# ThomasZiegler/RS-aware-differential-SfM

Hardware: AMD Instinct MI355X
Metric: Mpixels/sec RS depth+pose solve, 1280x720 pair (higher is better)
Workload: dtype f64

## Files before the change

### rs-aware-differential-sfm_amd/csrc/frame_host.hip

```cpp
#include <stdlib.h>
#include <string.h>

#include <atomic>

#include <algorithm>
#include <new>

#include "rsdsfm_internal.hpp"
#include "sequence_host.hpp"

namespace rsdsfm {

static std::atomic<int> g_frames_in_flight[64];
int frames_in_flight(const Ctx* c) { return g_frames_in_flight[c->device & 63].load(std::memory_order_relaxed); }

int alpha_ones_launch(Ctx* c, double* d_alpha, int64_t n);
int flatten_device(Ctx* c, const double* d_img, int32_t rows, int32_t cols, int32_t col0, double fx, double fy, double cx, double cy, double gamma,
                   double thr, double* d_q, double* d_u, double* d_alpha, double* d_alpha_k, int64_t* n_out);

struct FrameRun {
    rsdsfm_frame_job job;
    rsdsfm_frame_params prm;
    size_t N = 0;
    int64_t n = 0;
    double *d_q = nullptr, *d_u = nullptr, *d_a = nullptr, *d_ak = nullptr, *d_in_a = nullptr, *d_in_ak = nullptr, *d_inl = nullptr, *d_inl_ref = nullptr;
    int64_t* d_idx = nullptr;
    uint8_t* d_mask = nullptr;
    int32_t* d_ys = nullptr;
    double *d_zpartials = nullptr, *d_zheader = nullptr;
    char* d_refine_ws = nullptr;
    rsdsfm_ransac_out ro;
    RansacRun ransac;
    RefineRun refine;
    Minimal9Direct direct;
    DenseFlatten dense;
    bool refinement_enqueued = false, ahead = false, side_flatten = false, dense_in_launch = false, open = false;
    bool counted = false;
    int rc_begin = RSDSFM_OK;
    int64_t m_known = -1;
    RefineTail tail;
    FinishClaim claim;
    RansacSpecTail spec_tail;
    std::function<int()> join;
};

namespace {

inline double* header_host(Ctx* c) { return reinterpret_cast<double*>(static_cast<char*>(c->h_pinned) + c->pinned_bytes - 64); }
inline RefineState* state_host(Ctx* c) { return reinterpret_cast<RefineState*>(static_cast<char*>(c->h_pinned) + c->pinned_bytes - kPinnedTail); }
inline int64_t* count_host(Ctx* c) { return reinterpret_cast<int64_t*>(static_cast<char*>(c->h_pinned) + c->pinned_bytes - kPinnedTail / 2); }
static_assert(sizeof(RefineState) + sizeof(int) <= kPinnedTail / 2, "reserved tail: state read-back | point count ... depth-map header");

struct StreamSwap {
    Ctx* c;
    hipStream_t main;
    StreamSwap(Ctx* ctx, hipStream_t other) : c(ctx), main(ctx->stream) { c->stream = other; }
    ~StreamSwap() { c->stream = main; }
};

int ensure_side_stream(Ctx* c) {
    if (c->aux_stream) return RSDSFM_OK;
    RSDSFM_HIP_CHECK(c, hipStreamCreateWithFlags(&c->aux_stream, hipStreamNonBlocking));
    RSDSFM_HIP_CHECK(c, hipEventCreateWithFlags(&c->ev_fork, hipEventDisableTiming));
    RSDSFM_HIP_CHECK(c, hipEventCreateWithFlags(&c->ev_join, hipEventDisableTiming));
    return RSDSFM_OK;
}

static void frame_uncount(const Ctx* c, FrameRun* F) {
    if (F && F->counted) {
        F->counted = false;
        g_frames_in_flight[c->device & 63].fetch_sub(1, std::memory_order_relaxed);
    }
}
struct FrameInFlightEnd {
    const Ctx* c;
    FrameRun* F;
    ~FrameInFlightEnd() { frame_uncount(c, F); }
};

int frame_begin(Ctx* c, FrameRun* F) {
    const rsdsfm_frame_job& J = F->job;
    const rsdsfm_frame_params* prm = &F->prm;
    frame_uncount(c, F);
    F->open = false;
    F->rc_begin = RSDSFM_OK;
    if (J.rows <= 0 || J.cols <= 0 || !J.d_flow_img || !J.d_depth_map_colmajor) return fail(c, RSDSFM_ERR_INVALID, "bad arguments");
    if (prm->flow_index_mode != RSDSFM_FLOW_COMPAT_RANK && prm->flow_index_mode != RSDSFM_FLOW_GATHERED) return fail(c, RSDSFM_ERR_INVALID, "unknown flow_index_mode");
    if (prm->struct_bytes != 0 && prm->struct_bytes != (int32_t)sizeof(rsdsfm_frame_params))
        return fail(c, RSDSFM_ERR_INVALID, "rsdsfm_frame_params: struct_bytes is neither 0 nor sizeof(rsdsfm_frame_params) -- caller built against another header (use rsdsfm_frame_params_init)");
    const int32_t rows = J.rows, cols = J.cols;
    const double fx = J.fx, fy = J.fy, cx = J.cx, cy = J.cy, gamma = J.gamma;
    const size_t N = (size_t)rows * (size_t)cols;
    F->N = N;
    const size_t ncells = (size_t)flatten_cells(rows, cols);
    const size_t need = 2 * Arena::need(16 * N) + 4 * Arena::need(8 * N) + 2 * Arena::need(24 * N) + Arena::need(8 * N) + Arena::need(N) +
                        Arena::need(4 * N) + Arena::need(8 * 1024) + Arena::need(64) + Arena::need(refine_workspace_bytes(c, (int64_t)N, true)) +
                        2 * Arena::need(sizeof(int64_t) * (ncells + 2048)) + Arena::need(64) + 4096;
    if (need > c->frame_bytes) {
        RSDSFM_HIP_CHECK(c, hipStreamSynchronize(c->stream));
        if (c->d_frame) RSDSFM_HIP_CHECK(c, hipFree(c->d_frame));
        c->d_frame = nullptr;
        c->frame_bytes = 0;
        RSDSFM_HIP_CHECK(c, hipMalloc(&c->d_frame, need));
        c->frame_bytes = need;
    }
    Arena fa(c->d_frame);
    F->d_q = fa.take<double>(2 * N);
    F->d_u = fa.take<double>(2 * N);
    F->d_a = fa.take<double>(N);
    F->d_ak = fa.take<double>(N);
    F->d_in_a = fa.take<double>(N);
    F->d_in_ak = fa.take<double>(N);
    F->d_inl = fa.take<double>(3 * N);
    F->d_inl_ref = fa.take<double>(3 * N);
    F->d_idx = fa.take<int64_t>(N);
    F->d_mask = fa.take<uint8_t>(N);
    F->d_ys = fa.take<int32_t>(N);
    F->d_zpartials = fa.take<double>(1024);
    F->d_zheader = fa.take<double>(8);
    F->d_refine_ws = fa.take<char>(refine_workspace_bytes(c, (int64_t)N, true));
    int64_t* d_flat_counts = fa.take<int64_t>(ncells);
    int64_t* d_flat_offsets = fa.take<int64_t>(ncells + 2048);

    int rc = ensure_pinned(c, ransac_pinned_bytes(prm->ransac_trials));
    if (rc != RSDSFM_OK) return rc;
    int64_t n = (int64_t)N;
    F->side_flatten = false;
    if (c->frame_dense_hint) {
        *count_host(c) = -1;
        int side = prm->ransac_trials > 0 ? c->frame_side_flatten : 0;
        if (side == 3 && prm->ransac_trials > c->num_cus * 2) side = 0;
        F->dense_in_launch = false;
        if (side) {
            F->side_flatten = true;
            F->direct = Minimal9Direct();
            F->direct.img = J.d_flow_img, F->direct.rows = rows, F->direct.cols = cols, F->direct.alpha_ones = prm->use_global_shutter_mode ? 1 : 0;
            F->direct.fx = fx, F->direct.fy = fy, F->direct.cx = cx, F->direct.cy = cy, F->direct.gamma = gamma;
        }
        if (side == 3) {
            if (!c->d_flat_counters) {
                RSDSFM_HIP_CHECK(c, hipMalloc(reinterpret_cast<void**>(&c->d_flat_counters), 2 * sizeof(unsigned long long)));
                RSDSFM_HIP_CHECK(c, hipMemsetAsync(c->d_flat_counters, 0, 2 * sizeof(unsigned long long), c->stream));
            }
            F->dense = DenseFlatten();
            F->dense.thr = prm->flow_threshold;
            F->dense.d_q = F->d_q, F->dense.d_u = F->d_u, F->dense.d_alpha = F->d_a, F->dense.d_alpha_k = F->d_ak;
            F->dense.d_counters = c->d_flat_counters;
            F->dense.total_out = count_host(c);
            F->dense_in_launch = true;
        } else if (side == 2) {
            F->join = [c, F, d_flat_counts, d_flat_offsets]() -> int {
                const rsdsfm_frame_job& J2 = F->job;
                int rc2 = flatten_launch(c, J2.d_flow_img, J2.rows, J2.cols, 0, J2.fx, J2.fy, J2.cx, J2.cy, J2.gamma, F->prm.flow_threshold, F->d_q, F->d_u, F->d_a,
                                         F->d_ak, d_flat_counts, d_flat_offsets, count_host(c), nullptr);
                if (rc2 == RSDSFM_OK && F->prm.use_global_shutter_mode) rc2 = alpha_ones_launch(c, F->d_a, (int64_t)F->N);
                return rc2;
            };
        } else if (side == 1) {
            rc = ensure_side_stream(c);
            if (rc != RSDSFM_OK) return rc;
            RSDSFM_HIP_CHECK(c, hipEventRecord(c->ev_fork, c->stream));
            RSDSFM_HIP_CHECK(c, hipStreamWaitEvent(c->aux_stream, c->ev_fork, 0));
            {
                StreamSwap on_side(c, c->aux_stream);
                rc = flatten_launch(c, J.d_flow_img, rows, cols, 0, fx, fy, cx, cy, gamma, prm->flow_threshold, F->d_q, F->d_u, F->d_a, F->d_ak,
                                    d_flat_counts, d_flat_offsets, count_host(c), nullptr);
                if (rc == RSDSFM_OK && prm->use_global_shutter_mode) rc = alpha_ones_launch(c, F->d_a, n);
            }
            if (rc != RSDSFM_OK) return rc;
            RSDSFM_HIP_CHECK(c, hipEventRecord(c->ev_join, c->aux_stream));
            F->join = [c]() -> int {
                RSDSFM_HIP_CHECK(c, hipStreamWaitEvent(c->stream, c->ev_join, 0));
                return RSDSFM_OK;
            };
        } else {
            rc = flatten_enqueue(c, J.d_flow_img, rows, cols, fx, fy, cx, cy, gamma, prm->flow_threshold, F->d_q, F->d_u, F->d_a, F->d_ak, count_host(c));
            if (rc != RSDSFM_OK) return rc;
        }
    } else {
        rc = flatten_device(c, J.d_flow_img, rows, cols, 0, fx, fy, cx, cy, gamma, prm->flow_threshold, F->d_q, F->d_u, F->d_a, F->d_ak, &n);
        if (rc != RSDSFM_OK) return rc;
        *count_host(c) = n;
    }
    if (prm->use_global_shutter_mode && !F->side_flatten) {
        rc = alpha_ones_launch(c, F->d_a, n);
        if (rc != RSDSFM_OK) return rc;
    }
    F->n = n;
    memset(&F->ro, 0, sizeof(F->ro));
    F->ro.inlier_idx = F->d_idx;
    F->ro.inliers = F->d_inl;
    F->ro.alpha = F->d_in_a;
    F->ro.alpha_k = F->d_in_ak;
    F->ro.mask = F->d_mask;
    F->m_known = -1;
    F->tail = [c, F](const RefineBuffers& B) -> int {
        const rsdsfm_frame_job& J2 = F->job;
        const RefineState* st = B.state;
        const int64_t m_arg = F->m_known >= 0 ? F->m_known : F->n;
        const int64_t* m_dev = F->m_known >= 0 ? nullptr : &st->m;
        PoseTableOut pt;
        if (J2.d_R_rows9_or_null && J2.d_t_rows3_or_null)
            pt.R = J2.d_R_rows9_or_null, pt.t = J2.d_t_rows3_or_null, pt.rows = J2.rows, pt.gamma = J2.gamma, pt.wk_dev = st->p + 3;
        if (B.claim.on)
            return depth_map_decided_launch(c, F->d_inl_ref, m_arg, F->d_zpartials, refine_finish_grid(c, B), B, J2.d_depth_map_colmajor, F->d_zheader,
                                            header_host(c), st->p, m_dev, &pt);
        return depth_map_slab_launch(c, F->d_inl_ref, m_arg, F->d_zpartials, refine_finish_grid(c, B), m_arg, nullptr, J2.fx, J2.fy, J2.cx, J2.cy, J2.rows,
                                     0, J2.cols, J2.d_depth_map_colmajor, nullptr, F->d_ys, F->d_zheader, header_host(c), st->p, m_dev, &pt);
    };
    F->claim = FinishClaim();
    if (c->frame_tail == 0) {
        F->claim.on = true;
        F->claim.fx = J.fx, F->claim.fy = J.fy, F->claim.cx = J.cx, F->claim.cy = J.cy;
        F->claim.rows = rows, F->claim.cols = cols;
        F->claim.ys = F->d_ys;
    }
    F->spec_tail = [c, F](const RansacBest* d_best) -> int {
        return refine_begin(c, F->d_u, F->n, F->n, F->d_inl, F->d_in_a, F->d_in_ak, F->d_idx, nullptr, nullptr, 0.0, F->prm.use_acceleration_mode,
                            F->prm.flow_index_mode, F->d_inl_ref, &F->tail, d_best, F->d_refine_ws, &F->refine, state_host(c), F->d_zpartials, false,
                            &F->claim);
    };
    F->refinement_enqueued = false;
    F->ahead = prm->use_refinement && c->ransac_spec_miss < 2;
    F->open = true;
    g_frames_in_flight[c->device & 63].fetch_add(1, std::memory_order_relaxed);
    F->counted = true;
    F->rc_begin = ransac_begin(c, F->d_q, F->d_u, F->d_a, F->d_ak, n, prm->use_acceleration_mode, prm->ransac_trials, prm->ransac_tol, nullptr, J.seed,
                               prm->depth_mode, prm->k_sign_mode, &F->ro, prm->use_refinement ? &F->spec_tail : nullptr, &F->refinement_enqueued, &F->ransac,
                               F->side_flatten ? &F->direct : nullptr, F->side_flatten && !F->dense_in_launch ? &F->join : nullptr,
                               F->dense_in_launch ? &F->dense : nullptr, F->ahead, true,
                               F->claim.on && prm->use_refinement ? refine_flag_words(F->d_refine_ws) : nullptr);
    return RSDSFM_OK;
}

int frame_finish(Ctx* c, FrameRun* F, rsdsfm_frame_result* res) {
    if (!F->open) return fail(c, RSDSFM_ERR_INVALID, "no frame solve in flight");
    F->open = false;
    FrameInFlightEnd in_flight_end_{c, F};
    const rsdsfm_frame_job& J = F->job;
    const rsdsfm_frame_params* prm = &F->prm;
    memset(res, 0, sizeof(*res));
    int rc = F->rc_begin;
    if (rc == RSDSFM_OK) rc = ransac_finish(c, &F->ransac);
    if (rc != RSDSFM_OK) RSDSFM_HIP_CHECK(c, hipStreamSynchronize(c->stream));
    if (F->side_flatten && c->aux_stream) RSDSFM_HIP_CHECK(c, hipStreamSynchronize(c->aux_stream));
    int64_t n = F->n;
    if (*count_host(c) < 0) {
        c->frame_dense_hint = 1;
        return rc != RSDSFM_OK ? rc : fail(c, RSDSFM_ERR_NUMERIC, "frame solve: the point count did not arrive");
    }
    bool counted = true;
    if (*count_host(c) != n) {
        if (F->dense_in_launch) {
            int64_t n_real = 0;
            rc = flatten_device(c, J.d_flow_img, J.rows, J.cols, 0, J.fx, J.fy, J.cx, J.cy, J.gamma, prm->flow_threshold, F->d_q, F->d_u, F->d_a, F->d_ak, &n_real);
            if (rc == RSDSFM_OK && prm->use_global_shutter_mode) rc = alpha_ones_launch(c, F->d_a, n_real);
            if (rc != RSDSFM_OK) return rc;
            *count_host(c) = n_real;
        }
        n = *count_host(c);
        F->n = n;
        F->refinement_enqueued = false;
        counted = false;
        rc = ransac_begin(c, F->d_q, F->d_u, F->d_a, F->d_ak, n, prm->use_acceleration_mode, prm->ransac_trials, prm->ransac_tol, nullptr, J.seed,
                          prm->depth_mode, prm->k_sign_mode, &F->ro, prm->use_refinement ? &F->spec_tail : nullptr, &F->refinement_enqueued, &F->ransac, nullptr, nullptr,
                          nullptr, F->ahead, true,
                               F->claim.on && prm->use_refinement ? refine_flag_words(F->d_refine_ws) : nullptr);
        if (rc == RSDSFM_OK) rc = ransac_finish(c, &F->ransac);
        counted = rc == RSDSFM_OK;
    }
    c->frame_dense_hint = n == (int64_t)F->N ? 1 : 0;
    if (rc != RSDSFM_OK) return rc;
    if (counted) ransac_commit_hints(c, F->ransac);
    const rsdsfm_ransac_out& ro = F->ro;
    res->n_points = n;
    res->num_inliers = ro.num_inliers;
    res->best_trial = ro.best_trial;
    memcpy(res->ransac_w, ro.w, sizeof(ro.w));
    memcpy(res->ransac_v, ro.v, sizeof(ro.v));
    res->ransac_k = ro.k;
    double v[3], w[3], k = ro.k;
    for (int i = 0; i < 3; ++i) v[i] = ro.v[i], w[i] = ro.w[i];
    double* d_final = F->d_inl;
    int flipped = 0;
    F->m_known = ro.num_inliers;
    if (prm->use_refinement) {
        bool exact = false;
        if (F->refinement_enqueued) {
            rc = refine_poll(c, &F->refine, v, w, &k, &res->refine_summary);
            exact = rc == kRcRefineRestartExact;
        }
        if (!F->refinement_enqueued || exact)
            rc = refine_device(c, F->d_u, n, ro.num_inliers, F->d_inl, F->d_in_a, F->d_in_ak, F->d_idx, v, w, k, prm->use_acceleration_mode,
                               prm->flow_index_mode, F->d_inl_ref, v, w, &k, &res->refine_summary, &F->tail, F->d_zpartials, exact, &F->claim);
        if (rc != RSDSFM_OK) return rc;
        d_final = F->d_inl_ref;
        const double* h_header = header_host(c);
        flipped = h_header[0] != 0.0;
        v[0] = h_header[1], v[1] = h_header[2], v[2] = h_header[3];
    } else {
        rc = depth_map_device(c, d_final, ro.num_inliers, v, J.fx, J.fy, J.cx, J.cy, J.rows, J.cols, J.d_depth_map_colmajor, nullptr, F->d_ys, &flipped, w,
                              k, J.gamma, J.d_R_rows9_or_null, J.d_t_rows3_or_null);
        if (rc != RSDSFM_OK) return rc;
    }
    res->flipped = flipped;
    memcpy(res->v, v, sizeof(v));
    memcpy(res->w, w, sizeof(w));
    res->k = k;
    res->d_inliers = d_final;
    res->d_inlier_idx = F->d_idx;
    res->d_scanline = F->d_ys;
    return RSDSFM_OK;
}

FrameRun* frame_run_of(Ctx* c) {
    if (!c->frame_run) c->frame_run = new (std::nothrow) FrameRun();
    return static_cast<FrameRun*>(c->frame_run);
}

}

void frame_release(Ctx* c) {
    frame_uncount(c, static_cast<FrameRun*>(c->frame_run));
    delete static_cast<FrameRun*>(c->frame_run);
    c->frame_run = nullptr;
    for (rsdsfm_ctx* lane : c->lanes) rsdsfm_destroy(lane);
    c->lanes.clear();
    if (c->ev_fork) (void)hipEventDestroy(c->ev_fork);
    if (c->ev_join) (void)hipEventDestroy(c->ev_join);
    if (c->ev_seq) (void)hipEventDestroy(c->ev_seq);
    if (c->aux_stream) (void)hipStreamDestroy(c->aux_stream);
    if (c->d_flat_counters) (void)hipFree(c->d_flat_counters);
    c->d_flat_counters = nullptr;
    c->ev_fork = c->ev_join = c->ev_seq = nullptr;
    c->aux_stream = nullptr;
}

}

using namespace rsdsfm;

extern "C" {

void rsdsfm_frame_params_init(rsdsfm_frame_params* p) {
    if (!p) return;
    memset(p, 0, sizeof(*p));
    p->ransac_trials = 5;
    p->use_acceleration_mode = 0;
    p->use_refinement = 1;
    p->depth_mode = RSDSFM_DEPTH_CERES_LM;
    p->k_sign_mode = RSDSFM_K_COMPAT;
    p->flow_index_mode = RSDSFM_FLOW_COMPAT_RANK;
    p->use_global_shutter_mode = 0;
    p->struct_bytes = (int32_t)sizeof(rsdsfm_frame_params);
    p->ransac_tol = 0.05;
    p->flow_threshold = 1e-10;
    p->seed = 1;
}

int rsdsfm_solve_frame_dev(rsdsfm_ctx* ctx, const double* d_flow_img, int32_t rows, int32_t cols, double fx, double fy, double cx,
                           double cy, double gamma, const rsdsfm_frame_params* prm, double* d_depth_map, double* d_R_rows9,
                           double* d_t_rows3, rsdsfm_frame_result* res) {
    if (!ctx) return RSDSFM_ERR_INVALID;
    Ctx* c = &ctx->c;
    DeviceGuard device_guard_(c);
    if (!prm || !res) return fail(c, RSDSFM_ERR_INVALID, "bad arguments");
    FrameRun* F = frame_run_of(c);
    if (!F) return fail(c, RSDSFM_ERR_INVALID, "out of host memory");
    F->prm = *prm;
    F->job = rsdsfm_frame_job{d_flow_img, rows, cols, fx, fy, cx, cy, gamma, d_depth_map, d_R_rows9, d_t_rows3, prm->seed};
    int rc = frame_begin(c, F);
    if (rc != RSDSFM_OK) return rc;
    return frame_finish(c, F, res);
}

int rsdsfm_set_sequence_lanes(rsdsfm_ctx* ctx, int32_t lanes) {
    if (!ctx) return RSDSFM_ERR_INVALID;
    Ctx* c = &ctx->c;
    DeviceGuard device_guard_(c);
    if (lanes < 0 || lanes > 16) return fail(c, RSDSFM_ERR_INVALID, "lanes must be 0 (default) .. 16");
    c->seq_lanes = lanes;
    return RSDSFM_OK;
}

int rsdsfm_set_frame_tail(rsdsfm_ctx* ctx, int mode) {
    if (!ctx) return RSDSFM_ERR_INVALID;
    if (mode < 0 || mode > 1) return fail(&ctx->c, RSDSFM_ERR_INVALID, "mode must be 0 (short launch tail) or 1 (stage-by-stage launches)");
    ctx->c.frame_tail = mode;
    return RSDSFM_OK;
}

int rsdsfm_set_frame_side_flatten(rsdsfm_ctx* ctx, int mode) {
    if (!ctx) return RSDSFM_ERR_INVALID;
    if (mode < 0 || mode > 3) return fail(&ctx->c, RSDSFM_ERR_INVALID, "mode must be 0 (flatten first), 1 (flatten on a second stream), 2 (flatten behind the minimal solver) or 3 (flatten inside the solver's launch)");
    ctx->c.frame_side_flatten = mode;
    return RSDSFM_OK;
}

}

namespace rsdsfm {

int sequence_lane_count(const Ctx* c, int count) { return std::max(1, std::min<int>(count, c->seq_lanes > 0 ? c->seq_lanes : kSequenceLanesDefault)); }

int solve_frames_run(Ctx* c, const rsdsfm_frame_job* jobs, int32_t count, const rsdsfm_frame_params* prm, rsdsfm_frame_result* results, const PairHook* hook) {
    const int L = sequence_lane_count(c, count);
    while ((int)c->lanes.size() < L - 1) {
        rsdsfm_ctx* lane = nullptr;
        int rc = rsdsfm_create(&lane, c->device, nullptr);
        if (rc != RSDSFM_OK) return fail(c, rc, "could not create a sequence lane");
        c->lanes.push_back(lane);
    }
    auto lane_ctx = [&](int l) -> Ctx* { return l == 0 ? c : &c->lanes[(size_t)l - 1]->c; };
    if (L > 1) {
        if (!c->ev_seq) RSDSFM_HIP_CHECK(c, hipEventCreateWithFlags(&c->ev_seq, hipEventDisableTiming));
        RSDSFM_HIP_CHECK(c, hipEventRecord(c->ev_seq, c->stream));
    }
    for (int l = 1; l < L; ++l) {
        Ctx* lc = lane_ctx(l);
        RSDSFM_HIP_CHECK(c, hipStreamWaitEvent(lc->stream, c->ev_seq, 0));
        lc->ransac_k0 = c->ransac_k0;
        lc->ransac_math_mode = c->ransac_math_mode;
        lc->lm_arithmetic = c->lm_arithmetic;
        lc->refine_arithmetic = c->refine_arithmetic;
        lc->lma_count_only_force = c->lma_count_only_force;
        lc->frame_side_flatten = c->frame_side_flatten;
        lc->frame_tail = c->frame_tail;
        lc->refine_stage_mode = c->refine_stage_mode;
    }
    for (int l = 0; l < L; ++l) lane_ctx(l)->refine_stage_separate = L > 1;
    int first_error = RSDSFM_OK;
    int in_flight[16];
    for (int l = 0; l < 16; ++l) in_flight[l] = -1;
    auto finish_lane = [&](int l) {
        const int i = in_flight[l];
        if (i < 0) return;
        in_flight[l] = -1;
        Ctx* lc = lane_ctx(l);
        int rc = frame_finish(lc, static_cast<FrameRun*>(lc->frame_run), &results[i]);
        if (rc != RSDSFM_OK && first_error == RSDSFM_OK) {
            first_error = rc;
            if (lc != c) c->err = "pair " + std::to_string(i) + ": " + lc->err;
        }
        if (rc == RSDSFM_OK && hook && first_error == RSDSFM_OK) {
            rc = (*hook)(lc, i, static_cast<FrameRun*>(lc->frame_run)->job, results[i]);
            if (rc != RSDSFM_OK) {
                first_error = rc;
                c->err = "pair " + std::to_string(i) + ": " + std::string(lc->err);
            }
        }
    };
    for (int i = 0; i < count && first_error == RSDSFM_OK; ++i) {
        const int l = i % L;
        finish_lane(l);
        if (first_error != RSDSFM_OK) break;
        Ctx* lc = lane_ctx(l);
        FrameRun* F = frame_run_of(lc);
        if (!F) {
            first_error = fail(c, RSDSFM_ERR_INVALID, "out of host memory");
            break;
        }
        F->prm = *prm;
        F->job = jobs[i];
        int rc = frame_begin(lc, F);
        if (rc != RSDSFM_OK) {
            first_error = rc;
            if (lc != c) c->err = "pair " + std::to_string(i) + ": " + lc->err;
            break;
        }
        in_flight[l] = i;
    }
    for (;;) {
        int best = -1;
        for (int l = 0; l < L; ++l)
            if (in_flight[l] >= 0 && (best < 0 || in_flight[l] < in_flight[best])) best = l;
        if (best < 0) break;
        finish_lane(best);
    }
    for (int l = 0; l < L; ++l) lane_ctx(l)->refine_stage_separate = false;
    return first_error;
}

}

extern "C" {

int rsdsfm_solve_frames_dev(rsdsfm_ctx* ctx, const rsdsfm_frame_job* jobs, int32_t count, const rsdsfm_frame_params* prm, rsdsfm_frame_result* results) {
    if (!ctx) return RSDSFM_ERR_INVALID;
    Ctx* c = &ctx->c;
    DeviceGuard device_guard_(c);
    if (count < 0 || !prm || (count > 0 && (!jobs || !results))) return fail(c, RSDSFM_ERR_INVALID, "bad arguments");
    if (count == 0) return RSDSFM_OK;
    return solve_frames_run(c, jobs, count, prm, results, nullptr);
}

int rsdsfm_set_refine_stage(rsdsfm_ctx* ctx, int mode) {
    if (!ctx) return RSDSFM_ERR_INVALID;
    Ctx* c = &ctx->c;
    if (mode < 0 || mode > 2) return fail(c, RSDSFM_ERR_INVALID, "refine stage: 0 (automatic), 1 (in the next pass's prologue) or 2 (a launch of its own)");
    c->refine_stage_mode = mode;
    return RSDSFM_OK;
}

}
```

### rs-aware-differential-sfm_amd/csrc/ransac_host.hip

```cpp
#include <stdio.h>
#include <stdlib.h>
#include <string.h>

#include <algorithm>
#include <vector>

#include "rsdsfm_internal.hpp"

namespace rsdsfm {

namespace {


inline uint64_t splitmix64(uint64_t& state) {
    uint64_t z = (state += 0x9E3779B97F4A7C15ULL);
    z = (z ^ (z >> 30)) * 0xBF58476D1CE4E5B9ULL;
    z = (z ^ (z >> 27)) * 0x94D049BB133111EBULL;
    return z ^ (z >> 31);
}

void sample_indices(int64_t n, int T, uint64_t seed, std::vector<int32_t>& out) {
    struct Slot {
        int64_t key;
        int32_t val;
        uint32_t gen;
    };
    thread_local std::vector<Slot> table;
    thread_local uint32_t gen = 0;
    size_t cap = 64;
    while (cap < (size_t)T * 18 * 4) cap <<= 1;
    if (table.size() != cap || gen == 0xFFFFFFFFu) {
        table.assign(cap, Slot{-1, 0, 0});
        gen = 0;
    }
    gen += 1;
    Slot* tb = table.data();
    const uint32_t g = gen;
    auto slot = [&](int64_t i) -> size_t {
        size_t h = (size_t)(((uint64_t)i * 0x9E3779B97F4A7C15ull) >> 20) & (cap - 1);
        while (tb[h].gen == g && tb[h].key != i) h = (h + 1) & (cap - 1);
        return h;
    };
    auto get = [&](int64_t i) -> int32_t {
        const size_t h = slot(i);
        return tb[h].gen == g ? tb[h].val : (int32_t)i;
    };
    auto put = [&](int64_t i, int32_t v) {
        const size_t h = slot(i);
        tb[h].key = i;
        tb[h].val = v;
        tb[h].gen = g;
    };
    out.resize((size_t)T * 9);
    uint64_t st = seed;
    for (int t = 0; t < T; ++t) {
        int64_t n_temp = n;
        for (int j = 0; j < 9; ++j) {
            const int64_t r = (int64_t)(splitmix64(st) % (uint64_t)n_temp);
            const int32_t a = get(n_temp - 1), b = get(r);
            put(n_temp - 1, b);
            put(r, a);
            out[(size_t)t * 9 + j] = b;
            n_temp--;
        }
    }
}

}

void sample_indices(int64_t n, int T, uint64_t seed, int32_t* out) {
    std::vector<int32_t> v;
    sample_indices(n, T, seed, v);
    if (!v.empty()) memcpy(out, v.data(), sizeof(int32_t) * v.size());
}

size_t ransac_pinned_bytes(int T) {
    const size_t Tn = (size_t)std::max(T, 1);
    return sizeof(RansacBest) + 8 * sizeof(int) + sizeof(double) * 2 * Tn + sizeof(double) * 8 * Tn + sizeof(LmState) * Tn + 64 +
           sizeof(int32_t) * Tn * 9 + kPinnedTail;
}

namespace {

enum RansacPc { kPcStart = 0, kPcBatchBegin, kPcRoundEnqueue, kPcRoundWait, kPcAfterRounds, kPcScore, kPcFinal, kPcFinalWait, kPcDone };

int lma_start_over(Ctx* c, RansacRun& R, int guards) {
    R.analytic = false;
    R.lma_restarted = true;
    R.lma_guard |= guards;
    R.tie_margin = -kLmaTie;
    R.not_one_step = 0;
    R.final_done = R.spec_scored = R.tail_enqueued = R.spec_final = false;
    RSDSFM_HIP_CHECK(c, hipMemsetAsync(R.zero_begin, 0, R.zero_bytes, c->stream));
    R.b0 = 0;
    R.pc = kPcBatchBegin;
    return RSDSFM_OK;
}

int ransac_advance(Ctx* c, RansacRun& R, bool yield_at_wait) {
    rsdsfm_ransac_out* out = R.out;
    const int T = R.T, Tn = R.Tn, batch = R.batch, depth_mode = R.depth_mode;
    const int64_t n = R.n;
    const double tol = R.tol;
    int rc = RSDSFM_OK;
    for (;;) {
        switch (R.pc) {
            case kPcStart: {
                const bool zero_in_minimal9 = T > 0 && R.zero_bytes % 8 == 0 && (reinterpret_cast<uintptr_t>(R.zero_begin) & 7) == 0;
                if (!zero_in_minimal9) RSDSFM_HIP_CHECK(c, hipMemsetAsync(R.zero_begin, 0, R.zero_bytes, c->stream));
                if (T > 0) {
                    memcpy(R.h_samples_pinned, R.samples.data(), sizeof(int32_t) * (size_t)T * 9);
                    Minimal9Direct dir = R.direct ? *R.direct : Minimal9Direct();
                    R.core_epoch = 0;
                    if (R.core_math && depth_mode == RSDSFM_DEPTH_CERES_LM && T <= c->num_cus * 2 && c->d_core_flag) {
                        c->core_epoch = c->core_epoch >= 0x3fffffff ? 1 : c->core_epoch + 1;
                        dir.core_flag = c->d_core_flag;
                        dir.core_epoch = R.core_epoch = c->core_epoch;
                    }
                    if (R.direct && R.dense && T <= c->num_cus * 2)
                        rc = minimal9_flatten_launch(c, R.h_samples_pinned, T, R.use_alpha_k, R.k_sign_mode, R.d_hyp, zero_in_minimal9 ? R.zero_begin : nullptr,
                                                     zero_in_minimal9 ? R.zero_bytes : 0, dir, R.dense->thr, R.dense->d_q, R.dense->d_u, R.dense->d_alpha,
                                                     R.dense->d_alpha_k, R.dense->d_counters, R.dense->total_out);
                    else
                        rc = minimal9_launch(c, R.d_q, R.d_u, R.d_a, R.d_ak, R.h_samples_pinned, T, R.use_alpha_k, R.k_sign_mode, R.d_hyp,
                                             zero_in_minimal9 ? R.zero_begin : nullptr, zero_in_minimal9 ? R.zero_bytes : 0, &dir);
                    if (rc != RSDSFM_OK) return rc;
                    if (R.after_minimal9) {
                        rc = (*R.after_minimal9)();
                        if (rc != RSDSFM_OK) return rc;
                    }
                }
                R.b0 = 0;
                R.pc = kPcBatchBegin;
                break;
            }
            case kPcBatchBegin: {
                if (R.b0 >= T) {
                    R.pc = kPcFinal;
                    break;
                }
                R.B = std::min(batch, T - R.b0);
                R.need_score = true;
                if (depth_mode == RSDSFM_DEPTH_CERES_LM) {
                    if (R.b0 > 0)
                        RSDSFM_HIP_CHECK(c, hipMemsetAsync(R.d_flags, 0, (size_t)(reinterpret_cast<char*>(R.d_irr_count + R.batch) - reinterpret_cast<char*>(R.d_flags)), c->stream));
                    R.round = 0;
                    R.pc = kPcRoundEnqueue;
                } else {
                    R.pc = kPcScore;
                }
                break;
            }
            case kPcRoundEnqueue: {
                const int b0 = R.b0, B = R.B, round = R.round;
                bool flags_via_pick = false;
                if (round > 4 * kMaxIter) return fail(c, RSDSFM_ERR_NUMERIC, "LM state machines did not terminate");
                if (R.analytic && round == 0) {
                    rc = ransac_lma_launch(c, R.d_q, R.d_u, R.d_a, R.d_ak, n, R.d_hyp + (size_t)b0 * 8, B, R.d_states + b0, R.d_partials, R.d_flags,
                                           R.d_scored + b0, R.d_tcount + b0, R.d_terr + b0, tol, R.lma_cand, 2, R.d_irr_count, R.d_irr_list, R.d_unscored,
                                           nullptr, R.core_epoch ? c->d_core_flag : nullptr, R.core_epoch, R.count_only);
                } else {
                    rc = ransac_lm_round_launch(c, R.d_q, R.d_u, R.d_a, R.d_ak, n, R.d_hyp + (size_t)b0 * 8, B, R.d_states + b0, R.d_partials, R.d_flags,
                                                R.d_scored + b0, R.d_tcount + b0, R.d_terr + b0, round, tol, R.k0, R.fused_base, R.core_math,
                                                R.core_epoch ? c->d_core_flag : nullptr, R.core_epoch, R.d_unscored);
                }
                if (rc != RSDSFM_OK) return rc;
                if (round == 0 && B == T) {
                    const PickLazy lazy = R.count_only ? PickLazy{R.d_scored, R.d_unscored, R.d_flags + 1} : PickLazy();
                    if (c->ransac_score_idle < kScoreIdleLimit) {
                        if (R.count_only) {
                            rc = ransac_pick_launch(c, R.d_tcount, R.d_terr, T, R.d_hyp, R.d_best, nullptr, R.d_flags, nullptr, 0, nullptr, 0, 0, nullptr, 0.0, lazy);
                            if (rc != RSDSFM_OK) return rc;
                        }
                        rc = ransac_score_launch(c, R.d_q, R.d_u, R.d_a, R.d_ak, n, R.d_hyp, T, R.d_states, depth_mode, tol, R.d_scored, R.d_partials,
                                                 R.d_tcount, R.d_terr, R.d_unscored, R.d_flags + 1);
                        if (rc != RSDSFM_OK) return rc;
                        R.spec_scored = true;
                    }
                    rc = ransac_pick_launch(c, R.d_tcount, R.d_terr, T, R.d_hyp, R.d_best, R.h_best, R.d_flags, R.h_running, R.spec_scored ? 1 : 0,
                                            nullptr, 0, 0, nullptr, R.tie_margin, lazy);
                    if (rc != RSDSFM_OK) return rc;
                    flags_via_pick = true;
                    rc = ransac_final_launch(c, R.d_q, R.d_u, R.d_a, R.d_ak, n, R.d_best, R.d_states, depth_mode, tol, R.d_rho, R.d_mask, R.d_bcounts,
                                             R.d_boffs, out->inlier_idx, out->inliers, out->alpha, out->alpha_k, R.h_best, R.refine_flag_words);
                    if (rc != RSDSFM_OK) return rc;
                    R.final_done = true;
                    R.spec_final = true;
                    if (R.spec_tail && R.tail_ahead) {
                        rc = (*R.spec_tail)(R.d_best);
                        if (rc != RSDSFM_OK) return rc;
                        R.tail_enqueued = true;
                    }
                }
                if (!flags_via_pick) RSDSFM_HIP_CHECK(c, hipMemcpyAsync(R.h_running, R.d_flags, sizeof(int) * 8, hipMemcpyDeviceToHost, c->stream));
                R.pc = kPcRoundWait;
                if (yield_at_wait) return RSDSFM_OK;
                break;
            }
            case kPcRoundWait: {
                yield_at_wait = false;
                if (int rcs = sync_stream(c, "ransac_finish line 244")) return rcs;
                const int* h_running = R.h_running;
                if (R.round == 0 && R.analytic && (h_running[3] & 16) != 0) R.lma_guard |= h_running[3] >> 8;
                if (R.round == 0 && R.analytic && (h_running[3] & 6) != 0 && !((h_running[3] & 1) && R.core_math)) {
                    rc = lma_start_over(c, R, (h_running[3] >> 8) | ((h_running[3] & 4) ? (1 << 7) : 0));
                    if (rc != RSDSFM_OK) return rc;
                    break;
                }
                if (R.round == 0 && R.core_math && (h_running[3] & 1) != 0) {
                    R.core_math = false;
                    R.restarted = true;
                    R.not_one_step = 0;
                    R.final_done = R.spec_scored = R.tail_enqueued = R.spec_final = false;
                    R.dense = nullptr;
                    R.after_minimal9 = nullptr;
                    R.pc = kPcStart;
                    break;
                }
                if (R.round == 0) {
                    R.not_one_step += h_running[2];
                    if (R.b0 == 0) {
                        int best = 0;
                        for (int a2 = 1; a2 <= 3; ++a2)
                            if (h_running[4 + a2] > (best ? h_running[4 + best] : 0)) best = a2;
                        if (best) R.fused_base_next = best;
                        int second = 0;
                        for (int a2 = 1; a2 <= 3; ++a2)
                            if (a2 != best && h_running[4 + a2] > (second ? h_running[4 + second] : 0)) second = a2;
                        if (best) {
                            R.lma_cand_next[0] = best;
                            R.lma_cand_next[1] = second ? second : (best > 1 ? best - 1 : 2);
                        }
                    }
                }
                if (h_running[0] == 0) {
                    R.pc = kPcAfterRounds;
                } else {
                    R.final_done = false;
                    R.round += 1;
                    R.pc = kPcRoundEnqueue;
                }
                break;
            }
            case kPcAfterRounds: {
                R.need_score = R.h_running[1] > 0;
                if (R.B == T) R.score_hint_next = R.need_score ? 1 : 0;
                if (R.need_score && R.final_done && R.spec_scored && !R.h_best->lazy_pending) R.need_score = false;
                if (R.need_score) R.final_done = false;
                R.pc = kPcScore;
                break;
            }
            case kPcScore: {
                if (R.need_score) {
                    rc = ransac_score_launch(c, R.d_q, R.d_u, R.d_a, R.d_ak, n, R.d_hyp + (size_t)R.b0 * 8, R.B, R.d_states + R.b0, depth_mode, tol,
                                             depth_mode == RSDSFM_DEPTH_CERES_LM ? R.d_scored + R.b0 : nullptr, R.d_partials, R.d_tcount + R.b0,
                                             R.d_terr + R.b0, depth_mode == RSDSFM_DEPTH_CERES_LM ? R.d_unscored : nullptr, R.d_flags + 1);
                    if (rc != RSDSFM_OK) return rc;
                }
                R.b0 += batch;
                R.pc = kPcBatchBegin;
                break;
            }
            case kPcFinal: {
                if (!R.final_done) {
                    R.tail_enqueued = false;
                    R.spec_final = false;
                    rc = ransac_pick_launch(c, R.d_tcount, R.d_terr, T, R.d_hyp, R.d_best, R.h_best, nullptr, nullptr, 0, nullptr, 0, 0, nullptr, R.tie_margin,
                                            R.count_only ? PickLazy{R.d_scored, R.d_unscored, R.d_flags + 1} : PickLazy());
                    if (rc != RSDSFM_OK) return rc;
                    rc = ransac_final_launch(c, R.d_q, R.d_u, R.d_a, R.d_ak, n, R.d_best, R.d_states, depth_mode, tol, R.d_rho, R.d_mask, R.d_bcounts,
                                             R.d_boffs, out->inlier_idx, out->inliers, out->alpha, out->alpha_k, R.h_best, R.refine_flag_words);
                    if (rc != RSDSFM_OK) return rc;
                }
                if (R.spec_tail && !R.tail_enqueued) {
                    rc = (*R.spec_tail)(R.d_best);
                    if (rc != RSDSFM_OK) return rc;
                    R.tail_enqueued = true;
                }
                if (T > 0 && out->trial_count) RSDSFM_HIP_CHECK(c, hipMemcpyAsync(R.h_tcount, R.d_tcount, sizeof(double) * T, hipMemcpyDeviceToHost, c->stream));
                if (T > 0 && out->trial_err) RSDSFM_HIP_CHECK(c, hipMemcpyAsync(R.h_terr, R.d_terr, sizeof(double) * T, hipMemcpyDeviceToHost, c->stream));
                if (T > 0 && out->trial_vel) RSDSFM_HIP_CHECK(c, hipMemcpyAsync(R.h_hyp, R.d_hyp, sizeof(double) * 8 * T, hipMemcpyDeviceToHost, c->stream));
                if (T > 0 && out->trial_steps && depth_mode == RSDSFM_DEPTH_CERES_LM)
                    RSDSFM_HIP_CHECK(c, hipMemcpyAsync(R.h_states, R.d_states, sizeof(LmState) * T, hipMemcpyDeviceToHost, c->stream));
                R.pc = kPcFinalWait;
                if (yield_at_wait) return RSDSFM_OK;
                break;
            }
            case kPcFinalWait: {
                if (int rcs = sync_stream(c, "ransac_finish line 345")) return rcs;
                const RansacBest* h_best = R.h_best;
#ifdef RSDSFM_DEBUG_HOOKS
                if (getenv("RSDSFM_RANSAC_DEBUG")) fprintf(stderr, "[ransac] final wait: lazy_pending %d undecided %d flags %d %d %d %d hist %d %d %d %d spec_scored %d spec_final %d tail %d idle %d\n", h_best->lazy_pending, h_best->undecided, R.h_running[0], R.h_running[1], R.h_running[2], R.h_running[3], R.h_running[4], R.h_running[5], R.h_running[6], R.h_running[7], (int)R.spec_scored, (int)R.spec_final, (int)R.tail_enqueued, c->ransac_score_idle);
#endif
                if (R.count_only && h_best->lazy_pending) {
                    if (++R.lazy_rounds > T + 2) return fail(c, RSDSFM_ERR_NUMERIC, "lazy error sums did not settle");
                    R.final_done = R.tail_enqueued = R.spec_final = false;
                    R.need_score = true;
                    R.score_hint_next = 1;
                    R.b0 = 0;
                    R.B = T;
                    R.pc = kPcScore;
                    break;
                }
                if (R.analytic && h_best->lma_tie) {
                    rc = lma_start_over(c, R, 1 << 7);
                    if (rc != RSDSFM_OK) return rc;
                    break;
                }
                R.lma_tie_seen = h_best->lma_tie != 0;
                R.shared_best = h_best->shared_best;
                if (h_best->num_inliers != h_best->num_inliers_scan) {
                    if (R.analytic) {
                        rc = lma_start_over(c, R, 1 << 10);
                        if (rc != RSDSFM_OK) return rc;
                        break;
                    }
                    return fail(c, RSDSFM_ERR_NUMERIC, "inlier count mismatch between scoring and compaction");
                }
                out->num_inliers = h_best->num_inliers;
                out->best_trial = h_best->best_trial;
                memcpy(out->w, &h_best->hyp[0], 3 * sizeof(double));
                memcpy(out->v, &h_best->hyp[3], 3 * sizeof(double));
                out->k = h_best->hyp[6];
                out->inlier_error = h_best->inlier_error;
                for (int t = 0; t < T; ++t) {
                    if (out->trial_count) out->trial_count[t] = (int64_t)R.h_tcount[t];
                    if (out->trial_err) out->trial_err[t] = R.h_terr[t];
                    if (out->trial_vel) memcpy(out->trial_vel + (size_t)7 * t, R.h_hyp + (size_t)8 * t, 7 * sizeof(double));
                    if (out->trial_steps) out->trial_steps[t] = depth_mode == RSDSFM_DEPTH_CERES_LM ? R.h_states[t].num_successful : 1;
                }
                if (R.spec_tail_held) *R.spec_tail_held = R.tail_enqueued;
                R.hints_ready = true;
                R.pc = kPcDone;
                (void)Tn;
                return RSDSFM_OK;
            }
            default:
                return RSDSFM_OK;
        }
    }
}

}

void ransac_commit_hints(Ctx* c, const RansacRun& R) {
    if (!R.hints_ready || R.depth_mode != RSDSFM_DEPTH_CERES_LM || R.T <= 0) return;
    if (R.fused_base_next) c->ransac_fused_base = R.fused_base_next;
    if (R.score_hint_next >= 0) c->ransac_score_idle = R.score_hint_next ? 0 : std::min(c->ransac_score_idle + 1, kScoreIdleLimit);
    c->ransac_not_one_step = R.not_one_step;
    c->ransac_spec_miss = R.spec_final ? 0 : std::min(c->ransac_spec_miss + 1, 2);
    if (R.count_only) c->lma_count_only_runs += 1, c->lma_lazy_runs += (R.lazy_rounds > 0 || R.shared_best > 1) ? 1 : 0;
    if (R.lazy_rounds > 0 || R.shared_best > 1) c->lma_unique_run = 0;
    else if (R.shared_best == 1) c->lma_unique_run = std::min(c->lma_unique_run + 1, 2);
    if (R.lma_guard) c->lma_last_guard = R.lma_guard, c->lma_handed_over += 1;
    if (R.lma_restarted) {
        c->lma_hold = 16;
        c->lma_restarts += 1;
        c->lma_last_guard = R.lma_guard;
    } else if (c->lma_hold > 0 && !R.analytic) {
        c->lma_hold = R.lma_tie_seen ? 16 : c->lma_hold - 1;
    }
    if (R.restarted) {
        c->ransac_standard_math = 16;
        c->ransac_restarts += 1;
    } else if (c->ransac_standard_math > 0) {
        c->ransac_standard_math -= 1;
    }
}

int ransac_begin(Ctx* c, const double* d_q, const double* d_u, const double* d_a, const double* d_ak, int64_t n, int use_alpha_k, int T,
                 double tol, const int32_t* h_samples, uint64_t seed, int depth_mode, int k_sign_mode, rsdsfm_ransac_out* out,
                 const RansacSpecTail* spec_tail, bool* spec_tail_held, RansacRun* run, const Minimal9Direct* direct,
                 const std::function<int()>* after_minimal9, const DenseFlatten* dense, bool tail_ahead, bool count_only, int* refine_flag_words) {
    RansacRun& R = *run;
    R = RansacRun();
    R.tail_ahead = tail_ahead;
    R.core_math = c->ransac_math_mode == 0 && c->ransac_standard_math == 0;
    R.analytic = depth_mode == RSDSFM_DEPTH_CERES_LM && T > 0 && c->lm_arithmetic == 0 && c->lma_hold == 0;
    R.tie_margin = depth_mode != RSDSFM_DEPTH_CERES_LM || c->lm_arithmetic != 0 ? 0.0 : (R.analytic ? kLmaTie : -kLmaTie);
    R.lma_cand[0] = c->lma_cand[0], R.lma_cand[1] = c->lma_cand[1];
    R.count_only = count_only && R.analytic && T <= kRansacBatch && (c->lma_unique_run >= 2 || c->lma_count_only_force);
    if (R.count_only) R.tie_margin = 0.0;
    R.refine_flag_words = refine_flag_words;
    if (spec_tail_held) *spec_tail_held = false;
    if (!out) return fail(c, RSDSFM_ERR_INVALID, "null out");
    if (n < 9) return fail(c, RSDSFM_ERR_INVALID, "ransac needs at least 9 points (the reference would compute rand() % 0)");
    if (T < 0) return fail(c, RSDSFM_ERR_INVALID, "negative iterations");
    if (depth_mode != RSDSFM_DEPTH_CLOSED_FORM && depth_mode != RSDSFM_DEPTH_CERES_LM) return fail(c, RSDSFM_ERR_INVALID, "unknown depth_mode");
    if (n > (int64_t)INT32_MAX) return fail(c, RSDSFM_ERR_INVALID, "n exceeds the int32 sample index range");
    if (T > 0) {
        if (h_samples) {
            R.samples.assign(h_samples, h_samples + (size_t)T * 9);
            for (int32_t s : R.samples)
                if (s < 0 || s >= n) return fail(c, RSDSFM_ERR_INVALID, "sample index out of range");
        } else {
            sample_indices(n, T, seed, R.samples);
        }
    }
    const int Tn = std::max(T, 1);
    const int batch = std::min(Tn, kRansacBatch);
    const size_t partials_doubles = std::max<size_t>((size_t)ransac_lm_partials_doubles(c, n, batch), (size_t)ransac_lma_partials_doubles(c, n, batch));
    size_t need = Arena::need(sizeof(double) * Tn * 8) + Arena::need(sizeof(int) * batch) + Arena::need(sizeof(int) * ransac_lma_list_ints(batch)) +
                  Arena::need(sizeof(LmState) * Tn) + Arena::need(sizeof(double) * partials_doubles) +
                  Arena::need(sizeof(int) * 8) + 2 * Arena::need(sizeof(int) * Tn) + 2 * Arena::need(sizeof(double) * Tn) + Arena::need(sizeof(RansacBest)) +
                  2 * Arena::need(sizeof(int64_t) * 2048) + Arena::need(sizeof(double) * (size_t)n) + Arena::need((size_t)n) + 4096;
    int rc = ensure_ws(c, need);
    if (rc != RSDSFM_OK) return rc;
    Arena ws(c->d_ws);
    R.d_hyp = ws.take<double>((size_t)Tn * 8);
    R.zero_begin = ws.base + ws.off;
    R.d_states = ws.take<LmState>(Tn);
    R.d_scored = ws.take<int>(Tn);
    R.d_flags = ws.take<int>(8);
    R.d_irr_count = ws.take<int>(batch);
    R.zero_bytes = (size_t)((ws.base + ws.off) - R.zero_begin);
    R.d_irr_list = ws.take<int>(ransac_lma_list_ints(batch));
    R.d_unscored = ws.take<int>(batch);
    R.d_partials = ws.take<double>(partials_doubles);
    R.d_tcount = ws.take<double>(Tn);
    R.d_terr = ws.take<double>(Tn);
    R.d_best = ws.take<RansacBest>(1);
    R.d_bcounts = ws.take<int64_t>(2048);
    R.d_boffs = ws.take<int64_t>(2048);
    R.d_rho = out->inv_depth ? out->inv_depth : ws.take<double>((size_t)n);
    R.d_mask = out->mask ? out->mask : ws.take<uint8_t>((size_t)n);

    rc = ensure_pinned(c, ransac_pinned_bytes(T));
    if (rc != RSDSFM_OK) return rc;
    if (!c->d_core_flag) {
        RSDSFM_HIP_CHECK(c, hipMalloc(reinterpret_cast<void**>(&c->d_core_flag), 64));
        RSDSFM_HIP_CHECK(c, hipMemsetAsync(c->d_core_flag, 0, 64, c->stream));
    }
    char* hp = static_cast<char*>(c->h_pinned);
    R.h_best = reinterpret_cast<RansacBest*>(hp);
    R.h_running = reinterpret_cast<int*>(hp + sizeof(RansacBest));
    R.h_tcount = reinterpret_cast<double*>(hp + sizeof(RansacBest) + 32);
    R.h_terr = R.h_tcount + Tn;
    R.h_hyp = R.h_terr + Tn;
    R.h_states = reinterpret_cast<LmState*>(R.h_hyp + (size_t)8 * Tn);
    R.h_samples_pinned = reinterpret_cast<int32_t*>(R.h_states + Tn);

    R.d_q = d_q, R.d_u = d_u, R.d_a = d_a, R.d_ak = d_ak;
    R.n = n, R.T = T, R.Tn = Tn, R.batch = batch, R.tol = tol, R.depth_mode = depth_mode, R.use_alpha_k = use_alpha_k, R.k_sign_mode = k_sign_mode;
    R.out = out, R.spec_tail = spec_tail, R.spec_tail_held = spec_tail_held;
    R.direct = direct, R.after_minimal9 = after_minimal9, R.dense = dense;
    R.k0 = c->ransac_k0 != 0 ? c->ransac_k0 : (c->ransac_not_one_step == 0 ? 2 : (int)KMAX);
    R.fused_base = R.k0 == 2 ? 1 : std::min(std::max(c->ransac_fused_base, 1), (int)KMAX);
    R.pc = kPcStart;
    return ransac_advance(c, R, true);
}

int ransac_finish(Ctx* c, RansacRun* run) { return ransac_advance(c, *run, false); }

int ransac_device(Ctx* c, const double* d_q, const double* d_u, const double* d_a, const double* d_ak, int64_t n,
                  int use_alpha_k, int T, double tol, const int32_t* h_samples, uint64_t seed, int depth_mode,
                  int k_sign_mode, rsdsfm_ransac_out* out, const RansacSpecTail* spec_tail, bool* spec_tail_held) {
    RansacRun run;
    int rc = ransac_begin(c, d_q, d_u, d_a, d_ak, n, use_alpha_k, T, tol, h_samples, seed, depth_mode, k_sign_mode, out, spec_tail, spec_tail_held,
                          &run, nullptr, nullptr);
    if (rc == RSDSFM_OK) rc = ransac_finish(c, &run);
    if (rc == RSDSFM_OK) ransac_commit_hints(c, run);
    return rc;
}

}

using namespace rsdsfm;

extern "C" {

int rsdsfm_calculate_velocities(rsdsfm_ctx* ctx, const double* q, const double* u, const double* alpha, const double* alpha_k,
                                int32_t count, int use_alpha_k, int k_sign_mode, double* w, double* v, double* k) {
    if (!ctx) return RSDSFM_ERR_INVALID;
    Ctx* c = &ctx->c;
    DeviceGuard device_guard_(c);
    if (count < 0 || (count > 0 && (!q || !u || !alpha || !alpha_k || !w || !v || !k))) return fail(c, RSDSFM_ERR_INVALID, "bad arguments");
    if (count == 0) return RSDSFM_OK;
    const size_t T = (size_t)count;
    int rc = ensure_stage(c, 2 * Arena::need(144 * T) + 2 * Arena::need(72 * T) + Arena::need(64 * T));
    if (rc != RSDSFM_OK) return rc;
    Arena sa(c->d_stage);
    double* d_q = sa.take<double>(18 * T);
    double* d_u = sa.take<double>(18 * T);
    double* d_a = sa.take<double>(9 * T);
    double* d_ak = sa.take<double>(9 * T);
    double* d_h = sa.take<double>(8 * T);
    RSDSFM_HIP_CHECK(c, hipMemcpyAsync(d_q, q, 144 * T, hipMemcpyHostToDevice, c->stream));
    RSDSFM_HIP_CHECK(c, hipMemcpyAsync(d_u, u, 144 * T, hipMemcpyHostToDevice, c->stream));
    RSDSFM_HIP_CHECK(c, hipMemcpyAsync(d_a, alpha, 72 * T, hipMemcpyHostToDevice, c->stream));
    RSDSFM_HIP_CHECK(c, hipMemcpyAsync(d_ak, alpha_k, 72 * T, hipMemcpyHostToDevice, c->stream));
    rc = minimal9_launch(c, d_q, d_u, d_a, d_ak, nullptr, count, use_alpha_k, k_sign_mode, d_h);
    if (rc != RSDSFM_OK) return rc;
    std::vector<double> h(8 * T);
    RSDSFM_HIP_CHECK(c, hipMemcpyAsync(h.data(), d_h, 64 * T, hipMemcpyDeviceToHost, c->stream));
    RSDSFM_HIP_CHECK(c, hipStreamSynchronize(c->stream));
    int worst = 0;
    for (size_t t = 0; t < T; ++t) {
        memcpy(w + 3 * t, &h[8 * t], 3 * sizeof(double));
        memcpy(v + 3 * t, &h[8 * t + 3], 3 * sizeof(double));
        k[t] = h[8 * t + 6];
        if (h[8 * t + 7] != 0.0) worst = (int)h[8 * t + 7];
    }
    if (worst != 0) return fail(c, RSDSFM_ERR_NUMERIC, worst == -1 ? "no real eigenvalue k for at least one hypothesis" : "singular system in the k estimation");
    return RSDSFM_OK;
}

int rsdsfm_ransac_dev(rsdsfm_ctx* ctx, const double* d_q, const double* d_u, const double* d_alpha, const double* d_alpha_k,
                      int64_t n, int use_alpha_k, int32_t iterations, double tolerance, const int32_t* samples, uint64_t seed,
                      int depth_mode, int k_sign_mode, rsdsfm_ransac_out* out) {
    if (!ctx) return RSDSFM_ERR_INVALID;
    Ctx* c = &ctx->c;
    DeviceGuard device_guard_(c);
    if (!d_q || !d_u || !d_alpha || !d_alpha_k) return fail(c, RSDSFM_ERR_INVALID, "null device pointer");
    return ransac_device(c, d_q, d_u, d_alpha, d_alpha_k, n, use_alpha_k, iterations, tolerance, samples, seed, depth_mode, k_sign_mode, out,
                         nullptr, nullptr);
}

int rsdsfm_ransac(rsdsfm_ctx* ctx, const double* q, const double* u, const double* alpha, const double* alpha_k, int64_t n,
                  int use_alpha_k, int32_t iterations, double tolerance, const int32_t* samples, uint64_t seed, int depth_mode,
                  int k_sign_mode, rsdsfm_ransac_out* out) {
    if (!ctx) return RSDSFM_ERR_INVALID;
    Ctx* c = &ctx->c;
    DeviceGuard device_guard_(c);
    if (!out || !q || !u || !alpha || !alpha_k) return fail(c, RSDSFM_ERR_INVALID, "null pointer");
    if (n < 9) return fail(c, RSDSFM_ERR_INVALID, "ransac needs at least 9 points (the reference would compute rand() % 0)");
    const size_t N = (size_t)n;
    int rc = ensure_stage(c, 2 * Arena::need(16 * N) + 6 * Arena::need(8 * N) + Arena::need(24 * N) + Arena::need(N) + 4096);
    if (rc != RSDSFM_OK) return rc;
    Arena sa(c->d_stage);
    double* d_q = sa.take<double>(2 * N);
    double* d_u = sa.take<double>(2 * N);
    double* d_a = sa.take<double>(N);
    double* d_ak = sa.take<double>(N);
    rsdsfm_ransac_out dev = *out;
    dev.inlier_idx = sa.take<int64_t>(N);
    dev.inliers = sa.take<double>(3 * N);
    dev.alpha = sa.take<double>(N);
    dev.alpha_k = sa.take<double>(N);
    dev.inv_depth = sa.take<double>(N);
    dev.mask = sa.take<uint8_t>(N);
    c->ransac_cache.tag = 0;
    const uint64_t gen = c->stage_gen;
    xfer_trace("begin");
    const XferUp up[4] = {{d_q, q, 16 * N}, {d_u, u, 16 * N}, {d_a, alpha, 8 * N}, {d_ak, alpha_k, 8 * N}};
    if ((rc = xfer_h2d_many(c, up, 4)) != RSDSFM_OK) return rc;
    xfer_trace("uploaded");
    rc = ransac_device(c, d_q, d_u, d_a, d_ak, n, use_alpha_k, iterations, tolerance, samples, seed, depth_mode, k_sign_mode, &dev, nullptr, nullptr);
    if (rc != RSDSFM_OK) return rc;
    xfer_trace("solved");
    const size_t M = (size_t)dev.num_inliers;
    XferItem items[6];
    int ni = 0;
    if (out->inliers && M) items[ni++] = {out->inliers, dev.inliers, 24 * M};
    if (out->inlier_idx && M) items[ni++] = {out->inlier_idx, dev.inlier_idx, 8 * M};
    if (out->alpha && M) items[ni++] = {out->alpha, dev.alpha, 8 * M};
    if (out->alpha_k && M) items[ni++] = {out->alpha_k, dev.alpha_k, 8 * M};
    if (out->inv_depth) items[ni++] = {out->inv_depth, dev.inv_depth, 8 * N};
    if (out->mask) items[ni++] = {out->mask, dev.mask, N};
    if ((rc = xfer_d2h_many(c, items, ni)) != RSDSFM_OK) return rc;
    RSDSFM_HIP_CHECK(c, hipStreamSynchronize(c->stream));
    xfer_trace("downloaded");
    xfer_trace_dump("rsdsfm_ransac");
    if (out->inliers && out->alpha && out->alpha_k && out->inlier_idx && gen == c->stage_gen) {
        Ctx::RansacCache& rcache = c->ransac_cache;
        rcache.stage_gen = gen;
        rcache.d_u = d_u, rcache.d_inl = dev.inliers, rcache.d_alpha = dev.alpha, rcache.d_alpha_k = dev.alpha_k, rcache.d_idx = dev.inlier_idx;
        rcache.n = n, rcache.m = (int64_t)M, rcache.h_u = u;
        for (int j = 0; j < 16; ++j) {
            rcache.u_probe[j] = u[(2 * N - 1) * (size_t)j / 15];
            rcache.inl_probe[j] = M ? out->inliers[(3 * M - 1) * (size_t)j / 15] : 0.0;
        }
        rcache.tag = ++c->ransac_tag_counter;
    }
    out->num_inliers = dev.num_inliers;
    out->best_trial = dev.best_trial;
    memcpy(out->w, dev.w, sizeof(dev.w));
    memcpy(out->v, dev.v, sizeof(dev.v));
    out->k = dev.k;
    out->inlier_error = dev.inlier_error;
    return RSDSFM_OK;
}

}
```

### rs-aware-differential-sfm_amd/csrc/ransac_kernels.hip

```cpp
#include <algorithm>

#include "device_math.hpp"
#include "lm_common.hpp"
#include "rsdsfm_internal.hpp"

namespace rsdsfm {

namespace {

constexpr int kRB = 256;
constexpr int kRP = RSDSFM_FUSED ? 5 : 6;
constexpr int kFused = 1;
constexpr int kTiledFusedBase = 2;
constexpr int NSR = NS + 2 * kFused;
constexpr int kNSum = NSR - (KMAX + 1);
constexpr int kTStride = 65;

template <int K0>
struct R0Shape {
    static constexpr int NSk = 3 + 5 * K0;
    static constexpr int F = kFused;
    static constexpr int nsum = NSk - (K0 + 1) + 2 * F;
};
static_assert(R0Shape<KMAX>::nsum == kNSum, "full shape uses every sum slot");
// ... 281 lines not shown
__global__ __launch_bounds__(256) void ransac_lm_rows_kernel(const double* __restrict__ partials, int nblocks, int T,
                                                            const LmState* __restrict__ states, int round,
                                                            double* __restrict__ rows, const int* __restrict__ core_flags) {
    __shared__ double s_red[4][NSR];
    __shared__ double s_sums[NSR];
    const int t = blockIdx.x;
    if (core_flags && t == 0 && threadIdx.x < 2) rows[(int64_t)T * NSR + threadIdx.x] = (threadIdx.x == 0 && core_flags[3] != 0) ? 1.0 : 0.0;
    const LmState* state = states + t;
    if (round > 0 && (state->status != 0 || state->next_launch != round)) {
        if (threadIdx.x < NSR) rows[(int64_t)t * NSR + threadIdx.x] = 0.0;
        return;
    }
    reduce_hyp_sums(partials, nblocks, T, t, true, s_red, s_sums);
    if (threadIdx.x < NSR) rows[(int64_t)t * NSR + threadIdx.x] = s_sums[threadIdx.x];
}

__global__ __launch_bounds__(256) void ransac_decide_kernel(const double* __restrict__ partials, int nblocks, int T, int hyp_major,
                                                           LmState* states, int64_t n, int round, int k0, int* flags, int* pred_flag,
                                                           int* __restrict__ scored, double* __restrict__ trial_count,
                                                           double* __restrict__ trial_err, int fused_base, int* steps_hist,
                                                           int* __restrict__ unscored_list, int rank_stride2 = 0,
                                                           double* __restrict__ cnt_rt = nullptr, int cnt_stride = 0) {
    __shared__ double s_red[4][NSR];
    __shared__ double s_sums[NSR];
    __shared__ int s_fused_score;
    const int t = blockIdx.x;
    const int tid = threadIdx.x;
    LmState* state = states + t;
    if (tid == 0) s_fused_score = 0;
    if (rank_stride2 && t == 0 && tid < nblocks) {
        if (partials[(int64_t)tid * rank_stride2 * 2 + (int64_t)T * NSR] != 0.0) flags[3] = 1;
    }
    if (round > 0 && (state->status != 0 || state->next_launch != round)) return;
    reduce_hyp_sums(partials, nblocks, T, t, hyp_major != 0, s_red, s_sums, rank_stride2);
    if (tid == 0) {
        LmScal st = *static_cast<const LmScal*>(state);
        const bool first = round == 0 || st.launches == 0;
        const int used_K = (round == 0) ? k0 : st.K;
        lm_advance(st, state->hist, s_sums, n, first, used_K, 0, round);
        if (pred_flag && round == 0 && (st.status == 0 || st.n_hist >= 2)) atomicAdd(pred_flag, 1);
        if (steps_hist && round == 0) atomicAdd(&steps_hist[st.status == 0 ? 3 : (st.n_hist < 1 ? 0 : (st.n_hist > 3 ? 3 : st.n_hist))], 1);
        if (st.status == 0) {
            atomicAdd(&flags[0], 1);
        } else if (round == 0 && st.n_hist == fused_base) {
            trial_count[t] = s_sums[NS];
            trial_err[t] = s_sums[NS + 1];
            scored[t] = 1;
            s_fused_score = 1;
        } else {
            const int pos = atomicAdd(&flags[1], 1);
            if (unscored_list) unscored_list[pos] = t;
        }
        *static_cast<LmScal*>(state) = st;
    }
    if (cnt_rt) {
        __syncthreads();
        if (s_fused_score && tid < nblocks)
            cnt_rt[(int64_t)tid * cnt_stride + t] = partials[((int64_t)tid * (rank_stride2 ? rank_stride2 : T * (NSR / 2)) + (int64_t)t * (NSR / 2)) * 2 + NS];
    }
}

__device__ __forceinline__ double hyp_rho(double x, double y, double ux, double uy, double al, double ak, const Pose& pose,
                                          double two_over, int depth_mode, const LmPlanLds& plan) {
    if (depth_mode == RSDSFM_DEPTH_CLOSED_FORM) return closed_form_rho(x, y, ux, uy, al, ak, pose, two_over);
    double dummy[NS];
    return lm_pixel(x, y, ux, uy, al, ak, pose, two_over, plan, dummy);
}

__device__ __forceinline__ double score_error(const PixelModel& m, double x, double y, double ux, double uy, double al, double ak,
                                              const Pose& pose, double two_over, double rho) {
#if RSDSFM_FUSED
    (void)m;
    return point_error(x, y, ux, uy, al, ak, pose, two_over, rho);
#else
    (void)x, (void)y, (void)ux, (void)uy, (void)al, (void)ak, (void)pose, (void)two_over;
    return point_error_from_model(m, rho);
#endif
}

template <int NH>
__device__ __forceinline__ void score_pixels(const Tile& px, bool full_tile, const Pose& pose, double two_over, const LmState& st, double tol,
                                             double& cnt, double& es) {
    LmPlanReplay<NH> plan;
#pragma unroll
    for (int h = 0; h < NH; ++h) plan.ih[h] = 1.0 / st.hist[h];
    double dummy[NS];
#pragma unroll
    for (int j = 0; j < kRP; ++j) {
        if (full_tile || px.ok[j]) {
            PixelModel m;
            const double rho = lm_pixel(px.x[j], px.y[j], px.ux[j], px.uy[j], px.al[j], px.ak[j], pose, two_over, plan, dummy, NoHook(), &m);
            const double err = score_error(m, px.x[j], px.y[j], px.ux[j], px.uy[j], px.al[j], px.ak[j], pose, two_over, rho);
            if (err < tol) {
                cnt += 1.0;
                es += err;
            }
        }
    }
}

__device__ __forceinline__ void tile_group_of_block(int bid, int ntile_blocks, int ngroups, int& tb, int& grp) {
    const int tiles8 = ((ntile_blocks + 7) / 8) * 8;
    const int nfull = ngroups - 1;
    if (nfull > 0 && bid < tiles8 * nfull) {
        const int window = 8 * nfull;
        tb = (bid / window) * 8 + (bid % 8);
        grp = (bid % window) / 8;
    } else {
        tb = bid - tiles8 * nfull;
        grp = nfull;
    }
}

__global__ __launch_bounds__(kRB) void ransac_score_kernel(const double2* __restrict__ q, const double2* __restrict__ u,
                                                          const double* __restrict__ alpha,
                                                          const double* __restrict__ alpha_k, int64_t n,
                                                          const double* __restrict__ hyp, int T,
                                                          const LmState* __restrict__ states, int depth_mode, double tol,
                                                          const int* __restrict__ scored, double* __restrict__ partials, int ntile_blocks,
                                                          int ngroups, const int* __restrict__ list, const int* __restrict__ list_count) {
    extern __shared__ double s_acc[];
    __shared__ LmPlanLds plan;
    __shared__ double s_red[2][kRB / 64][2];
    __shared__ double s_T2[kRB / 64][2 * kTStride];
    __shared__ double s_half2[kRB / 64][2][2];
    const int tid = threadIdx.x, lane = tid & 63, wv = tid >> 6;
    int tb, grp;
    tile_group_of_block((int)blockIdx.x, ntile_blocks, ngroups, tb, grp);
    if (tb >= ntile_blocks) return;
    int t_begin, t_end;
    if (list) {
        const int U = min(*list_count, T);
        const int per = max(2, (U + ngroups - 1) / ngroups);
        t_begin = grp * per, t_end = min(U, t_begin + per);
        if (t_begin >= t_end) return;
    } else {
        const int per_group = (T + ngroups - 1) / ngroups;
        t_begin = grp * per_group, t_end = min(T, t_begin + per_group);
        if (scored) {
            bool any = false;
            for (int t = t_begin; t < t_end; ++t) any = any || !scored[t];
            if (!any) return;
        }
    }
    for (int i = tid; i < T * 2; i += kRB) s_acc[i] = 0.0;
    __syncthreads();
    const int64_t tile_pixels = (int64_t)kRB * kRP;
    const int64_t ntiles = (n + tile_pixels - 1) / tile_pixels;
    for (int64_t tile = tb; tile < ntiles; tile += ntile_blocks) {
        Tile px;
        load_tile(px, q, u, alpha, alpha_k, tile * tile_pixels, n);
        const bool full_tile = (tile + 1) * tile_pixels <= n;
        int done = 0;
        for (int ti = t_begin; ti < t_end; ++ti) {
            const int t = list ? list[ti] : ti;
            if (!list && scored && scored[t]) continue;
            RSDSFM_LOAD_POSE(pose, hyp, t)
            const double two_over = 2.0 / (2.0 + pose.k);
            double cnt = 0.0, es = 0.0;
            const int nh = depth_mode == RSDSFM_DEPTH_CERES_LM ? states[t].n_hist : -1;
            if (nh == 0) score_pixels<0>(px, full_tile, pose, two_over, states[t], tol, cnt, es);
            else if (nh == 1) score_pixels<1>(px, full_tile, pose, two_over, states[t], tol, cnt, es);
            else if (nh == 2) score_pixels<2>(px, full_tile, pose, two_over, states[t], tol, cnt, es);
            else if (nh == 3) score_pixels<3>(px, full_tile, pose, two_over, states[t], tol, cnt, es);
            else if (nh == 4) score_pixels<4>(px, full_tile, pose, two_over, states[t], tol, cnt, es);
            else {
                if (depth_mode == RSDSFM_DEPTH_CERES_LM) {
                    __syncthreads();
                    if (tid == 0) {
                        plan.n_hist = states[t].n_hist;
                        plan.K = 0;
                        plan.write_which = 0;
                    }
                    if (tid < kMaxIter) plan.inv_hist[tid] = 1.0 / states[t].hist[tid];
                    __syncthreads();
                }
#pragma unroll
                for (int j = 0; j < kRP; ++j) {
                    if (px.ok[j]) {
                        const double rho = hyp_rho(px.x[j], px.y[j], px.ux[j], px.uy[j], px.al[j], px.ak[j], pose, two_over, depth_mode, plan);
                        const double err = point_error(px.x[j], px.y[j], px.ux[j], px.uy[j], px.al[j], px.ak[j], pose, two_over, rho);
                        if (err < tol) {
                            cnt += 1.0;
                            es += err;
                        }
                    }
                }
            }
            double(*red)[2] = s_red[done & 1];
            ++done;
            {
                double* Tw = s_T2[wv];
                Tw[lane] = cnt;
                Tw[kTStride + lane] = es;
                __builtin_amdgcn_wave_barrier();
                const int sl = lane & 31, half = lane >> 5;
                if (sl < 2) {
                    const double* row = Tw + sl * kTStride + half * 32;
                    double part = row[0];
#pragma unroll
                    for (int j = 1; j < 32; ++j) part += row[j];
                    s_half2[wv][half][sl] = part;
                }
                __builtin_amdgcn_wave_barrier();
                if (lane < 2) red[wv][lane] = s_half2[wv][0][lane] + s_half2[wv][1][lane];
                __builtin_amdgcn_wave_barrier();
            }
            __syncthreads();
            if (tid < 2) {
                double r = red[0][tid];
                for (int w2 = 1; w2 < kRB / 64; ++w2) r += red[w2][tid];
                s_acc[t * 2 + tid] += r;
            }
        }
        __syncthreads();
    }
    __syncthreads();
    double* out = partials + (int64_t)tb * T * 2;
    if (list) {
        for (int i = t_begin * 2 + tid; i < t_end * 2; i += kRB) {
            const int t = list[i >> 1];
            out[t * 2 + (i & 1)] = s_acc[t * 2 + (i & 1)];
        }
    } else {
        for (int i = t_begin * 2 + tid; i < t_end * 2; i += kRB) out[i] = s_acc[i];
    }
}

__device__ __forceinline__ void reduce_score_rows(const double* __restrict__ partials, int nblocks, int T, int t, double& c_out, double& e_out) {
    constexpr int G = 256 / (NSR / 2);
    __shared__ double s_grp[G][2];
    const int tid = threadIdx.x;
    if (tid < G) {
        constexpr int U = 16;
        const double2* __restrict__ p2 = reinterpret_cast<const double2*>(partials);
        double c = 0.0, e = 0.0;
        for (int b = tid; b < nblocks; b += U * G) {
            double2 v[U];
#pragma unroll
            for (int j = 0; j < U; ++j) {
                const int bj = b + j * G;
                const double2 x = p2[(int64_t)(bj < nblocks ? bj : tid) * T + t];
                v[j] = bj < nblocks ? x : make_double2(0.0, 0.0);
            }
#pragma unroll
            for (int j = 0; j < U; ++j) {
                c += v[j].x;
                e += v[j].y;
            }
        }
        s_grp[tid][0] = c;
        s_grp[tid][1] = e;
    }
    __syncthreads();
    double c = s_grp[0][0], e = s_grp[0][1];
#pragma unroll
    for (int g2 = 1; g2 < G; ++g2) c += s_grp[g2][0], e += s_grp[g2][1];
    c_out = c, e_out = e;
}

__global__ __launch_bounds__(256) void ransac_reduce_scores_kernel(const double* __restrict__ partials, int nblocks, int T,
                                                                  const int* __restrict__ scored,
                                                                  double* __restrict__ trial_count,
                                                                  double* __restrict__ trial_err, double* __restrict__ cnt_rt = nullptr,
                                                                  int cnt_stride = 0) {
    const int t = blockIdx.x, tid = threadIdx.x;
    if (scored && scored[t]) return;
    double c, e;
    reduce_score_rows(partials, nblocks, T, t, c, e);
    if (tid == 0) {
        trial_count[t] = c;
        trial_err[t] = e;
    }
    if (cnt_rt && tid < nblocks) cnt_rt[(int64_t)tid * cnt_stride + t] = partials[((int64_t)tid * T + t) * 2];
}

__global__ __launch_bounds__(256) void ransac_score_rows_kernel(const double* __restrict__ partials, int nblocks, int T,
                                                               const int* __restrict__ scored, double* __restrict__ rows) {
    __shared__ double s_red[4][2];
    const int t = blockIdx.x, tid = threadIdx.x, lane = tid & 63, wv = tid >> 6;
    if (scored && scored[t]) {
        if (tid < 2) rows[(int64_t)t * 2 + tid] = 0.0;
        return;
    }
    double c = 0.0, e = 0.0;
    for (int b = tid; b < nblocks; b += 256) {
        c += partials[((int64_t)b * T + t) * 2 + 0];
        e += partials[((int64_t)b * T + t) * 2 + 1];
    }
    c = wave_sum(c);
    e = wave_sum(e);
    if (lane == 0) {
        s_red[wv][0] = c;
        s_red[wv][1] = e;
    }
    __syncthreads();
    if (tid == 0) {
        rows[(int64_t)t * 2 + 0] = ((s_red[0][0] + s_red[1][0]) + s_red[2][0]) + s_red[3][0];
        rows[(int64_t)t * 2 + 1] = ((s_red[0][1] + s_red[1][1]) + s_red[2][1]) + s_red[3][1];
    }
}

__device__ __forceinline__ void pick_best_trial(const double* __restrict__ trial_count, const double* __restrict__ trial_err, int T,
                                                int lane, int& bi, double& best_count, double& best_err) {
    best_count = -1.0, best_err = 0.0;
    bi = -1;
    for (int t0 = 0; t0 < T; t0 += 64) {
        const int t = t0 + lane;
        const double cl = t < T ? trial_count[t] : 0.0, el = t < T ? trial_err[t] : 0.0;
        const int nt = T - t0 < 64 ? T - t0 : 64;
        for (int j = 0; j < nt; ++j) {
            const double c = lane_value(cl, j), e = lane_value(el, j);
            if (c > best_count || (c == best_count && e < best_err)) {
                best_count = c;
                best_err = e;
                bi = t0 + j;
            }
        }
    }
}

__global__ __launch_bounds__(64) void ransac_pick_kernel(const double* __restrict__ trial_count, const double* __restrict__ trial_err, int T,
                                                        const double* __restrict__ hyp, RansacBest* best, RansacBest* best_host,
                                                        const int* __restrict__ flags, int* __restrict__ flags_host, int scored_ahead,
                                                        const double* __restrict__ cnt_rt = nullptr, int cnt_stride = 0, int nranks = 0,
                                                        int64_t* __restrict__ m_all = nullptr, double tie_margin = 0.0, PickLazy lazy = PickLazy()) {
    if (blockIdx.x != 0) return;
    const int lane = threadIdx.x;
    int undecided = (flags && (flags[0] != 0 || (flags[1] > 0 && !scored_ahead) || flags[3] != 0)) ? 1 : 0;
    double best_count, best_err;
    int bi;
    pick_best_trial(trial_count, trial_err, T, lane, bi, best_count, best_err);
    int tie = 0;
    if (tie_margin != 0.0 && bi >= 0 && best_count > 0.0 && !(flags && (flags[0] != 0 || (flags[1] > 0 && !scored_ahead)))) {
        const double tm = fabs(tie_margin);
        for (int t0 = 0; t0 < T; t0 += 64) {
            const int t = t0 + lane;
            const bool hit = t < T && t != bi && trial_count[t] == best_count && fabs(trial_err[t] - best_err) <= tm * best_count;
            if (__builtin_amdgcn_ballot_w64(hit) != 0) tie = 1;
        }
    }
    if (tie_margin > 0.0) undecided |= tie;
    int pending = 0, list_n = 0, ns = 0;
    if (bi >= 0 && best_count > 0.0 && !(flags && (flags[0] != 0 || (flags[1] > 0 && !scored_ahead) || flags[3] != 0))) {
        int nco = 0;
        for (int t0 = 0; t0 < T; t0 += 64) {
            const int t = t0 + lane;
            const bool hit = t < T && trial_count[t] == best_count;
            ns += __builtin_popcountll(__builtin_amdgcn_ballot_w64(hit));
            nco += __builtin_popcountll(__builtin_amdgcn_ballot_w64(hit && lazy.scored && lazy.scored[t] == 2));
        }
        if (ns > 1 && nco > 0) {
            int base = 0;
            for (int t0 = 0; t0 < T; t0 += 64) {
                const int t = t0 + lane;
                const bool co = t < T && trial_count[t] == best_count && lazy.scored[t] == 2;
                const unsigned long long mk = __builtin_amdgcn_ballot_w64(co);
                if (co) {
                    lazy.list[base + __builtin_popcountll(mk & ((1ull << lane) - 1ull))] = t;
                    lazy.scored[t] = 0;
                }
                base += __builtin_popcountll(mk);
            }
            if (lane == 0) *lazy.list_count = nco;
            pending = 1;
            list_n = nco;
            undecided = 1;
        }
    }
    if (flags_host && lane < 8) flags_host[lane] = (lane == 1 && pending) ? list_n : (flags[lane] | ((lane == 3 && tie && tie_margin > 0.0) ? 4 : 0));
    if (m_all)
        for (int r = lane; r < nranks; r += 64) m_all[r] = bi >= 0 ? (int64_t)cnt_rt[(int64_t)r * cnt_stride + bi] : 0;
    const double h = (lane < 8 && bi >= 0) ? hyp[(int64_t)bi * 8 + lane] : 0.0;
    if (lane < 8) best->hyp[lane] = h;
    if (lane < 8 && best_host) best_host->hyp[lane] = h;
    if (lane == 0) {
        best->best_trial = bi;
        best->undecided = undecided;
        best->lma_tie = tie;
        best->lazy_pending = pending;
        best->shared_best = ns;
        best->num_inliers = bi >= 0 ? (int64_t)best_count : 0;
        best->inlier_error = best_err;
        if (best_host) {
            best_host->best_trial = bi;
            best_host->undecided = undecided;
            best_host->lma_tie = tie;
            best_host->lazy_pending = pending;
            best_host->shared_best = ns;
            best_host->num_inliers = bi >= 0 ? (int64_t)best_count : 0;
            best_host->inlier_error = best_err;
        }
    }
}

__global__ __launch_bounds__(kRB) void ransac_final_kernel(const double2* __restrict__ q, const double2* __restrict__ u,
                                                          const double* __restrict__ alpha,
                                                          const double* __restrict__ alpha_k, int64_t n, int64_t chunk,
                                                          const RansacBest* __restrict__ best,
                                                          const LmState* __restrict__ states, int depth_mode, double tol,
                                                          double* __restrict__ rho_out, uint8_t* __restrict__ mask_out,
                                                          int64_t* __restrict__ block_counts) {
    __shared__ LmPlanLds plan;
    __shared__ int s_cnt[kRB / 64];
    const int tid = threadIdx.x, lane = tid & 63, wv = tid >> 6;
    if (best->undecided) return;
    const int bt = best->best_trial;
    Pose pose;
    pose.w[0] = best->hyp[0], pose.w[1] = best->hyp[1], pose.w[2] = best->hyp[2];
    pose.v[0] = best->hyp[3], pose.v[1] = best->hyp[4], pose.v[2] = best->hyp[5];
    pose.k = best->hyp[6];
    if (depth_mode == RSDSFM_DEPTH_CERES_LM && bt >= 0) {
        if (tid == 0) {
            plan.n_hist = states[bt].n_hist;
            plan.K = 0;
            plan.write_which = 0;
        }
        if (tid < kMaxIter) plan.inv_hist[tid] = 1.0 / states[bt].hist[tid];
    }
    __syncthreads();
    const double two_over = 2.0 / (2.0 + pose.k);
    const int64_t i0 = (int64_t)blockIdx.x * chunk;
    const int64_t i1 = (i0 + chunk < n) ? i0 + chunk : n;
    int count = 0;
    for (int64_t i = i0 + tid; i < i1; i += kRB) {
        double2 qq = q[i], uu = u[i];
        const double al = alpha[i], ak = alpha_k[i];
        bool in = false;
        double rho = 0.0;
        if (bt >= 0) {
            rho = hyp_rho(qq.x, qq.y, uu.x, uu.y, al, ak, pose, two_over, depth_mode, plan);
            in = point_error(qq.x, qq.y, uu.x, uu.y, al, ak, pose, two_over, rho) < tol;
        }
        rho_out[i] = rho;
        mask_out[i] = in ? 1 : 0;
        count += in ? 1 : 0;
    }
    for (int off = 32; off >= 1; off >>= 1) count += __shfl_xor(count, off, 64);
    if (lane == 0) s_cnt[wv] = count;
    __syncthreads();
    if (tid == 0) {
        int c = 0;
        for (int w2 = 0; w2 < kRB / 64; ++w2) c += s_cnt[w2];
        block_counts[blockIdx.x] = c;
    }
}

__global__ __launch_bounds__(256) void ransac_scan_kernel(const int64_t* __restrict__ block_counts, int nblocks,
                                                         int64_t* __restrict__ block_offsets, RansacBest* best, RansacBest* best_host) {
    __shared__ int64_t s_part[256];
    const int tid = threadIdx.x;
    const int per = (nblocks + 255) / 256;
    int64_t sum = 0;
    for (int j = 0; j < per; ++j) {
        const int b = tid * per + j;
        if (b < nblocks) sum += block_counts[b];
    }
    s_part[tid] = sum;
    __syncthreads();
    if (tid == 0) {
        int64_t run = 0;
        for (int i = 0; i < 256; ++i) {
            int64_t v = s_part[i];
            s_part[i] = run;
            run += v;
        }
        best->num_inliers_scan = run;
        if (best_host) best_host->num_inliers_scan = run;
    }
    __syncthreads();
    int64_t run = s_part[tid];
    for (int j = 0; j < per; ++j) {
        const int b = tid * per + j;
        if (b < nblocks) {
            block_offsets[b] = run;
            run += block_counts[b];
        }
    }
}

__global__ __launch_bounds__(kRB) void ransac_scatter_kernel(const double2* __restrict__ q, const double* __restrict__ alpha,
                                                            const double* __restrict__ alpha_k, int64_t n, int64_t chunk,
                                                            const double* __restrict__ rho, const uint8_t* __restrict__ mask,
                                                            const int64_t* __restrict__ block_counts, RansacBest* best,
                                                            RansacBest* best_host, int64_t* __restrict__ inlier_idx, double* __restrict__ inliers,
                                                            double* __restrict__ out_alpha, double* __restrict__ out_alpha_k,
                                                            int* __restrict__ zero_words = nullptr) {
    __shared__ int s_wave[kRB / 64];
    __shared__ int64_t s_base;
    if (zero_words && blockIdx.x == 0 && threadIdx.x < (int)(kRefineStateBlockTail / sizeof(int))) zero_words[threadIdx.x] = 0;
    __shared__ int64_t s_pre[kRB / 64], s_all[kRB / 64];
    const int tid = threadIdx.x, lane = tid & 63, wv = tid >> 6;
    const int undecided = best->undecided;
    const int64_t i0 = (int64_t)blockIdx.x * chunk;
    const int64_t i1 = (i0 + chunk < n) ? i0 + chunk : n;
    {
        int64_t pre = 0, all = 0;
        for (int b = tid; b < (int)gridDim.x; b += kRB) {
            const int64_t cnt = block_counts[b];
            all += cnt;
            if (b < (int)blockIdx.x) pre += cnt;
        }
#pragma unroll
        for (int off = 32; off > 0; off >>= 1) {
            pre += __shfl_down(pre, off);
            all += __shfl_down(all, off);
        }
        if (lane == 0) s_pre[wv] = pre, s_all[wv] = all;
        __syncthreads();
        if (tid == 0) {
            int64_t p2 = 0, a2 = 0;
            for (int w2 = 0; w2 < kRB / 64; ++w2) p2 += s_pre[w2], a2 += s_all[w2];
            s_base = p2;
            if (blockIdx.x == 0 && !undecided) {
                best->num_inliers_scan = a2;
                if (best_host) best_host->num_inliers_scan = a2;
            }
        }
    }
    if (undecided) return;
    __syncthreads();
    for (int64_t start = i0; start < i1; start += kRB) {
        const int64_t i = start + tid;
        const bool in = (i < i1) && mask[i] != 0;
        const unsigned long long bal = __ballot(in);
        const int prefix = __popcll(bal & ((1ull << lane) - 1ull));
        if (lane == 0) s_wave[wv] = __popcll(bal);
        __syncthreads();
        int woff = 0, total = 0;
#pragma unroll
        for (int w2 = 0; w2 < kRB / 64; ++w2) {
            const int c = s_wave[w2];
            if (w2 < wv) woff += c;
            total += c;
        }
        if (in) {
            const int64_t o = s_base + woff + prefix;
            double2 qq = q[i];
            if (inlier_idx) inlier_idx[o] = i;
            if (inliers) {
                inliers[3 * o + 0] = qq.x;
                inliers[3 * o + 1] = qq.y;
                inliers[3 * o + 2] = 1.0 / rho[i];
            }
            if (out_alpha) out_alpha[o] = alpha[i];
            if (out_alpha_k) out_alpha_k[o] = alpha_k[i];
        }
        __syncthreads();
        if (tid == 0) s_base += total;
        __syncthreads();
    }
}

int ransac_pixel_grid(const Ctx* c, int64_t n) {
    const int64_t tiles = (n + (int64_t)kRB * kRP - 1) / ((int64_t)kRB * kRP);
    int64_t g = tiles < 1 ? 1 : tiles;
    const int64_t cap = (int64_t)c->num_cus * 4;
    if (g > cap) {
        const int64_t iters = (g + cap - 1) / cap;
        g = (g + iters - 1) / iters;
    }
    return (int)g;
}

static int ransac_lm_groups(const Ctx* c, int grid, int T) {
    const int slots = c->num_cus * 2;
    int g = (8 * slots + grid - 1) / grid;
    g = std::min(g, T / 8);
    return std::max(g, 1);
}

int ransac_lm_partials_doubles(const Ctx* c, int64_t n, int batch) { return ransac_pixel_grid(c, n) * batch * NSR; }

static int lm_launch(Ctx* c, const dim3& g2, int k0, const double* q, const double* u, const double* a, const double* ak, int64_t n,
                     const double* hyp, int T, const LmState* states, double* partials, int round, double tol, int* flags, int fused_base,
                     bool core_math, const int* m9_flag, int m9_epoch, unsigned long long* clk = nullptr) {
    const double2* q2 = reinterpret_cast<const double2*>(q);
    const double2* u2 = reinterpret_cast<const double2*>(u);
    const size_t lds = sizeof(double) * T * NSR;
    const int tiles = (int)g2.x, groups = (int)g2.y;
    const dim3 g1((unsigned)(((tiles + 7) / 8) * 8 * groups));
    const int clk_bid = !clk ? -1 : groups > 1 ? (((tiles + 7) / 8) / 2) * 8 * (groups - 1) : tiles / 2;
#define RSDSFM_LM_LAUNCH(R0, K0, BASE, CORE) \
    hipLaunchKernelGGL((ransac_lm_kernel<R0, K0, BASE, CORE>), g1, dim3(kRB), lds, c->stream, q2, u2, a, ak, n, hyp, T, states, partials, round, tol, flags, tiles, groups, m9_flag, m9_epoch, clk, clk_bid)
    const bool core = core_math && flags != nullptr && !RSDSFM_FUSED;
    (void)core;
#if RSDSFM_FUSED
#define RSDSFM_LM_LAUNCH2(R0, K0, BASE) RSDSFM_LM_LAUNCH(R0, K0, BASE, false)
#else
#define RSDSFM_LM_LAUNCH2(R0, K0, BASE)                 \
    do {                                                \
        if (core) RSDSFM_LM_LAUNCH(R0, K0, BASE, true); \
        else RSDSFM_LM_LAUNCH(R0, K0, BASE, false);     \
    } while (0)
#endif
    if (round != 0)
        RSDSFM_LM_LAUNCH(false, KMAX, 0, false);
    else if (k0 == 2)
        RSDSFM_LM_LAUNCH2(true, 2, 1);
    else if (fused_base == 1)
        RSDSFM_LM_LAUNCH2(true, KMAX, 1);
    else if (fused_base == 3)
        RSDSFM_LM_LAUNCH2(true, KMAX, 3);
    else
        RSDSFM_LM_LAUNCH2(true, KMAX, 2);
#undef RSDSFM_LM_LAUNCH2
#undef RSDSFM_LM_LAUNCH
    RSDSFM_HIP_CHECK(c, hipGetLastError());
    return RSDSFM_OK;
}

int ransac_lm_round_launch(Ctx* c, const double* q, const double* u, const double* a, const double* ak, int64_t n,
                           const double* hyp, int T, LmState* states, double* partials, int* flags, int* scored,
                           double* trial_count, double* trial_err, int round, double tol, int k0, int fused_base, bool core_math,
                           const int* m9_core_flag, int m9_core_epoch, int* unscored_list) {
    const int grid = ransac_pixel_grid(c, n);
    const dim3 g2(grid, ransac_lm_groups(c, grid, T));
    if (k0 != 2) k0 = KMAX;
    if (fused_base < 1 || fused_base > k0) fused_base = std::min(2, k0);
    const bool prof = c->profile && round == 0 && c->ev_prof[0] && c->ev_prof[1];
    if (prof) RSDSFM_HIP_CHECK(c, hipEventRecord(c->ev_prof[0], c->stream));
    int rc = lm_launch(c, g2, k0, q, u, a, ak, n, hyp, T, states, partials, round, tol, flags, fused_base, core_math, round == 0 ? m9_core_flag : nullptr, m9_core_epoch,
                       prof ? c->d_clk_probe : nullptr);
    if (rc != RSDSFM_OK) return rc;
    if (prof) {
        RSDSFM_HIP_CHECK(c, hipEventRecord(c->ev_prof[1], c->stream));
        c->prof_pending = true;
        c->prof_what = 0;
    }
    hipLaunchKernelGGL(ransac_decide_kernel, dim3(T), dim3(256), 0, c->stream, partials, grid, T, 1, states, n, round, k0, flags, flags + 2, scored,
                       trial_count, trial_err, fused_base, flags + 4, unscored_list);
    RSDSFM_HIP_CHECK(c, hipGetLastError());
    return RSDSFM_OK;
}

int ransac_score_launch(Ctx* c, const double* q, const double* u, const double* a, const double* ak, int64_t n,
                        const double* hyp, int T, const LmState* states, int depth_mode, double tol, const int* scored,
                        double* partials, double* trial_count, double* trial_err, const int* unscored_list, const int* unscored_count) {
    const int grid = ransac_pixel_grid(c, n);
    const int groups = ransac_lm_groups(c, grid, T);
    hipLaunchKernelGGL(ransac_score_kernel, dim3(((grid + 7) / 8) * 8 * groups), dim3(kRB), sizeof(double) * T * 2, c->stream,
                       reinterpret_cast<const double2*>(q), reinterpret_cast<const double2*>(u), a, ak, n, hyp, T, states,
                       depth_mode, tol, scored, partials, grid, groups, unscored_list, unscored_list ? unscored_count : nullptr);
    RSDSFM_HIP_CHECK(c, hipGetLastError());
    hipLaunchKernelGGL(ransac_reduce_scores_kernel, dim3(T), dim3(256), 0, c->stream, partials, grid, T, scored, trial_count,
                       trial_err);
    RSDSFM_HIP_CHECK(c, hipGetLastError());
    return RSDSFM_OK;
}

int ransac_lm_rows_launch(Ctx* c, const double* q, const double* u, const double* a, const double* ak, int64_t n,
                          const double* hyp, int T, const LmState* states, double* partials, int round, double tol, double* rows,
                          int* core_flags, const int* m9_flag, int m9_epoch) {
    const int grid = ransac_pixel_grid(c, n);
    const dim3 g2(grid, ransac_lm_groups(c, grid, T));
    const bool core = core_flags != nullptr && round == 0;
    int rc = lm_launch(c, g2, KMAX, q, u, a, ak, n, hyp, T, states, partials, round, tol, core ? core_flags : nullptr, kTiledFusedBase, core,
                       core ? m9_flag : nullptr, m9_epoch);
    if (rc != RSDSFM_OK) return rc;
    hipLaunchKernelGGL(ransac_lm_rows_kernel, dim3(T), dim3(256), 0, c->stream, partials, grid, T, states, round, rows,
                       static_cast<const int*>(core ? core_flags : nullptr));
    RSDSFM_HIP_CHECK(c, hipGetLastError());
    return RSDSFM_OK;
}

int ransac_rows_payload_doubles(int T, bool core_trailer) { return T * NSR + (core_trailer ? 2 : 0); }

int ransac_decide_rows_launch(Ctx* c, const double* rows_all, int nranks, int T, LmState* states, int64_t n_total, int round,
                              int* flags, int* scored, double* trial_count, double* trial_err, bool core_trailer, double* cnt_rt, int cnt_stride) {
    if (cnt_rt && nranks > 256) return fail(c, RSDSFM_ERR_INVALID, "more than 256 ranks");
    RSDSFM_HIP_CHECK(c, hipMemsetAsync(flags, 0, sizeof(int), c->stream));
    hipLaunchKernelGGL(ransac_decide_kernel, dim3(T), dim3(256), 0, c->stream, rows_all, nranks, T, 0, states, n_total, round, (int)KMAX, flags,
                       static_cast<int*>(nullptr), scored, trial_count, trial_err, kTiledFusedBase, static_cast<int*>(nullptr),
                       static_cast<int*>(nullptr), core_trailer ? T * NSR / 2 + 1 : 0, cnt_rt, cnt_stride);
    RSDSFM_HIP_CHECK(c, hipGetLastError());
    return RSDSFM_OK;
}

int ransac_score_rows_launch(Ctx* c, const double* q, const double* u, const double* a, const double* ak, int64_t n,
                             const double* hyp, int T, const LmState* states, int depth_mode, double tol, const int* scored,
                             double* partials, double* rows) {
    const int grid = ransac_pixel_grid(c, n);
    const int groups = ransac_lm_groups(c, grid, T);
    hipLaunchKernelGGL(ransac_score_kernel, dim3(((grid + 7) / 8) * 8 * groups), dim3(kRB), sizeof(double) * T * 2, c->stream,
                       reinterpret_cast<const double2*>(q), reinterpret_cast<const double2*>(u), a, ak, n, hyp, T, states,
                       depth_mode, tol, scored, partials, grid, groups, static_cast<const int*>(nullptr), static_cast<const int*>(nullptr));
    RSDSFM_HIP_CHECK(c, hipGetLastError());
    hipLaunchKernelGGL(ransac_score_rows_kernel, dim3(T), dim3(256), 0, c->stream, partials, grid, T, scored, rows);
    RSDSFM_HIP_CHECK(c, hipGetLastError());
    return RSDSFM_OK;
}

int ransac_score_merge_launch(Ctx* c, const double* rows_all, int nranks, int T, const int* scored, double* trial_count,
                              double* trial_err, double* cnt_rt, int cnt_stride) {
    if (cnt_rt && nranks > 256) return fail(c, RSDSFM_ERR_INVALID, "more than 256 ranks");
    hipLaunchKernelGGL(ransac_reduce_scores_kernel, dim3(T), dim3(256), 0, c->stream, rows_all, nranks, T, scored, trial_count,
                       trial_err, cnt_rt, cnt_stride);
    RSDSFM_HIP_CHECK(c, hipGetLastError());
    return RSDSFM_OK;
}

int ransac_rows_doubles() { return NSR; }

int ransac_pick_launch(Ctx* c, const double* trial_count, const double* trial_err, int T, const double* hyp, RansacBest* best,
                       RansacBest* best_host, const int* d_flags, int* h_flags, int scored_ahead, const double* cnt_rt, int cnt_stride,
                       int nranks, int64_t* m_all, double tie_margin, PickLazy lazy) {
    hipLaunchKernelGGL(ransac_pick_kernel, dim3(1), dim3(64), 0, c->stream, trial_count, trial_err, T, hyp, best, best_host, d_flags, h_flags, scored_ahead,
                       cnt_rt, cnt_stride, nranks, m_all, tie_margin, lazy);
    RSDSFM_HIP_CHECK(c, hipGetLastError());
    return RSDSFM_OK;
}

int ransac_final_launch(Ctx* c, const double* q, const double* u, const double* a, const double* ak, int64_t n,
                        RansacBest* best, const LmState* states, int depth_mode, double tol, double* rho, uint8_t* mask,
                        int64_t* block_counts, int64_t* block_offsets, int64_t* inlier_idx, double* inliers,
                        double* out_alpha, double* out_alpha_k, RansacBest* best_host, int* zero_words) {
    int64_t blocks = (n + kRB - 1) / kRB;
    if (blocks < 1) blocks = 1;
    const int64_t cap = 2048;
    int64_t chunk = kRB;
    if (blocks > cap) {
        chunk = ((blocks + cap - 1) / cap) * kRB;
        blocks = (n + chunk - 1) / chunk;
    }
    hipLaunchKernelGGL(ransac_final_kernel, dim3((int)blocks), dim3(kRB), 0, c->stream, reinterpret_cast<const double2*>(q),
                       reinterpret_cast<const double2*>(u), a, ak, n, chunk, best, states, depth_mode, tol, rho, mask,
                       block_counts);
    RSDSFM_HIP_CHECK(c, hipGetLastError());
    if (inlier_idx || inliers || out_alpha || out_alpha_k) {
        hipLaunchKernelGGL(ransac_scatter_kernel, dim3((int)blocks), dim3(kRB), 0, c->stream, reinterpret_cast<const double2*>(q),
                           a, ak, n, chunk, rho, mask, block_counts, best, best_host, inlier_idx, inliers, out_alpha, out_alpha_k, zero_words);
    } else {
        if (zero_words) RSDSFM_HIP_CHECK(c, hipMemsetAsync(zero_words, 0, kRefineStateBlockTail, c->stream));
        hipLaunchKernelGGL(ransac_scan_kernel, dim3(1), dim3(256), 0, c->stream, block_counts, (int)blocks, block_offsets, best, best_host);
    }
    RSDSFM_HIP_CHECK(c, hipGetLastError());
    return RSDSFM_OK;
}

}
```

### rs-aware-differential-sfm_amd/csrc/refine_host.hip

```cpp
#include <string.h>

#include <algorithm>

#include "rsdsfm_internal.hpp"

namespace rsdsfm {

int refine_begin(Ctx* c, const double* d_flow, int64_t n_flow, int64_t m, const double* d_inl, const double* d_alpha,
                 const double* d_alpha_k, const int64_t* d_inlier_idx, const double v_in[3], const double w_in[3], double k_in,
                 int const_acceleration, int flow_index_mode, double* d_inl_out, const RefineTail* tail, const RansacBest* d_best,
                 void* ws_base, RefineRun* run, RefineState* hs_prefetch, double* d_zpartials, bool exact, const FinishClaim* claim) {
    if (m < 0 || n_flow < 0 || (!d_best && (!v_in || !w_in))) return fail(c, RSDSFM_ERR_INVALID, "bad arguments");
    if (flow_index_mode != RSDSFM_FLOW_COMPAT_RANK && flow_index_mode != RSDSFM_FLOW_GATHERED) return fail(c, RSDSFM_ERR_INVALID, "unknown flow_index_mode");
    if (flow_index_mode == RSDSFM_FLOW_GATHERED && m > 0 && !d_inlier_idx) return fail(c, RSDSFM_ERR_INVALID, "gathered mode needs inlier_idx");
    if (m > 0 && (!d_flow || !d_inl || !d_alpha || !d_alpha_k || !d_inl_out)) return fail(c, RSDSFM_ERR_INVALID, "null device pointer");
    const int np = const_acceleration ? 7 : 6;
    const size_t M = (size_t)std::max<int64_t>(m, 1);
    const size_t npart = (size_t)(d_best ? refine_partials_doubles_cap(c) : refine_partials_doubles(c, m));
    int rc = RSDSFM_OK;
    if (!ws_base) {
        rc = ensure_ws(c, refine_workspace_bytes(c, m, d_best != nullptr));
        if (rc != RSDSFM_OK) return rc;
        ws_base = c->d_ws;
    }
    rc = ensure_pinned(c, sizeof(RefineState) + 64);
    if (rc != RSDSFM_OK) return rc;
    Arena ws(ws_base);
    RefineBuffers& B = run->B;
    B = RefineBuffers();
    B.flow = d_flow;
    B.n_flow = n_flow;
    B.m = m;
    B.m_on_device = d_best != nullptr;
    B.inl = d_inl;
    B.alpha = d_alpha;
    B.alpha_k = d_alpha_k;
    B.inlier_idx = d_inlier_idx;
    B.flow_index_mode = flow_index_mode;
    static_assert(sizeof(RefineState) % sizeof(int) == 0, "flag follows the state");
    char* state_block = ws.take<char>(sizeof(RefineState) + 64);
    B.state = reinterpret_cast<RefineState*>(state_block);
    B.uu = ws.take<double>(4 * M);
    B.beta = ws.take<double>(M);
    B.rho_a = ws.take<double>(M);
    B.rho_b = ws.take<double>(M);
    B.srho = ws.take<double>(M);
    B.partials = ws.take<double>(npart);
    B.bad_index = reinterpret_cast<int*>(state_block + sizeof(RefineState));
    B.zpartials = d_zpartials;
    if (claim && claim->on && d_zpartials) B.claim = *claim;
    run->np = np;
    run->rf = !exact && c->lm_arithmetic == 0 && c->refine_arithmetic == 0;
    if (run->rf) c->refine_rf_runs += 1;
    run->d_inl_out = d_inl_out;
    run->tail = tail;
    run->launched = 0;
    run->hint_prev = c->refine_iters_hint;
    run->hs = hs_prefetch ? hs_prefetch : static_cast<RefineState*>(c->h_pinned);
    run->prefetch = hs_prefetch != nullptr;
    run->prefetched = false;
    B.state_host = hs_prefetch;
    if (d_best && claim && claim->on && run->rf && !c->refine_stage_separate) {
        B.best_dev = d_best;
    } else if (d_best) {
        rc = refine_state_from_best_launch(c, d_best, B, np);
        if (rc != RSDSFM_OK) return rc;
    } else {
        RefineState* hs = static_cast<RefineState*>(c->h_pinned);
        int* h_bad = reinterpret_cast<int*>(static_cast<char*>(c->h_pinned) + sizeof(RefineState));
        memset(hs, 0, sizeof(RefineState));
        hs->np = np;
        for (int i = 0; i < 3; ++i) {
            hs->p[i] = v_in[i];
            hs->p[3 + i] = w_in[i];
        }
        hs->p[6] = k_in;
        hs->termination = -1;
        hs->radius = kInitialRadius;
        hs->need_schur = 1;
        memset(h_bad, 0, kRefineStateBlockTail);
        RSDSFM_HIP_CHECK(c, hipMemcpyAsync(B.state, hs, sizeof(RefineState) + kRefineStateBlockTail, hipMemcpyHostToDevice, c->stream));
    }
    rc = refine_trace_reset(c);
    if (rc != RSDSFM_OK) return rc;
    if (!run->rf) {
        rc = refine_init_launch(c, B, np);
        if (rc != RSDSFM_OK) return rc;
    }
    const int hp = run->hint_prev;
    run->chunk = (hp >= 0 && hp <= 3) ? hp + 1 : (hp > 8 ? std::min(hp + 1, 28) : 7);
    return refine_enqueue_chunk(c, run);
}

int refine_enqueue_chunk(Ctx* c, RefineRun* run) {
    static const bool watch = getenv("RSDSFM_SYNC_WATCHDOG_S") != nullptr;
    if (watch) {
        const RefineBuffers B = run->B;
        const int launched = run->launched, chunk = run->chunk, rf = run->rf ? 1 : 0;
        set_sync_dumper([B, launched, chunk, rf](Ctx* cc) {
            fprintf(stderr, "[rsdsfm] last refinement chunk enqueued: slots [%d, %d), radius-factorised %d\n", launched, launched + chunk, rf);
            refine_rf_debug_dump(cc, B);
        });
    }
    if (run->rf) {
        for (int i = 0; i <= run->chunk; ++i) {
            const int g = run->launched + i;
            int rc = refine_rf_pass_launch(c, run->B, run->np, g, run->launched, nullptr, 0, -1, nullptr, i == run->chunk);
            if (rc != RSDSFM_OK) return rc;
        }
        run->launched += 1;
    } else {
        for (int i = 0; i < run->chunk; ++i) {
            int rc = refine_iter_launch(c, run->B, run->np, i, run->chunk);
            if (rc != RSDSFM_OK) return rc;
        }
    }
    run->launched += run->chunk;
    int rc = RSDSFM_OK;
    if (run->B.claim.on) {
        FinishClaim& C = run->B.claim;
        const int64_t npix = (int64_t)C.rows * C.cols;
        if (run->B.m >= ((int64_t)1 << 31)) return fail(c, RSDSFM_ERR_INVALID, "depth map: more than 2^31 inliers");
        rc = claim_map_acquire(c, 2, (size_t)std::max<int64_t>(std::max<int64_t>(npix, run->B.m), 1), &C.owner, &C.tag, &C.mask);
        if (rc != RSDSFM_OK) return rc;
    }
    rc = refine_finish_launch(c, run->B, run->d_inl_out);
    if (rc != RSDSFM_OK) return rc;
    run->tail_done = false;
    if (run->tail && !(run->hint_prev > run->launched + 1)) {
        rc = (*run->tail)(run->B);
        run->tail_done = true;
    }
    if (rc != RSDSFM_OK) return rc;
    if (run->prefetch) run->prefetched = true;
    return rc;
}

int refine_poll(Ctx* c, RefineRun* run, double v_out[3], double w_out[3], double* k_out, rsdsfm_lm_summary* summary) {
    if (!v_out || !w_out || !k_out) return fail(c, RSDSFM_ERR_INVALID, "bad arguments");
    RefineState* hs = run->hs;
    int* h_bad = reinterpret_cast<int*>(reinterpret_cast<char*>(hs) + sizeof(RefineState));
    for (bool first = true;; first = false) {
        if (!(first && run->prefetch && run->prefetched)) {
            if (!run->prefetch) RSDSFM_HIP_CHECK(c, hipMemcpyAsync(hs, run->B.state, sizeof(RefineState) + sizeof(int), hipMemcpyDeviceToHost, c->stream));
            if (int rcs = sync_stream(c, "refine_poll line 168")) return rcs;
        }
        if (*h_bad) return fail(c, RSDSFM_ERR_INVALID, "flow index out of range (flow has fewer columns than inliers / bad inlier_idx)");
        if (hs->termination == kTermRestartExact) {
            c->refine_rf_restarts += 1;
            c->refine_rf_last_guard = hs->rf_guard;
            return kRcRefineRestartExact;
        }
        if (hs->termination >= 0) {
            if (run->tail && !run->tail_done) {
                int rc = (*run->tail)(run->B);
                if (rc != RSDSFM_OK) return rc;
                run->tail_done = true;
                if (int rcs = sync_stream(c, "refine_poll line 181")) return rcs;
            }
            break;
        }
        if (run->launched > 8 * kMaxIter + 16) return fail(c, RSDSFM_ERR_NUMERIC, "refinement did not terminate");
        run->chunk = std::min(8, std::max(2, run->hint_prev - run->launched));
        int rc = refine_enqueue_chunk(c, run);
        if (rc != RSDSFM_OK) return rc;
    }
    c->refine_iters_hint = hs->slots;
    if (run->rf) c->refine_rf_resolves += hs->rf_resolves;
    for (int i = 0; i < 3; ++i) {
        v_out[i] = hs->p[i];
        w_out[i] = hs->p[3 + i];
    }
    *k_out = hs->p[6];
    if (summary) {
        summary->num_iterations = hs->iteration;
        summary->num_successful_steps = hs->num_successful;
        summary->num_unsuccessful_steps = hs->num_unsuccessful;
        summary->termination = hs->termination;
        summary->initial_cost = hs->initial_cost;
        summary->final_cost = hs->cost;
        summary->final_radius = hs->radius;
    }
    return RSDSFM_OK;
}

int* refine_flag_words(void* ws_base) {
    Arena ws(ws_base);
    return reinterpret_cast<int*>(ws.take<char>(sizeof(RefineState) + 64) + sizeof(RefineState));
}

size_t refine_workspace_bytes(const Ctx* c, int64_t m, bool m_on_device) {
    const size_t M = (size_t)std::max<int64_t>(m, 1);
    const size_t npart = (size_t)(m_on_device ? refine_partials_doubles_cap(c) : refine_partials_doubles(c, m));
    return Arena::need(sizeof(RefineState) + 64) + Arena::need(32 * M) + 4 * Arena::need(8 * M) + Arena::need(8 * npart) + Arena::need(64) + 1024;
}

int refine_device(Ctx* c, const double* d_flow, int64_t n_flow, int64_t m, const double* d_inl, const double* d_alpha,
                  const double* d_alpha_k, const int64_t* d_inlier_idx, const double v_in[3], const double w_in[3], double k_in,
                  int const_acceleration, int flow_index_mode, double* d_inl_out, double v_out[3], double w_out[3], double* k_out,
                  rsdsfm_lm_summary* summary, const RefineTail* tail, double* d_zpartials, bool exact, const FinishClaim* claim) {
    if (!v_out || !w_out || !k_out) return fail(c, RSDSFM_ERR_INVALID, "bad arguments");
    const double v0[3] = {v_in[0], v_in[1], v_in[2]}, w0[3] = {w_in[0], w_in[1], w_in[2]};
    for (int attempt = 0;; ++attempt) {
        RefineRun run;
        int rc = refine_begin(c, d_flow, n_flow, m, d_inl, d_alpha, d_alpha_k, d_inlier_idx, v0, w0, k_in, const_acceleration, flow_index_mode,
                              d_inl_out, tail, nullptr, nullptr, &run, nullptr, d_zpartials, exact || attempt > 0, claim);
        if (rc != RSDSFM_OK) return rc;
        rc = refine_poll(c, &run, v_out, w_out, k_out, summary);
        if (rc != kRcRefineRestartExact || attempt > 0) return rc == kRcRefineRestartExact ? fail(c, RSDSFM_ERR_NUMERIC, "refinement: restart loop") : rc;
    }
}

}

using namespace rsdsfm;

extern "C" {

int rsdsfm_refine_dev(rsdsfm_ctx* ctx, const double* d_flow, int64_t n_flow, int64_t m, const double* d_inl, const double* d_alpha,
                      const double* d_alpha_k, const int64_t* d_inlier_idx, const double v_in[3], const double w_in[3], double k_in,
                      int const_acceleration, int flow_index_mode, double* d_inl_out, double v_out[3], double w_out[3], double* k_out,
                      rsdsfm_lm_summary* summary) {
    if (!ctx) return RSDSFM_ERR_INVALID;
    DeviceGuard device_guard_(&ctx->c);
    return refine_device(&ctx->c, d_flow, n_flow, m, d_inl, d_alpha, d_alpha_k, d_inlier_idx, v_in, w_in, k_in, const_acceleration,
                         flow_index_mode, d_inl_out, v_out, w_out, k_out, summary, nullptr, nullptr);
}

static int refine_host(rsdsfm_ctx* ctx, uint64_t tag, const double* flow, int64_t n_flow, int64_t m, const double* inl, const double* alpha,
                       const double* alpha_k, const int64_t* inlier_idx, const double v_in[3], const double w_in[3], double k_in,
                       int const_acceleration, int flow_index_mode, double* inl_out, double v_out[3], double w_out[3], double* k_out,
                       rsdsfm_lm_summary* summary) {
    if (!ctx) return RSDSFM_ERR_INVALID;
    Ctx* c = &ctx->c;
    DeviceGuard device_guard_(c);
    if (m < 0 || n_flow < 0) return fail(c, RSDSFM_ERR_INVALID, "bad arguments");
    if (m > 0 && (!flow || !inl || !alpha || !alpha_k || !inl_out)) return fail(c, RSDSFM_ERR_INVALID, "null pointer");
    const size_t M = (size_t)m, NF = (size_t)n_flow;
    const Ctx::RansacCache& rcache = c->ransac_cache;
    bool cached = tag != 0 && tag == rcache.tag && rcache.stage_gen == c->stage_gen && rcache.m == m && M > 0 && (inlier_idx != nullptr || flow_index_mode == RSDSFM_FLOW_COMPAT_RANK);
    for (int j = 0; cached && j < 16; ++j) cached = memcmp(&rcache.inl_probe[j], &inl[(3 * M - 1) * (size_t)j / 15], sizeof(double)) == 0;
    bool flow_cached = cached && flow == rcache.h_u && n_flow == rcache.n;
    for (int j = 0; flow_cached && j < 16; ++j) flow_cached = memcmp(&rcache.u_probe[j], &flow[(2 * NF - 1) * (size_t)j / 15], sizeof(double)) == 0;
    int rc = RSDSFM_OK;
    const double *d_flow, *d_inl, *d_a, *d_ak;
    const int64_t* d_idx;
    double* d_out;
    if (cached) {
        const size_t extra = Arena::need(24 * M) + (flow_cached ? 0 : Arena::need(16 * NF)) + 1024;
        const size_t ws_ref = refine_workspace_bytes(c, m, false);
        rc = ensure_ws(c, ws_ref + extra);
        if (rc != RSDSFM_OK) return rc;
        Arena xa(static_cast<char*>(c->d_ws) + ((ws_ref + 255) & ~(size_t)255));
        d_out = xa.take<double>(3 * M);
        double* d_fl = flow_cached ? nullptr : xa.take<double>(2 * NF);
        if (!flow_cached && NF && (rc = xfer_h2d(c, d_fl, flow, 16 * NF)) != RSDSFM_OK) return rc;
        d_flow = flow_cached ? rcache.d_u : d_fl;
        d_inl = rcache.d_inl, d_a = rcache.d_alpha, d_ak = rcache.d_alpha_k, d_idx = inlier_idx ? rcache.d_idx : nullptr;
        c->refine_cache_hits += 1;
    } else {
        rc = ensure_stage(c, Arena::need(16 * NF) + 2 * Arena::need(24 * M) + 3 * Arena::need(8 * M) + 2048);
        if (rc != RSDSFM_OK) return rc;
        Arena sa(c->d_stage);
        double* s_flow = sa.take<double>(2 * NF);
        double* s_inl = sa.take<double>(3 * M);
        d_out = sa.take<double>(3 * M);
        double* s_a = sa.take<double>(M);
        double* s_ak = sa.take<double>(M);
        int64_t* s_idx = sa.take<int64_t>(M);
        const XferUp up[5] = {{s_flow, flow, 16 * NF}, {s_inl, inl, 24 * M}, {s_a, alpha, 8 * M}, {s_ak, alpha_k, 8 * M}, {s_idx, inlier_idx, inlier_idx ? 8 * M : 0}};
        if ((rc = xfer_h2d_many(c, up, 5)) != RSDSFM_OK) return rc;
        d_flow = s_flow, d_inl = s_inl, d_a = s_a, d_ak = s_ak, d_idx = inlier_idx ? s_idx : nullptr;
    }
    xfer_trace(cached ? "begin (resident)" : "uploaded");
    rc = refine_device(c, d_flow, n_flow, m, d_inl, d_a, d_ak, d_idx, v_in, w_in, k_in, const_acceleration, flow_index_mode, d_out, v_out, w_out, k_out,
                       summary, nullptr, nullptr);
    if (rc != RSDSFM_OK) return rc;
    xfer_trace("solved");
    if (M && (rc = xfer_d2h(c, inl_out, d_out, 24 * M)) != RSDSFM_OK) return rc;
    RSDSFM_HIP_CHECK(c, hipStreamSynchronize(c->stream));
    xfer_trace("downloaded");
    xfer_trace_dump("rsdsfm_refine");
    return RSDSFM_OK;
}

int rsdsfm_refine(rsdsfm_ctx* ctx, const double* flow, int64_t n_flow, int64_t m, const double* inl, const double* alpha,
                  const double* alpha_k, const int64_t* inlier_idx, const double v_in[3], const double w_in[3], double k_in,
                  int const_acceleration, int flow_index_mode, double* inl_out, double v_out[3], double w_out[3], double* k_out,
                  rsdsfm_lm_summary* summary) {
    return refine_host(ctx, 0, flow, n_flow, m, inl, alpha, alpha_k, inlier_idx, v_in, w_in, k_in, const_acceleration, flow_index_mode, inl_out, v_out, w_out,
                       k_out, summary);
}

int rsdsfm_refine_from_ransac(rsdsfm_ctx* ctx, uint64_t ransac_tag, const double* flow, int64_t n_flow, int64_t m, const double* inl,
                              const double* alpha, const double* alpha_k, const int64_t* inlier_idx, const double v_in[3], const double w_in[3],
                              double k_in, int const_acceleration, int flow_index_mode, double* inl_out, double v_out[3], double w_out[3],
                              double* k_out, rsdsfm_lm_summary* summary) {
    return refine_host(ctx, ransac_tag, flow, n_flow, m, inl, alpha, alpha_k, inlier_idx, v_in, w_in, k_in, const_acceleration, flow_index_mode, inl_out, v_out,
                       w_out, k_out, summary);
}

int rsdsfm_last_ransac_tag(rsdsfm_ctx* ctx, uint64_t* tag, int64_t* cache_hits_or_null) {
    if (!ctx || !tag) return RSDSFM_ERR_INVALID;
    *tag = ctx->c.ransac_cache.stage_gen == ctx->c.stage_gen ? ctx->c.ransac_cache.tag : 0;
    if (cache_hits_or_null) *cache_hits_or_null = ctx->c.refine_cache_hits;
    return RSDSFM_OK;
}

}
```

### rs-aware-differential-sfm_amd/csrc/refine_rf_kernels.hip

```cpp
#include "refine_common.hpp"

#ifndef RF_LOADS_ONLY
#define RF_LOADS_ONLY 0
#endif
#ifndef RF_NP7_PREFETCH
#define RF_NP7_PREFETCH 0
#endif

namespace rsdsfm {

namespace {

constexpr int kRfListCap = 64;
constexpr int kRfEntry = 8;

template <int NP>
struct RfRow {
    static constexpr int TRI = NP * (NP + 1) / 2;
    static constexpr int OFF_JTJ = 0, OFF_B = TRI, OFF_JTB = 2 * TRI, OFF_C = 2 * TRI + NP;
    static constexpr int NSCHUR = 2 * TRI + 2 * NP;
    static constexpr int MODEL = NSCHUR, STEPSQ = NSCHUR + 1, COST2 = NSCHUR + 2, XSQ = NSCHUR + 3, ZSUM = NSCHUR + 4, GMAX = NSCHUR + 5;
    static constexpr int NW = NSCHUR + 6;
    static constexpr int NF = TRI + NP;
    static_assert(NW % 2 == 0, "rows are read as double2");
// ... 574 lines not shown
    int* list_count;
    double* list_entries;
    int* list_count_zero;
    const RfExt* ext_in;
    RfExt* ext_out;
    double* partials;
    double* trace;
    int trace_rows;
    int64_t m_total;
    const int64_t* m_total_dev;
    const double2* flow;
    int64_t n_flow;
    const double* inl;
    const int64_t* inlier_idx;
    int flow_index_mode;
    int* bad_index;
    unsigned long long* beat;
    int slot;
    const RansacBest* best;
    int grid_cap;
    unsigned long long* stamps;
};

struct RfLoad {
    double4 c4;
    double rho, ab, ak;
};
template <int NP>
__device__ __forceinline__ RfLoad rf_load(const RfPassArgs& A, const double* __restrict__ rho, int64_t i, bool live) {
    RfLoad l;
    l.c4 = make_double4(0.0, 0.0, 0.0, 0.0), l.rho = 0.0, l.ab = 0.0, l.ak = 0.0;
    if (live) {
        l.c4 = A.xyuv_in[i];
        l.rho = rho[i];
        if (NP == 6) {
            l.ab = A.beta[i];
        } else {
            l.ab = A.alpha[i], l.ak = A.alpha_k[i];
        }
    }
    return l;
}

}

template <int NP, bool FIRST, bool ZSUM>
__global__ __launch_bounds__(kFB) void refine_rf_pass_kernel(const RfPassArgs A) {
    using RR = RfRow<NP>;
    __shared__ RfStageLds<NP> s_stage;
    __shared__ double s_red[kFB / 64][RR::NW];
    __shared__ RefineState s_state;
    const bool stamp = A.stamps && blockIdx.x == 0 && threadIdx.x == 0;
    if (A.beat && threadIdx.x == 0) {
        if (A.beat[7]) atomicAdd(&A.beat[2], 1ull);
        if (blockIdx.x == 0) A.beat[0] = ((unsigned long long)A.slot << 8) | 1;
        if (blockIdx.x < 512) A.beat[8 + blockIdx.x] = ((unsigned long long)A.slot << 8) | 1;
    }
    __shared__ unsigned long long tk[8];
    if (stamp) {
#pragma unroll
        for (int i = 0; i < 8; ++i) tk[i] = 0;
    }
    if (stamp) tk[0] = wall_clock64();
    if (FIRST && A.best) {
        if (threadIdx.x < sizeof(RefineState) / 8) reinterpret_cast<unsigned long long*>(&s_state)[threadIdx.x] = 0ull;
        __syncthreads();
        if (threadIdx.x == 0) {
            RefineState& z = s_state;
            z.np = NP;
            for (int i = 0; i < 3; ++i) {
                z.p[i] = A.best->hyp[3 + i];
                z.p[3 + i] = A.best->hyp[i];
            }
            z.p[6] = A.best->hyp[6];
            z.termination = -1;
            z.radius = kInitialRadius;
            z.need_schur = 1;
            const int64_t mb = A.best->undecided ? 0 : A.best->num_inliers_scan;
            z.m = mb;
            int64_t b = (mb + kFB - 1) / kFB;
            if (b < 1) b = 1;
            if (b > A.grid_cap) {
                const int64_t iters = (b + A.grid_cap - 1) / A.grid_cap;
                b = (b + iters - 1) / iters;
            }
            z.grid = (int)b;
        }
        __syncthreads();
    } else {
        state_to_lds(&s_state, A.st_in);
    }
    RefineState* st = &s_state;
    if (stamp) tk[1] = wall_clock64();
    if (FIRST) {
        if (threadIdx.x < 7) st->p0[threadIdx.x] = st->p[threadIdx.x];
        if (threadIdx.x == 0) st->rf = 1, st->rf_guard = 0, st->rf_resolves = 0, st->pending_apply = 0;
        __syncthreads();
    } else if (st->termination < 0 && st->pending_apply) {
        int64_t mt = A.m_total_dev ? *A.m_total_dev : (A.m_total >= 0 ? A.m_total : (A.m >= 0 ? A.m : st->m));
        rf_apply_body<NP>(st, s_stage, A.rows_prev, A.nrows_prev >= 0 ? A.nrows_prev : st->grid, A.row_stride, A.lists_prev, A.ext_in,
                          blockIdx.x == 0 ? A.ext_out : nullptr, mt, blockIdx.x == 0 ? A.trace : nullptr, A.trace_rows, stamp ? tk + 4 : nullptr);
        __syncthreads();
    }
    if (threadIdx.x == 0) st->pending_apply = st->termination < 0 ? 1 : 0;
    __syncthreads();
    if (stamp) tk[2] = wall_clock64();
    if (A.beat && threadIdx.x == 0) {
        if (blockIdx.x == 0) A.beat[0] = ((unsigned long long)A.slot << 8) | 2;
        if (blockIdx.x < 512) A.beat[8 + blockIdx.x] = ((unsigned long long)A.slot << 8) | ((st->termination >= 0 || (A.m < 0 && (int)blockIdx.x >= st->grid)) ? 9 : 2);
        if (A.beat[7] && (st->termination >= 0 || (A.m < 0 && (int)blockIdx.x >= st->grid))) atomicAdd(&A.beat[3], 1ull);
    }
    if (blockIdx.x == 0) {
        state_from_lds(A.st_out, st);
        if (threadIdx.x == 0) *A.list_count_zero = 0;
    }
    if (st->termination >= 0) return;
    const PassShape ps = pass_shape(st, A.m);
    if (!ps.live) return;
    const int64_t m = ps.m;
    double acc[RR::NW];
#pragma unroll
    for (int s = 0; s < RR::NW; ++s) acc[s] = 0.0;
    constexpr bool kLdsC = NP == 7 && !FIRST;
    __shared__ double s_cacc[kLdsC ? 3 * NP : 1][kLdsC ? kFB : 1];
    double* const lds_c = kLdsC ? &s_cacc[0][threadIdx.x] : nullptr;
    if (kLdsC) {
#pragma unroll
        for (int a = 0; a < 3 * NP; ++a) lds_c[a * kFB] = 0.0;
    }
    const int64_t stride = (int64_t)ps.grid * kFB;
    const int64_t i0 = (int64_t)blockIdx.x * kFB + threadIdx.x;
    RfPoint P0q = rf_point(st->p0);
    const RfPoint P0 = rf_point_uniform(P0q);
    if (FIRST) {
        RfPoint Pq = rf_point(st->p);
        const RfPoint P = rf_point_uniform(Pq);
        for (int64_t i = i0; i < m; i += stride) {
            int64_t fi = (A.flow_index_mode == RSDSFM_FLOW_GATHERED) ? A.inlier_idx[i] : i;
            if (fi < 0 || fi >= A.n_flow) {
                *A.bad_index = 1;
                fi = 0;
            }
            const double2 f = A.flow[fi];
            const double x = A.inl[3 * i], y = A.inl[3 * i + 1];
            const double rho = 1.0 / A.inl[3 * i + 2];
            const double al = A.alpha[i], ak = A.alpha_k[i];
            A.xyuv_out[i] = make_double4(x, y, f.x, f.y);
            const double ab = NP == 6 ? P.c1 * __builtin_fma(P.k, ak, al) : al;
            if (NP == 6) A.beta[i] = ab;
            A.rho_a[i] = rho;
            const RfGeom g = rf_geom(x, y);
            double be, dbe;
            rf_beta<NP>(ab, ak, P, be, dbe);
            RfEval<NP> o;
            rf_resid<NP>(g, f.x, f.y, be, P, rho, o);
            rf_jac<NP>(g, be, dbe, rho, o);
            acc[RR::COST2] = __builtin_fma(o.r0, o.r0, __builtin_fma(o.r1, o.r1, acc[RR::COST2]));
            acc[RR::GMAX] = fmax(acc[RR::GMAX], fabs(__builtin_fma(o.J0, o.r0, o.J1 * o.r1)));
            acc[RR::XSQ] = __builtin_fma(rho, rho, acc[RR::XSQ]);
            if (ZSUM) acc[RR::ZSUM] += 1.0 / rho;
            const bool flagged = rf_flagged(o.h, o.h);
            const double ihm = flagged ? 0.0 : rcp_core(flagged ? 1.0 : o.h);
            rf_schur_accumulate<NP>(o, ihm, acc);
            if (flagged) rf_list_append(A.list_count, A.list_entries, x, y, f.x, f.y, ab, ak, rho, i);
        }
    } else {
        RfPoint Pq = rf_point(st->p), Pcq = rf_point(st->pc);
        const RfPoint P = rf_point_uniform(Pq), Pc = rf_point_uniform(Pcq);
        double dp[7];
#pragma unroll
        for (int c = 0; c < 7; ++c) dp[c] = uniform_d(st->dp[c]);
        const double inv_radius = uniform_d(1.0 / st->radius);
        const double psi = uniform_d(1.0 / (1.0 + 1.0 / st->radius));
        const double* __restrict__ rho = st->cur ? A.rho_b : A.rho_a;
        double* __restrict__ cand = st->cur ? A.rho_a : A.rho_b;
        auto body = [&](const RfLoad& l0, int64_t i) {
            const double x = l0.c4.x, y = l0.c4.y, ux = l0.c4.z, uy = l0.c4.w, rh = l0.rho;
            const RfGeom g = rf_geom(x, y);
            double be, dbe, bec, dbec, be0, dbe0;
            rf_beta<NP>(l0.ab, l0.ak, P, be, dbe);
            rf_beta<NP>(l0.ab, l0.ak, Pc, bec, dbec);
            rf_beta<NP>(l0.ab, l0.ak, P0, be0, dbe0);
            RfEval<NP> o;
            rf_resid<NP>(g, ux, uy, be, P, rh, o);
            double da0, da1, db0, db1;
            rf_av(g, dp[0], dp[1], dp[2], da0, da1);
            rf_bw(g, dp[3], dp[4], dp[5], db0, db1);
            double t0 = be * __builtin_fma(rh, da0, db0), t1 = be * __builtin_fma(rh, da1, db1);
            if (NP == 7) {
                const double dk = dbe * dp[6];
                t0 = __builtin_fma(dk, o.in0, t0);
                t1 = __builtin_fma(dk, o.in1, t1);
            }
            double a00, a10;
            rf_av(g, P0.v0, P0.v1, P0.v2, a00, a10);
            const double h0 = (be0 * be0) * __builtin_fma(a00, a00, a10 * a10);
            const double gJ = __builtin_fma(o.J0, o.r0, o.J1 * o.r1), tJ = __builtin_fma(o.J0, t0, o.J1 * t1);
            const bool flagged = rf_flagged(o.h, h0);
            double drho = -((psi * (gJ + tJ)) * rcp_core(flagged ? 1.0 : o.h));
            if (__builtin_amdgcn_ballot_w64(flagged) != 0) {
                if (flagged) {
                    asm volatile("; listed inlier: exact e-block inverse" ::: "memory");
                    double sr, E0, E1;
                    const double ete_inv = rf_ete_inv_exact(o.J0, o.J1, h0, inv_radius, sr, E0, E1);
                    drho = -((ete_inv * (sr * (gJ + tJ))) * sr);
                }
            }
            const double m0 = __builtin_fma(o.J0, drho, t0), m1 = __builtin_fma(o.J1, drho, t1);
            acc[RR::MODEL] -= __builtin_fma(m0, __builtin_fma(0.5, m0, o.r0), m1 * __builtin_fma(0.5, m1, o.r1));
            const double cd = rh + drho;
            cand[i] = cd;
            acc[RR::STEPSQ] = __builtin_fma(drho, drho, acc[RR::STEPSQ]);
            RfEval<NP> oc;
            rf_resid<NP>(g, ux, uy, bec, Pc, cd, oc);
            rf_jac<NP>(g, bec, dbec, cd, oc);
            acc[RR::COST2] = __builtin_fma(oc.r0, oc.r0, __builtin_fma(oc.r1, oc.r1, acc[RR::COST2]));
            acc[RR::GMAX] = fmax(acc[RR::GMAX], fabs(__builtin_fma(oc.J0, oc.r0, oc.J1 * oc.r1)));
            acc[RR::XSQ] = __builtin_fma(cd, cd, acc[RR::XSQ]);
            if (ZSUM) acc[RR::ZSUM] += 1.0 / cd;
            const bool flagged_c = rf_flagged(oc.h, h0);
            const double ihm = flagged_c ? 0.0 : rcp_core(flagged_c ? 1.0 : oc.h);
            rf_schur_accumulate<NP>(oc, ihm, acc, lds_c);
            if (flagged_c) rf_list_append(A.list_count, A.list_entries, x, y, ux, uy, l0.ab, l0.ak, cd, i);
        };
        const int64_t last = m - 1;
        if (NP == 6) {
            RfLoad l0 = rf_load<NP>(A, rho, i0, i0 <= last);
            RfLoad l1 = rf_load<NP>(A, rho, i0 + stride, i0 + stride <= last);
            for (int64_t i = i0; i < m; i += stride) {
                const int64_t i2 = i + 2 * stride;
                const RfLoad l2 = rf_load<NP>(A, rho, i2, i2 <= last);
#if RF_LOADS_ONLY
                acc[0] += l0.c4.x + l0.c4.y + l0.c4.z + l0.c4.w + l0.rho + l0.ab;
                cand[i] = l0.rho;
#else
                body(l0, i);
#endif
                l0 = l1;
                l1 = l2;
            }
        } else {
#if RF_NP7_PREFETCH == 1
            RfLoad l0 = rf_load<NP>(A, rho, i0, i0 <= last);
            for (int64_t i = i0; i < m; i += stride) {
                const RfLoad l1 = rf_load<NP>(A, rho, i + stride, i + stride <= last);
                body(l0, i);
                l0 = l1;
            }
#else
            for (int64_t i = i0; i < m; i += stride) body(rf_load<NP>(A, rho, i, true), i);
#endif
        }
    }
    if (kLdsC) {
        int tri = 0;
#pragma unroll
        for (int a = 0; a < NP; ++a) {
            acc[RR::OFF_C + a] = lds_c[a * kFB];
            tri += NP - 1 - a;
            acc[RR::OFF_JTJ + tri] = lds_c[(NP + a) * kFB];
            acc[RR::OFF_B + tri] = lds_c[(2 * NP + a) * kFB];
            tri += 1;
        }
    }
    if (A.beat && threadIdx.x == 0 && blockIdx.x < 512) A.beat[8 + blockIdx.x] = ((unsigned long long)A.slot << 8) | 3;
    if (A.beat && (threadIdx.x & 63) == 0 && blockIdx.x < 64) A.beat[8 + 256 + blockIdx.x * 4 + 0] |= 1ull << (threadIdx.x >> 6);
    if (A.beat && blockIdx.x == 0 && threadIdx.x == 0) A.beat[0] = ((unsigned long long)A.slot << 8) | 3;
    if (stamp) tk[3] = wall_clock64();
    if (A.stamps && blockIdx.x == 0 && (threadIdx.x & 63) == 0) A.stamps[8 + (threadIdx.x >> 6)] += wall_clock64();
    static_assert(RR::GMAX == RR::NW - 1, "the max slot is the row's last");
    block_reduce_store_halving<RR::NW>(acc, s_red, A.partials + (int64_t)blockIdx.x * RR::NW);
    if (A.beat && threadIdx.x == 0) {
        if (A.beat[7]) atomicAdd(&A.beat[3], 1ull);
        if (blockIdx.x == 0) A.beat[0] = ((unsigned long long)A.slot << 8) | 4;
        if (blockIdx.x < 512) A.beat[8 + blockIdx.x] = ((unsigned long long)A.slot << 8) | 4;
    }
    if (stamp) {
        tk[4] = wall_clock64();
        A.stamps[0] += tk[1] - tk[0], A.stamps[1] += tk[2] - tk[1], A.stamps[2] += tk[3] - tk[2], A.stamps[3] += tk[4] - tk[3], A.stamps[4] += 1;
        if (tk[4 + 0]) A.stamps[5] += tk[4 + 0] - tk[1], A.stamps[6] += tk[4 + 1] - tk[4 + 0], A.stamps[7] += tk[2] - tk[4 + 1];
    }
}

template <int NP>
__global__ __launch_bounds__(kFB) void refine_rf_apply_kernel(const double* __restrict__ rows, int nrows, int row_stride, RfLists lists,
                                                             const RefineState* __restrict__ st_in, RefineState* __restrict__ st_out,
                                                             const RfExt* __restrict__ ext_in, RfExt* __restrict__ ext_out, int64_t m_total,
                                                             const int64_t* __restrict__ m_total_dev, double* __restrict__ trace, int trace_rows,
                                                             unsigned long long* __restrict__ beat, int slot) {
    __shared__ RfStageLds<NP> s_stage;
    __shared__ RefineState s_state;
    if (beat && threadIdx.x == 0) beat[1] = ((unsigned long long)slot << 8) | 1;
    state_to_lds(&s_state, st_in);
    RefineState* st = &s_state;
    if (st->termination < 0 && st->pending_apply) {
        const int64_t mt = m_total_dev ? *m_total_dev : (m_total >= 0 ? m_total : st->m);
        rf_apply_body<NP>(st, s_stage, rows, nrows >= 0 ? nrows : st->grid, row_stride, lists, ext_in, ext_out, mt, trace, trace_rows, nullptr, beat);
    }
    __syncthreads();
    if (beat && threadIdx.x == 0) beat[1] = ((unsigned long long)slot << 8) | 40;
    if (threadIdx.x == 0) st->pending_apply = 0;
    __syncthreads();
    state_from_lds(st_out, st);
}

template <int NP>
__global__ __launch_bounds__(kFB) void refine_rf_row_kernel(const double* __restrict__ partials, int nblocks, const RefineState* __restrict__ st,
                                                           const int* __restrict__ list_count, const double* __restrict__ list_entries,
                                                           double* __restrict__ row) {
    using RR = RfRow<NP>;
    __shared__ double s_grp[ReduceShape<RR::NW>::G][RR::NW];
    __shared__ double s[RR::NW];
    if (nblocks < 0) nblocks = st->grid;
    reduce_partials_groups<RR::NW>(partials, nblocks, RR::GMAX, s_grp, threadIdx.x, RR::NW, 0);
    __syncthreads();
    reduce_partials_slots<RR::NW>(s_grp, RR::GMAX, s, threadIdx.x);
    __syncthreads();
    if (threadIdx.x < RR::NW) row[threadIdx.x] = s[threadIdx.x];
    const int n = *list_count;
    double* lr = row + RR::NW;
    if (threadIdx.x == 0) {
        reinterpret_cast<int*>(lr)[0] = n;
        reinterpret_cast<int*>(lr)[1] = 0;
        lr[1] = 0.0;
    }
    if ((int)threadIdx.x < n && n <= kRfListCap) {
        const double* e = list_entries + (size_t)threadIdx.x * kRfEntry;
        int rank = 0;
        for (int j = 0; j < n; ++j) rank += (list_entries[(size_t)j * kRfEntry + 7] < e[7]) ? 1 : 0;
#pragma unroll
        for (int q = 0; q < kRfEntry; ++q) lr[2 + (size_t)rank * kRfEntry + q] = e[q];
    }
}


int refine_rf_extra_doubles() { return 3 * kRfListCap * kRfEntry + 2 * kRfExtDoubles + 8; }
int refine_rf_row_doubles(int np) { return (np == 7 ? RfRow<7>::NW : RfRow<6>::NW) + kRfListDoubles; }

namespace {
static_assert(kWorkgroupsPerCu == 1, "rf_grid_cap and the cap of RefineState::grid (refine_state_from_best_kernel) agree only at one workgroup per CU");
inline int rf_grid_cap(const Ctx* c) { return c->num_cus; }
inline int rf_grid(const Ctx* c, int64_t m) {
    int64_t b = (m + kFB - 1) / kFB;
    const int64_t cap = rf_grid_cap(c);
    if (b < 1) b = 1;
    if (b > cap) {
        const int64_t iters = (b + cap - 1) / cap;
        b = (b + iters - 1) / iters;
    }
    return (int)b;
}
struct RfLayout {
    double* rows[2];
    RefineState* cs[2];
    double* list[3];
    RfExt* ext[2];
};
static_assert(RfRow<7>::NW <= SlotRow<7>::NW && RfRow<6>::NW <= SlotRow<7>::NW, "the rows buffer is sized by SlotRow<7>::NW doubles per workgroup");
inline RfLayout rf_layout(const Ctx* c, const RefineBuffers& B) {
    RfLayout Lo;
    double* base = B.partials;
    const size_t half = (size_t)refine_partials_half_doubles(c);
    Lo.rows[0] = base, Lo.rows[1] = base + half;
    double* p = base + 2 * half;
    const size_t sd = (size_t)refine_state_doubles();
    Lo.cs[0] = reinterpret_cast<RefineState*>(p), Lo.cs[1] = reinterpret_cast<RefineState*>(p + sd);
    p += 2 * sd + 8;
    for (int i = 0; i < 3; ++i) Lo.list[i] = p + (size_t)i * kRfListCap * kRfEntry;
    p += 3 * kRfListCap * kRfEntry;
    Lo.ext[0] = reinterpret_cast<RfExt*>(p), Lo.ext[1] = reinterpret_cast<RfExt*>(p + kRfExtDoubles);
    return Lo;
}
inline int rf_mod3(int g) { return ((g % 3) + 3) % 3; }
inline int* rf_list_count(const RefineBuffers& B, int g) { return refine_rf_counters(B) + rf_mod3(g); }
inline double* rf_list_entries(const RfLayout& Lo, int g) { return Lo.list[rf_mod3(g)]; }
inline RfLists rf_lists_of(const RfLayout& Lo, const RefineBuffers& B, int g, const double* rows_all, int nranks, int nw) {
    RfLists l;
    if (rows_all) {
        l.counts = reinterpret_cast<const int*>(rows_all + nw), l.count_stride = 2 * (nw + kRfListDoubles);
        l.entries = rows_all + nw + 2, l.entry_stride = nw + kRfListDoubles, l.nlists = nranks;
    } else {
        l.counts = rf_list_count(B, g), l.count_stride = 0, l.entries = rf_list_entries(Lo, g), l.entry_stride = 0, l.nlists = 1;
    }
    return l;
}

struct RfBeat {
    const Ctx* c;
    unsigned long long* words;
};
RfBeat g_beats[32];
int g_nbeats = 0;
unsigned long long* rf_beat(Ctx* c) {
    static const bool on = getenv("RSDSFM_SYNC_WATCHDOG_S") != nullptr && getenv("RSDSFM_NO_BEAT") == nullptr;
    if (!on) return nullptr;
    for (int i = 0; i < g_nbeats; ++i)
        if (g_beats[i].c == c) return g_beats[i].words;
    if (g_nbeats >= 32) return nullptr;
    unsigned long long* w = nullptr;
    if (hipHostMalloc((void**)&w, 64 + 8 * 512, hipHostMallocDefault) != hipSuccess) return nullptr;
    for (int i = 0; i < 8 + 512; ++i) w[i] = 0;
    w[7] = getenv("RSDSFM_BEAT_COUNT_WORKGROUPS") ? 1 : 0;
    g_beats[g_nbeats].c = c, g_beats[g_nbeats].words = w;
    ++g_nbeats;
    return w;
}
unsigned long long* rf_stamps(Ctx* c) {
    static int on = -1;
    static unsigned long long* buf = nullptr;
    if (on < 0) {
        const char* e = getenv("RSDSFM_RF_STAMPS");
        on = (e && e[0] == '1') ? 1 : 0;
        if (on && (hipMalloc(&buf, 128) != hipSuccess || hipMemset(buf, 0, 128) != hipSuccess)) buf = nullptr;
    }
    (void)c;
    return buf;
}
template <int NP, bool ZSUM>
void rf_pass_launch_t(Ctx* c, const RfPassArgs& A, bool first, int grid) {
    if (first)
        hipLaunchKernelGGL((refine_rf_pass_kernel<NP, true, ZSUM>), dim3(grid), dim3(kFB), 0, c->stream, A);
    else
        hipLaunchKernelGGL((refine_rf_pass_kernel<NP, false, ZSUM>), dim3(grid), dim3(kFB), 0, c->stream, A);
}
}

int refine_rf_pass_launch(Ctx* c, const RefineBuffers& B, int np, int g, int g_first, const double* rows_all_prev, int nranks, int64_t m_total,
                          const int64_t* m_total_dev, bool publish) {
    const RfLayout Lo = rf_layout(c, B);
    const int grid = B.m_on_device ? rf_grid_cap(c) : rf_grid(c, B.m);
    const int nw = np == 7 ? RfRow<7>::NW : RfRow<6>::NW;
    RfPassArgs A = {};
    A.m = B.m_on_device ? -1 : B.m;
    A.xyuv_in = reinterpret_cast<const double4*>(B.uu);
    A.xyuv_out = reinterpret_cast<double4*>(B.uu);
    A.beta = B.beta;
    A.alpha = B.alpha;
    A.alpha_k = B.alpha_k;
    A.rho_a = B.rho_a;
    A.rho_b = B.rho_b;
    A.st_in = g == g_first ? B.state : Lo.cs[(g - 1) & 1];
    A.st_out = publish ? B.state : Lo.cs[g & 1];
    if (rows_all_prev)
        A.rows_prev = rows_all_prev, A.nrows_prev = nranks, A.row_stride = nw + kRfListDoubles;
    else
        A.rows_prev = Lo.rows[(g - 1) & 1], A.nrows_prev = B.m_on_device ? -1 : grid, A.row_stride = nw;
    A.lists_prev = rf_lists_of(Lo, B, g - 1, rows_all_prev, nranks, nw);
    A.list_count = rf_list_count(B, g);
    A.list_entries = rf_list_entries(Lo, g);
    A.list_count_zero = rf_list_count(B, g + 1);
    A.ext_in = Lo.ext[(g - 1) & 1];
    A.ext_out = Lo.ext[g & 1];
    A.partials = Lo.rows[g & 1];
    A.trace = c->d_refine_trace;
    A.trace_rows = c->refine_trace_rows;
    A.m_total = m_total;
    A.m_total_dev = m_total_dev;
    A.flow = reinterpret_cast<const double2*>(B.flow);
    A.n_flow = B.n_flow;
    A.inl = B.inl;
    A.inlier_idx = B.inlier_idx;
    A.flow_index_mode = B.flow_index_mode;
    A.bad_index = B.bad_index;
    A.best = g == 0 ? B.best_dev : nullptr;
    A.grid_cap = rf_grid_cap(c);
    A.stamps = rf_stamps(c);
    A.beat = rf_beat(c);
    A.slot = g;
    const bool first = g == 0;
    if (np == 7) {
        if (B.want_zsum) rf_pass_launch_t<7, true>(c, A, first, grid); else rf_pass_launch_t<7, false>(c, A, first, grid);
    } else {
        if (B.want_zsum) rf_pass_launch_t<6, true>(c, A, first, grid); else rf_pass_launch_t<6, false>(c, A, first, grid);
    }
    RSDSFM_HIP_CHECK(c, hipGetLastError());
    return RSDSFM_OK;
}

int refine_rf_apply_launch(Ctx* c, const RefineBuffers& B, int np, int g, bool to_published, const double* rows_all, int nranks, int64_t m_total,
                           const int64_t* m_total_dev) {
    const RfLayout Lo = rf_layout(c, B);
    const int grid = B.m_on_device ? rf_grid_cap(c) : rf_grid(c, B.m);
    const int nw = np == 7 ? RfRow<7>::NW : RfRow<6>::NW;
    const double* rows = rows_all ? rows_all : Lo.rows[g & 1];
    const int nrows = rows_all ? nranks : (B.m_on_device ? -1 : grid);
    const int stride = rows_all ? nw + kRfListDoubles : nw;
    const RfLists lists = rf_lists_of(Lo, B, g, rows_all, nranks, nw);
    RefineState* st_io = Lo.cs[g & 1];
    if (np == 7)
        hipLaunchKernelGGL(refine_rf_apply_kernel<7>, dim3(1), dim3(kFB), 0, c->stream, rows, nrows, stride, lists, st_io, to_published ? B.state : st_io,
                           Lo.ext[g & 1], Lo.ext[(g + 1) & 1], m_total, m_total_dev, c->d_refine_trace, c->refine_trace_rows, rf_beat(c), g);
    else
        hipLaunchKernelGGL(refine_rf_apply_kernel<6>, dim3(1), dim3(kFB), 0, c->stream, rows, nrows, stride, lists, st_io, to_published ? B.state : st_io,
                           Lo.ext[g & 1], Lo.ext[(g + 1) & 1], m_total, m_total_dev, c->d_refine_trace, c->refine_trace_rows, rf_beat(c), g);
    RSDSFM_HIP_CHECK(c, hipGetLastError());
    return RSDSFM_OK;
}

int refine_rf_row_launch(Ctx* c, const RefineBuffers& B, int np, int g, double* row) {
    const RfLayout Lo = rf_layout(c, B);
    const int grid = B.m_on_device ? rf_grid_cap(c) : rf_grid(c, B.m);
    if (np == 7)
        hipLaunchKernelGGL(refine_rf_row_kernel<7>, dim3(1), dim3(kFB), 0, c->stream, Lo.rows[g & 1], B.m_on_device ? -1 : grid, static_cast<const RefineState*>(Lo.cs[g & 1]),
                           rf_list_count(B, g), rf_list_entries(Lo, g), row);
    else
        hipLaunchKernelGGL(refine_rf_row_kernel<6>, dim3(1), dim3(kFB), 0, c->stream, Lo.rows[g & 1], B.m_on_device ? -1 : grid, static_cast<const RefineState*>(Lo.cs[g & 1]),
                           rf_list_count(B, g), rf_list_entries(Lo, g), row);
    RSDSFM_HIP_CHECK(c, hipGetLastError());
    return RSDSFM_OK;
}

void refine_rf_debug_dump(Ctx* c, const RefineBuffers& B) {
    const RfLayout Lo = rf_layout(c, B);
    hipStream_t s2 = nullptr;
    if (hipStreamCreateWithFlags(&s2, hipStreamNonBlocking) != hipSuccess) return;
    RefineState h[3];
    int cnt[8] = {0, 0, 0, 0, 0, 0, 0, 0};
    const RefineState* src[3] = {B.state, Lo.cs[0], Lo.cs[1]};
    for (int i = 0; i < 3; ++i) (void)hipMemcpyAsync(&h[i], src[i], sizeof(RefineState), hipMemcpyDeviceToHost, s2);
    (void)hipMemcpyAsync(cnt, B.bad_index, sizeof(int) * 8, hipMemcpyDeviceToHost, s2);
    if (hipStreamSynchronize(s2) != hipSuccess) {
        fprintf(stderr, "[rsdsfm] refinement dump: the copies did not complete either\n");
        return;
    }
    const char* names[3] = {"published", "chunk state 0", "chunk state 1"};
    for (int i = 0; i < 3; ++i)
        fprintf(stderr, "[rsdsfm] %s: np %d termination %d iteration %d slots %d pending_apply %d rf %d guard %d cur %d solve_ok %d m %lld grid %d radius %g cost %g successful %d unsuccessful %d invalid_run %d\n",
                names[i], h[i].np, h[i].termination, h[i].iteration, h[i].slots, h[i].pending_apply, h[i].rf, h[i].rf_guard, h[i].cur, h[i].solve_ok, (long long)h[i].m, h[i].grid, h[i].radius,
                h[i].cost, h[i].num_successful, h[i].num_unsuccessful, h[i].invalid_run);
    fprintf(stderr, "[rsdsfm] bad_index %d, list counters %d %d %d (m_on_device %d, m %lld)\n", cnt[0], cnt[4], cnt[5], cnt[6], (int)B.m_on_device, (long long)B.m);
    for (int i = 0; i < g_nbeats; ++i)
        fprintf(stderr, "[rsdsfm] context %p%s: last pass slot %llu phase %llu; pass workgroups started %llu, left %llu; last stage kernel slot %llu phase %llu\n", (const void*)g_beats[i].c, g_beats[i].c == c ? " (the waiting one)" : "",
                g_beats[i].words[0] >> 8, g_beats[i].words[0] & 255, g_beats[i].words[2], g_beats[i].words[3], g_beats[i].words[1] >> 8, g_beats[i].words[1] & 255);
    for (int i = 0; i < g_nbeats; ++i) {
        if (g_beats[i].c != c) continue;
        int hist[16] = {0};
        const unsigned long long last = g_beats[i].words[0] >> 8;
        fprintf(stderr, "[rsdsfm] workgroups of the waiting context's pass (slot %llu) not at phase 4 / 9:", last);
        for (int b = 0; b < 256; ++b) {
            const unsigned long long w = g_beats[i].words[8 + b];
            hist[w & 15] += 1;
            if ((w & 255) != 4 && (w & 255) != 9) fprintf(stderr, " [%d: slot %llu phase %llu]", b, w >> 8, w & 255);
        }
        fprintf(stderr, "\n[rsdsfm] phase histogram:");
        for (int p = 0; p < 10; ++p) fprintf(stderr, " %d:%d", p, hist[p]);
        fprintf(stderr, "\n");
    }
}

int refine_rf_read_stamps(Ctx* c, unsigned long long out[16]) {
    unsigned long long* b = rf_stamps(c);
    if (!b) return RSDSFM_ERR_INVALID;
    RSDSFM_HIP_CHECK(c, hipStreamSynchronize(c->stream));
    RSDSFM_HIP_CHECK(c, hipMemcpy(out, b, 128, hipMemcpyDeviceToHost));
    RSDSFM_HIP_CHECK(c, hipMemset(b, 0, 128));
    return RSDSFM_OK;
}

}
```

### rs-aware-differential-sfm_amd/csrc/rsdsfm_internal.hpp

```cpp
#pragma once

#include <hip/hip_runtime.h>
#include <stdint.h>

#include <functional>
#include <string>
#include <vector>

#include "../../include/rsdsfm.h"

namespace rsdsfm {

constexpr int kMaxIter = 50;
constexpr int kRefineTraceCols = RSDSFM_REFINE_TRACE_COLS;
constexpr double kInitialRadius = 1e4;
constexpr double kMaxRadius = 1e16;
constexpr double kMinRadius = 1e-32;
constexpr double kMinRelDecrease = 1e-3;
constexpr double kMinLmDiag = 1e-6;
constexpr double kMaxLmDiag = 1e32;
constexpr double kFunctionTol = 1e-6;
constexpr double kGradientTol = 1e-10;
static_assert(kGradientTol < 1.0, "the indicator encoding of the gradient-maximum slots needs kGradientTol < 1");
constexpr double kParameterTol = 1e-8;
constexpr int kMaxInvalid = 5;
constexpr double kLmaTie = 1e-11;

constexpr int KMAX = 3;
constexpr int NS = 3 + 5 * KMAX;

struct Pose {
    double v[3];
    double w[3];
    double k;
};

struct LmScal {
    int32_t status;
    int32_t n_hist;
    int32_t K;
    int32_t write_which;
    int32_t iteration;
    int32_t num_successful;
    int32_t num_unsuccessful;
    int32_t invalid_run;
    int32_t termination;
    int32_t rho_holds;
    int32_t launches;
    int32_t next_launch;
    int32_t predict;
    int32_t restart;
    double radius;
    double decrease_factor;
    double cost;
    double initial_cost;
    double cand[KMAX];
};
struct LmState : LmScal {
    double hist[kMaxIter];
};

constexpr size_t kRefineStateBlockTail = 32;
struct RansacBest {
    int32_t best_trial;
    int32_t undecided;
    int64_t num_inliers;
    int64_t num_inliers_scan;
    double inlier_error;
    double hyp[8];
    int32_t lma_tie;
    int32_t shared_best;
    int32_t _pad_shared;
    int32_t lazy_pending;
};
struct PickLazy {
    int* scored = nullptr;
    int* list = nullptr;
    int* list_count = nullptr;
};

constexpr int kScoreIdleLimit = 4;
constexpr int kRansacBatch = 128;

struct Ctx {
    int device = 0;
    hipStream_t stream = nullptr;
    bool own_stream = false;
    std::string err;
    double* d_partials = nullptr;
    unsigned* d_tickets = nullptr;
    LmState* d_lm = nullptr;
    LmState* h_lm = nullptr;
    int lm_issued_k = 0;
    int true_flow_exhaustive = 0;
    int ransac_fused_base = 2;
    int ransac_score_idle = kScoreIdleLimit;
    int refine_iters_hint = -1;
    int ransac_standard_math = 0;
    int* d_core_flag = nullptr;
    int core_epoch = 0;
    int ransac_math_mode = 0;
    int64_t ransac_restarts = 0;
    int lm_arithmetic = 0;
    int lma_hold = 0;
    bool lma_count_only_force = false;
    int64_t lma_count_only_runs = 0, lma_lazy_runs = 0;
    int lma_unique_run = 0;
    int64_t lma_restarts = 0;
    int64_t lma_handed_over = 0;
    int lma_last_guard = 0;
    int* d_lma_list = nullptr;
    int depth_lma_parity = 0;
    int lma_cand[2] = {2, 1};
    int ransac_spec_miss = 0;
    int frame_dense_hint = 1;
    int lm_issued_d = 0;
    int depth_epoch = 0;
    int depth_standard_math = 0;
    int64_t depth_restarts = 0;
    int depth_core_launch = 0;
    int prof_what = 0;
    void* d_stage = nullptr;
    size_t stage_bytes = 0;
    void* d_ws = nullptr;
    size_t ws_bytes = 0;
    void* d_frame = nullptr;
    size_t frame_bytes = 0;
    void* h_pinned = nullptr;
    hipEvent_t ev_ready = nullptr;
    size_t pinned_bytes = 0;
    int num_cus = 256;
    int ransac_k0 = 0;
    int ransac_not_one_step = -1;
    bool profile = false;
    hipEvent_t ev_prof[2] = {nullptr, nullptr};
    unsigned long long* d_clk_probe = nullptr;
    bool prof_pending = false;
    double* d_refine_trace = nullptr;
    int refine_trace_rows = 0;
    int depth_variant = 0;
    void* d_tile = nullptr;
    size_t tile_bytes = 0;
    void* tile_session = nullptr;
    int tile_np = 0;
    void* flow_pair = nullptr;
    void* flow_clip = nullptr;
    int flow_batch = 0;
    void* flow_check = nullptr;
    void* link = nullptr;
    void* fuse = nullptr;
    void* rectify_dense = nullptr;
    unsigned* d_claim[3] = {nullptr, nullptr, nullptr};
    size_t claim_words[3] = {0, 0, 0};
    unsigned claim_epoch[3] = {0, 0, 0};
    void* dist = nullptr;
    void* frame_run = nullptr;
    hipStream_t aux_stream = nullptr;
    hipEvent_t ev_fork = nullptr, ev_join = nullptr, ev_seq = nullptr;
    int frame_side_flatten = 3;
    int frame_tail = 0;
    unsigned long long* d_flat_counters = nullptr;
    int seq_lanes = 0;
    int refine_stage_mode = 0;
    bool refine_stage_separate = false;
    int refine_arithmetic = 0;
    int64_t refine_rf_runs = 0, refine_rf_restarts = 0, refine_rf_resolves = 0;
    int refine_rf_last_guard = 0;
    struct RansacCache {
        uint64_t tag = 0, stage_gen = 0;
        const double *d_u = nullptr, *d_inl = nullptr, *d_alpha = nullptr, *d_alpha_k = nullptr;
        const int64_t* d_idx = nullptr;
        int64_t n = 0, m = 0;
        const void* h_u = nullptr;
        double u_probe[16] = {0};
        double inl_probe[16] = {0};
    } ransac_cache;
    uint64_t stage_gen = 0, ransac_tag_counter = 0;
    int64_t refine_cache_hits = 0;
    std::vector<rsdsfm_ctx*> lanes;
};
constexpr int kSequenceLanesDefault = 3;
void dist_release(Ctx* c);
void dist_reset_hold(Ctx* c);
void frame_release(Ctx* c);
void flow_release(Ctx* c);
void flow_check_release(Ctx* c);
void rectify_dense_release(Ctx* c);
void link_release(Ctx* c);
void fuse_release(Ctx* c);

constexpr int kDepthBlock = 256;
constexpr int kDepthMaxBlocks = 512;
constexpr int kDecideBlock = 256;
constexpr int kDepthBatchMax = 8;

#define RSDSFM_HIP_CHECK(ctx, expr)                                                            \
    do {                                                                                       \
        hipError_t _e = (expr);                                                                \
        if (_e != hipSuccess) {                                                                \
            (ctx)->err = std::string(#expr) + ": " + hipGetErrorString(_e);                    \
            return RSDSFM_ERR_HIP;                                                             \
        }                                                                                      \
    } while (0)

struct DeviceGuard {
    int prev = -1;
    bool switched = false;
    explicit DeviceGuard(const Ctx* c) {
        if (hipGetDevice(&prev) == hipSuccess && prev != c->device) switched = hipSetDevice(c->device) == hipSuccess;
    }
    ~DeviceGuard() {
        if (switched) (void)hipSetDevice(prev);
    }
    DeviceGuard(const DeviceGuard&) = delete;
    DeviceGuard& operator=(const DeviceGuard&) = delete;
};

int fail(Ctx* c, int code, const char* msg);
int ensure_stage(Ctx* c, size_t bytes);
struct XferItem {
    void* host;
    const void* dev;
    size_t bytes;
};
struct XferUp {
    void* dev;
    const void* host;
    size_t bytes;
};
int xfer_h2d(Ctx* c, void* d_dst, const void* h_src, size_t bytes);
int xfer_h2d_many(Ctx* c, const XferUp* items, int count);
int xfer_d2h(Ctx* c, void* h_dst, const void* d_src, size_t bytes);
int xfer_d2h_many(Ctx* c, const XferItem* items, int count);
bool xfer_trace_on();
void xfer_trace(const char* label);
void xfer_trace_span(const char* label, double us);
void xfer_trace_dump(const char* what);
int ensure_ws(Ctx* c, size_t bytes);
int sync_stream(Ctx* c, const char* where);
void set_sync_dumper(std::function<void(Ctx*)> f);
int ensure_pinned(Ctx* c, size_t bytes);

struct Arena {
    char* base;
    size_t off = 0;
    explicit Arena(void* b) : base(static_cast<char*>(b)) {}
    template <class T>
    T* take(size_t count) {
        T* p = reinterpret_cast<T*>(base + off);
        off += need(count * sizeof(T));
        return p;
    }
    static size_t need(size_t bytes) { return (bytes + 255) & ~(size_t)255; }
};


int depth_closed_form_launch(Ctx* c, const double* q, const double* u, const double* a, const double* ak,
                             int64_t n, const Pose& pose, double* rho);
int depth_lm_launch(Ctx* c, const double* q, const double* u, const double* a, const double* ak, int64_t n,
                    const Pose& pose, double* rho, int launch_id, bool core = false);
int depth_lm_decide_launch(Ctx* c, int64_t n, int launch_id);
int depth_lm_decide_apply_launch(Ctx* c, const double* q, const double* u, const double* a, const double* ak, int64_t n,
                                 const Pose& pose, double* rho);
int depth_lm_batch_launch(Ctx* const* cs, int count, const double* const* q, const double* const* u, const double* const* a,
                          const double* const* ak, const int64_t* n, const Pose* poses, double* const* rho, int launch0_only);
int depth_lm_fused_launch(Ctx* c, const double* q, const double* u, const double* a, const double* ak, int64_t n,
                          const Pose& pose, double* rho);
int depth_lm_reduce_launch(Ctx* c, int64_t n, double* d_row);
void fill_lm_summary(const LmState& st, rsdsfm_lm_summary* s);
int depth_lm_decide_rows_launch(Ctx* c, const double* d_rows, int nrows, int64_t n_total, int launch_id);
bool depth_lma_allowed(const Ctx* c, int64_t n);
int depth_lma_batch_launch(Ctx* const* cs, int count, const double* const* q, const double* const* u, const double* const* a,
                           const double* const* ak, const int64_t* n, const Pose* poses, double* const* rho);
int depth_lma_row_doubles();
int depth_lma_shard_launch(Ctx* c, const double* q, const double* u, const double* a, const double* ak, int64_t n, const Pose& pose, double* rho, double* d_row);
int depth_lma_shard_finish_launch(Ctx* c, const double* q, const double* u, const double* a, const double* ak, int64_t n, const Pose& pose, double* rho,
                                  const double* d_rows_all, int nranks, int64_t n_total);

}

namespace rsdsfm {
int alpha_launch(Ctx* c, const double* flow_px, int64_t n, double h, double gamma, double* alpha);
int alpha_k_launch(Ctx* c, const double* q_px, const double* flow_px, int64_t n, double h, double gamma, double* alpha_k);
int depth_map_device(Ctx* c, double* d_inl, int64_t m, double v_inout[3], double fx, double fy, double cx, double cy, int32_t rows, int32_t cols,
                     double* d_depth_map, int32_t* d_xs, int32_t* d_ys, int* flipped, const double* w_or_null, double k, double gamma,
                     double* d_R_rows9, double* d_t_rows3);
struct PoseTableOut {
    double* R = nullptr;
    double* t = nullptr;
    int rows = 0;
    double gamma = 0.0;
    const double* wk_dev = nullptr;
};
int pose_table_launch(Ctx* c, const Pose& pose, double gamma, int rows, double* R, double* t, const double* v_dev = nullptr,
                      const double* wk_dev = nullptr);
int64_t flatten_cells(int rows, int cols);
int flatten_launch(Ctx* c, const double* d_img, int rows, int cols, int col0, double fx, double fy, double cx, double cy,
                   double gamma, double thr, double* d_q, double* d_u, double* d_alpha, double* d_alpha_k, int64_t* d_counts,
                   int64_t* d_offsets, int64_t* d_total, hipEvent_t total_ready = nullptr);
int depth_map_launch(Ctx* c, double* d_inl, int64_t m, const double v[3], double fx, double fy, double cx, double cy, int rows,
                     int cols, double* d_depth_map, int32_t* d_xs, int32_t* d_ys, double* d_header, double* d_partials,
                     double* h_header = nullptr, const double* v_dev = nullptr, const int64_t* m_dev = nullptr,
                     const PoseTableOut* pt = nullptr);
int depth_map_slab_launch(Ctx* c, double* d_inl, int64_t m, const double* d_zsums, int nz, int64_t m_total, const double v[3],
                          double fx, double fy, double cx, double cy, int rows, int col0, int ncols, double* d_depth_map,
                          int32_t* d_xs, int32_t* d_ys, double* d_header, double* h_header = nullptr, const double* v_dev = nullptr,
                          const int64_t* m_dev = nullptr, const PoseTableOut* pt = nullptr);
int claim_map_acquire(Ctx* c, int which, size_t npix, unsigned** map, unsigned* tag, unsigned* mask);
int claim_map_reserve(Ctx* c, int which, size_t words);
int zsum_row_launch(Ctx* c, const double* d_inl, int64_t m, double* d_partials, double* d_out);
}

namespace rsdsfm {
struct Minimal9Direct {
    const double* img = nullptr;
    int rows = 0, cols = 0, alpha_ones = 0;
    double fx = 0, fy = 0, cx = 0, cy = 0, gamma = 0;
    int* core_flag = nullptr;
    int core_epoch = 0;
    double* probe = nullptr;
};
int minimal9_launch(Ctx* c, const double* q, const double* u, const double* alpha, const double* alpha_k,
                    const int32_t* samples, int T, int use_alpha_k, int k_sign_mode, double* hyp_out, void* zero_begin = nullptr,
                    size_t zero_bytes = 0, const Minimal9Direct* direct = nullptr);
struct DenseFlatten {
    double thr = 0.0;
    double *d_q = nullptr, *d_u = nullptr, *d_alpha = nullptr, *d_alpha_k = nullptr;
    unsigned long long* d_counters = nullptr;
    int64_t* total_out = nullptr;
};
int minimal9_flatten_launch(Ctx* c, const int32_t* samples, int T, int use_alpha_k, int k_sign_mode, double* hyp_out, void* zero_begin, size_t zero_bytes,
                            const Minimal9Direct& direct, double thr, double* d_q, double* d_u, double* d_alpha, double* d_alpha_k,
                            unsigned long long* d_counters, int64_t* total_out);
}

namespace rsdsfm {
int ransac_pixel_grid(const Ctx* c, int64_t n);
int ransac_lm_partials_doubles(const Ctx* c, int64_t n, int batch);
int ransac_lm_round_launch(Ctx* c, const double* q, const double* u, const double* a, const double* ak, int64_t n,
                           const double* hyp, int T, LmState* states, double* partials, int* flags, int* scored,
                           double* trial_count, double* trial_err, int round, double tol, int k0, int fused_base, bool core_math,
                           const int* m9_core_flag = nullptr, int m9_core_epoch = 0, int* unscored_list = nullptr);
int ransac_score_launch(Ctx* c, const double* q, const double* u, const double* a, const double* ak, int64_t n,
                        const double* hyp, int T, const LmState* states, int depth_mode, double tol, const int* scored,
                        double* partials, double* trial_count, double* trial_err, const int* unscored_list = nullptr, const int* unscored_count = nullptr);
int ransac_pick_launch(Ctx* c, const double* trial_count, const double* trial_err, int T, const double* hyp, RansacBest* best,
                       RansacBest* best_host = nullptr, const int* d_flags = nullptr, int* h_flags = nullptr, int scored_ahead = 0,
                       const double* cnt_rt = nullptr, int cnt_stride = 0, int nranks = 0, int64_t* m_all = nullptr, double tie_margin = 0.0,
                       PickLazy lazy = PickLazy());
int ransac_final_launch(Ctx* c, const double* q, const double* u, const double* a, const double* ak, int64_t n,
                        RansacBest* best, const LmState* states, int depth_mode, double tol, double* rho, uint8_t* mask,
                        int64_t* block_counts, int64_t* block_offsets, int64_t* inlier_idx, double* inliers,
                        double* out_alpha, double* out_alpha_k, RansacBest* best_host = nullptr, int* zero_words = nullptr);
int ransac_rows_doubles();
int ransac_lm_rows_launch(Ctx* c, const double* q, const double* u, const double* a, const double* ak, int64_t n,
                          const double* hyp, int T, const LmState* states, double* partials, int round, double tol, double* rows,
                          int* core_flags = nullptr, const int* m9_flag = nullptr, int m9_epoch = 0);
int ransac_rows_payload_doubles(int T, bool core_trailer);
int ransac_decide_rows_launch(Ctx* c, const double* rows_all, int nranks, int T, LmState* states, int64_t n_total, int round,
                              int* flags, int* scored, double* trial_count, double* trial_err, bool core_trailer = false,
                              double* cnt_rt = nullptr, int cnt_stride = 0);
int ransac_score_rows_launch(Ctx* c, const double* q, const double* u, const double* a, const double* ak, int64_t n,
                             const double* hyp, int T, const LmState* states, int depth_mode, double tol, const int* scored,
                             double* partials, double* rows);
int ransac_score_merge_launch(Ctx* c, const double* rows_all, int nranks, int T, const int* scored, double* trial_count,
                              double* trial_err, double* cnt_rt = nullptr, int cnt_stride = 0);
void sample_indices(int64_t n, int T, uint64_t seed, int32_t* out);
int64_t ransac_lma_partials_doubles(const Ctx* c, int64_t n, int batch);
size_t ransac_lma_list_ints(int batch);
int ransac_lma_launch(Ctx* c, const double* q, const double* u, const double* a, const double* ak, int64_t n, const double* hyp, int T,
                      LmState* states, double* partials, int* flags, int* scored, double* trial_count, double* trial_err, double tol,
                      const int* cand_steps, int ncand, int* irr_count, int* irr_list, int* unscored_list, int* guard_word,
                      const int* m9_core_flag = nullptr, int m9_core_epoch = 0, bool count_only = false);
int ransac_lma_rows_doubles();
int ransac_lma_rows_launch(Ctx* c, const double* q, const double* u, const double* a, const double* ak, int64_t n, const double* hyp, int T,
                           double* partials, double tol, const int* cand_steps, int ncand, int* irr_count, int* irr_list, double* rows);
int ransac_lma_decide_rows_launch(Ctx* c, const double* rows_all, int nranks, int64_t rank_stride, int T, int64_t n_total, const double* hyp,
                                  LmState* states, int* flags, int* scored, double* trial_count, double* trial_err, double tol, const int* cand_steps,
                                  int ncand, int* unscored_list, int* guard_word, double* cnt_rt, int cnt_stride, const int* m9_core_flag = nullptr,
                                  int m9_core_epoch = 0);
}

namespace rsdsfm {
struct RefineState {
    int32_t np, cur, iteration, invalid_run, num_successful, num_unsuccessful, termination, solve_ok;
    double p[7], pc[7], sp[7], yp[7];
    double radius, decrease_factor, cost, initial_cost, x_norm, gmax, stepsq_p;
    int64_t m;
    int32_t grid;
    int32_t need_schur;
    double zsum;
    int32_t slots;
    int32_t spec_miss_run;
    int32_t pending_apply;
    int32_t rf;
    double dp[7];
    double p0[7];
    int32_t rf_guard, rf_resolves;
};
constexpr int kTermRestartExact = 64;
struct FinishClaim {
    bool on = false;
    double fx = 0.0, fy = 0.0, cx = 0.0, cy = 0.0;
    int rows = 0, cols = 0;
    int32_t* ys = nullptr;
    unsigned* owner = nullptr;
    unsigned tag = 0, mask = 0;
};
struct RefineBuffers {
    const double* flow;
    int64_t n_flow, m;
    bool m_on_device = false;
    const double* inl;
    const double* alpha;
    const double* alpha_k;
    const int64_t* inlier_idx;
    int flow_index_mode;
    RefineState* state;
    double* uu;
    double* beta;
    double* rho_a;
    double* rho_b;
    double* srho;
    double* partials;
    int* bad_index;
    RefineState* state_host = nullptr;
    double* zpartials = nullptr;
    const RansacBest* best_dev = nullptr;
    FinishClaim claim;
    bool want_zsum = false;
};
size_t ransac_pinned_bytes(int T);
typedef std::function<int(const RansacBest*)> RansacSpecTail;
struct RansacRun {
    int pc = 0;
    const double *d_q = nullptr, *d_u = nullptr, *d_a = nullptr, *d_ak = nullptr;
    int64_t n = 0;
    int T = 0, Tn = 1, batch = 1, depth_mode = 0, use_alpha_k = 0, k_sign_mode = 0, k0 = 0, fused_base = 0;
    double tol = 0.0;
    rsdsfm_ransac_out* out = nullptr;
    const RansacSpecTail* spec_tail = nullptr;
    bool* spec_tail_held = nullptr;
    int core_epoch = 0;
    int* d_unscored = nullptr;
    bool core_math = true;
    bool analytic = false;
    bool lma_restarted = false;
    int* refine_flag_words = nullptr;
    bool count_only = false;
    int lazy_rounds = 0;
    int shared_best = 0;
    double tie_margin = 0.0;
    int lma_guard = 0;
    bool lma_tie_seen = false;
    int lma_cand[2] = {2, 1}, lma_cand_next[2] = {0, 0};
    int *d_irr_count = nullptr, *d_irr_list = nullptr;
    bool restarted = false;
    bool tail_ahead = true;
    const Minimal9Direct* direct = nullptr;
    const DenseFlatten* dense = nullptr;
    const std::function<int()>* after_minimal9 = nullptr;
    std::vector<int32_t> samples;
    double *d_hyp = nullptr, *d_partials = nullptr, *d_tcount = nullptr, *d_terr = nullptr, *d_rho = nullptr;
    char* zero_begin = nullptr;
    size_t zero_bytes = 0;
    LmState* d_states = nullptr;
    int *d_scored = nullptr, *d_flags = nullptr;
    RansacBest* d_best = nullptr;
    int64_t *d_bcounts = nullptr, *d_boffs = nullptr;
    uint8_t* d_mask = nullptr;
    RansacBest* h_best = nullptr;
    int* h_running = nullptr;
    double *h_tcount = nullptr, *h_terr = nullptr, *h_hyp = nullptr;
    LmState* h_states = nullptr;
    int32_t* h_samples_pinned = nullptr;
    int b0 = 0, B = 0, round = 0;
    bool need_score = true, final_done = false, spec_scored = false, tail_enqueued = false, spec_final = false;
    int not_one_step = 0, fused_base_next = 0, score_hint_next = -1;
    bool hints_ready = false;
};
int ransac_begin(Ctx* c, const double* d_q, const double* d_u, const double* d_a, const double* d_ak, int64_t n, int use_alpha_k, int T,
                 double tol, const int32_t* h_samples, uint64_t seed, int depth_mode, int k_sign_mode, rsdsfm_ransac_out* out,
                 const RansacSpecTail* spec_tail, bool* spec_tail_held, RansacRun* run, const Minimal9Direct* direct,
                 const std::function<int()>* after_minimal9, const DenseFlatten* dense = nullptr, bool tail_ahead = true, bool count_only = false,
                 int* refine_flag_words = nullptr);
int ransac_finish(Ctx* c, RansacRun* run);
void ransac_commit_hints(Ctx* c, const RansacRun& run);
int flatten_enqueue(Ctx* c, const double* d_img, int32_t rows, int32_t cols, double fx, double fy, double cx, double cy, double gamma,
                    double thr, double* d_q, double* d_u, double* d_alpha, double* d_alpha_k, int64_t* h_total);
typedef std::function<int(const RefineBuffers&)> RefineTail;
int refine_finish_grid(const Ctx* c, const RefineBuffers& B);
int depth_map_decided_launch(Ctx* c, double* d_inl, int64_t m, const double* d_zsums, int nz, const RefineBuffers& B, double* d_depth_map,
                             double* d_header, double* h_header, const double* v_dev, const int64_t* m_dev, const PoseTableOut* pt);
struct RefineRun {
    RefineBuffers B;
    int np = 6, launched = 0, chunk = 5, hint_prev = -1;
    bool rf = false;
    double* d_inl_out = nullptr;
    const RefineTail* tail = nullptr;
    RefineState* hs = nullptr;
    bool prefetch = false, prefetched = false;
    bool tail_done = false;
};
constexpr size_t kPinnedTail = 1024;
size_t refine_workspace_bytes(const Ctx* c, int64_t m, bool m_on_device);
int refine_begin(Ctx* c, const double* d_flow, int64_t n_flow, int64_t m, const double* d_inl, const double* d_alpha,
                 const double* d_alpha_k, const int64_t* d_inlier_idx, const double v_in[3], const double w_in[3], double k_in,
                 int const_acceleration, int flow_index_mode, double* d_inl_out, const RefineTail* tail, const RansacBest* d_best,
                 void* ws_base, RefineRun* run, RefineState* hs_prefetch, double* d_zpartials, bool exact = false,
                 const FinishClaim* claim = nullptr);
constexpr int kRcRefineRestartExact = 1;
int refine_device(Ctx* c, const double* d_flow, int64_t n_flow, int64_t m, const double* d_inl, const double* d_alpha,
                  const double* d_alpha_k, const int64_t* d_inlier_idx, const double v_in[3], const double w_in[3], double k_in,
                  int const_acceleration, int flow_index_mode, double* d_inl_out, double v_out[3], double w_out[3], double* k_out,
                  rsdsfm_lm_summary* summary, const RefineTail* tail, double* d_zpartials, bool exact = false, const FinishClaim* claim = nullptr);
int refine_enqueue_chunk(Ctx* c, RefineRun* run);
int frames_in_flight(const Ctx* c);
int refine_poll(Ctx* c, RefineRun* run, double v_out[3], double w_out[3], double* k_out, rsdsfm_lm_summary* summary);
int refine_partials_doubles(const Ctx* c, int64_t m);
int refine_partials_doubles_cap(const Ctx* c);
int refine_state_from_best_launch(Ctx* c, const RansacBest* d_best, const RefineBuffers& B, int np);
int* refine_flag_words(void* ws_base);
inline int refine_trace_reset(Ctx* c) {
    if (!c->d_refine_trace) return RSDSFM_OK;
    return hipMemsetAsync(c->d_refine_trace, 0xFF, (size_t)c->refine_trace_rows * kRefineTraceCols * sizeof(double), c->stream) == hipSuccess ? RSDSFM_OK : RSDSFM_ERR_HIP;
}
int refine_init_launch(Ctx* c, const RefineBuffers& B, int np);
int refine_rf_pass_launch(Ctx* c, const RefineBuffers& B, int np, int g, int g_first, const double* rows_all_prev, int nranks, int64_t m_total,
                          const int64_t* m_total_dev, bool publish = false);
int refine_rf_apply_launch(Ctx* c, const RefineBuffers& B, int np, int g, bool to_published, const double* rows_all, int nranks, int64_t m_total,
                           const int64_t* m_total_dev);
int refine_rf_row_launch(Ctx* c, const RefineBuffers& B, int np, int g, double* row);
int refine_rf_row_doubles(int np);
void refine_rf_debug_dump(Ctx* c, const RefineBuffers& B);
int refine_rf_read_stamps(Ctx* c, unsigned long long out[16]);
int refine_rf_extra_doubles();
int refine_partials_half_doubles(const Ctx* c);
int refine_state_doubles();
inline int* refine_rf_counters(const RefineBuffers& B) { return B.bad_index + 4; }
int refine_iter_launch(Ctx* c, const RefineBuffers& B, int np, int j, int chunk);
int refine_finish_launch(Ctx* c, const RefineBuffers& B, double* inl_out);
int refine_stage_row_doubles(int np, int stage);
int refine_slot_row_doubles(int np);
int refine_slot_partials_doubles(const Ctx* c, int64_t m);
int refine_slot_rows_launch(Ctx* c, const RefineBuffers& B, int np, double* row, int j, const double* rows_all_prev, int nranks);
int refine_slot_apply_launch(Ctx* c, const RefineBuffers& B, int np, const double* rows_all, int nranks, int chunk);
int refine_stage_rows_launch(Ctx* c, const RefineBuffers& B, int np, int stage, double* row);
int refine_stage_apply_launch(Ctx* c, const RefineBuffers& B, int np, int stage, const double* rows_all, int nranks, int64_t m_total,
                              const int64_t* m_total_dev = nullptr);
}

namespace rsdsfm {
int back_project_launch(Ctx* c, const unsigned char* d_img, const double* d_depth_cm, const double* d_R, const double* d_t, double fx,
                        double fy, double cx, double cy, int rows, int cols, int mode, int q5_mode, unsigned char* d_gs, float* d_c3d);
int interpolate_cracky_launch(Ctx* c, const unsigned char* d_in, int rows, int cols, int offset, unsigned char* d_out);
int rectify_frame_launch(Ctx* c, const double* d_inl, int64_t m, const unsigned char* d_img, const double* d_depth_cm, const double* d_R,
                         const double* d_t, double fx, double fy, double cx, double cy, int rows, int cols, int mode, int q5_mode, int offset,
                         unsigned char* d_preview, unsigned char* d_gs, float* d_c3d, unsigned char* d_fixed, double* d_partials);
int depth_preview_launch(Ctx* c, const double* d_inl, int64_t m, double fx, double fy, double cx, double cy, int rows, int cols,
                         unsigned char* d_out, double* d_partials);
}

struct rsdsfm_ctx {
    rsdsfm::Ctx c;
};
```

Before: 1761.

## Fuse RANSAC best-trial pick into final kernel and refine apply into finish

```diff
diff --git a/rs-aware-differential-sfm_amd/csrc/frame_host.hip b/rs-aware-differential-sfm_amd/csrc/frame_host.hip
--- a/rs-aware-differential-sfm_amd/csrc/frame_host.hip
+++ b/rs-aware-differential-sfm_amd/csrc/frame_host.hip
@@ -229,7 +229,8 @@
                                prm->depth_mode, prm->k_sign_mode, &F->ro, prm->use_refinement ? &F->spec_tail : nullptr, &F->refinement_enqueued, &F->ransac,
                                F->side_flatten ? &F->direct : nullptr, F->side_flatten && !F->dense_in_launch ? &F->join : nullptr,
                                F->dense_in_launch ? &F->dense : nullptr, F->ahead, true,
-                               F->claim.on && prm->use_refinement ? refine_flag_words(F->d_refine_ws) : nullptr);
+                               F->claim.on && prm->use_refinement ? refine_flag_words(F->d_refine_ws) : nullptr,
+                               c->frame_tail == 0 && !c->refine_stage_separate ? c->frame_chain : 0);
     return RSDSFM_OK;
 }
 
@@ -265,7 +266,8 @@
         rc = ransac_begin(c, F->d_q, F->d_u, F->d_a, F->d_ak, n, prm->use_acceleration_mode, prm->ransac_trials, prm->ransac_tol, nullptr, J.seed,
                           prm->depth_mode, prm->k_sign_mode, &F->ro, prm->use_refinement ? &F->spec_tail : nullptr, &F->refinement_enqueued, &F->ransac, nullptr, nullptr,
                           nullptr, F->ahead, true,
-                               F->claim.on && prm->use_refinement ? refine_flag_words(F->d_refine_ws) : nullptr);
+                               F->claim.on && prm->use_refinement ? refine_flag_words(F->d_refine_ws) : nullptr,
+                               c->frame_tail == 0 && !c->refine_stage_separate ? c->frame_chain : 0);
         if (rc == RSDSFM_OK) rc = ransac_finish(c, &F->ransac);
         counted = rc == RSDSFM_OK;
     }
@@ -426,6 +428,7 @@
         lc->lma_count_only_force = c->lma_count_only_force;
         lc->frame_side_flatten = c->frame_side_flatten;
         lc->frame_tail = c->frame_tail;
+        lc->frame_chain = c->frame_chain;
         lc->refine_stage_mode = c->refine_stage_mode;
     }
     for (int l = 0; l < L; ++l) lane_ctx(l)->refine_stage_separate = L > 1;
diff --git a/rs-aware-differential-sfm_amd/csrc/ransac_host.hip b/rs-aware-differential-sfm_amd/csrc/ransac_host.hip
--- a/rs-aware-differential-sfm_amd/csrc/ransac_host.hip
+++ b/rs-aware-differential-sfm_amd/csrc/ransac_host.hip
@@ -177,12 +177,17 @@
                         if (rc != RSDSFM_OK) return rc;
                         R.spec_scored = true;
                     }
-                    rc = ransac_pick_launch(c, R.d_tcount, R.d_terr, T, R.d_hyp, R.d_best, R.h_best, R.d_flags, R.h_running, R.spec_scored ? 1 : 0,
-                                            nullptr, 0, 0, nullptr, R.tie_margin, lazy);
-                    if (rc != RSDSFM_OK) return rc;
+                    const bool pick_in_final = R.pick_in_final && !R.count_only;
+                    const RansacFinalPick fp{R.d_tcount, R.d_terr, R.d_hyp, T, R.h_best, R.d_flags, R.h_running, R.spec_scored ? 1 : 0, R.tie_margin};
+                    if (!pick_in_final) {
+                        rc = ransac_pick_launch(c, R.d_tcount, R.d_terr, T, R.d_hyp, R.d_best, R.h_best, R.d_flags, R.h_running, R.spec_scored ? 1 : 0,
+                                                nullptr, 0, 0, nullptr, R.tie_margin, lazy);
+                        if (rc != RSDSFM_OK) return rc;
+                    }
                     flags_via_pick = true;
                     rc = ransac_final_launch(c, R.d_q, R.d_u, R.d_a, R.d_ak, n, R.d_best, R.d_states, depth_mode, tol, R.d_rho, R.d_mask, R.d_bcounts,
-                                             R.d_boffs, out->inlier_idx, out->inliers, out->alpha, out->alpha_k, R.h_best, R.refine_flag_words);
+                                             R.d_boffs, out->inlier_idx, out->inliers, out->alpha, out->alpha_k, R.h_best, R.refine_flag_words,
+                                             pick_in_final ? &fp : nullptr);
                     if (rc != RSDSFM_OK) return rc;
                     R.final_done = true;
                     R.spec_final = true;
@@ -265,11 +270,16 @@
                 if (!R.final_done) {
                     R.tail_enqueued = false;
                     R.spec_final = false;
-                    rc = ransac_pick_launch(c, R.d_tcount, R.d_terr, T, R.d_hyp, R.d_best, R.h_best, nullptr, nullptr, 0, nullptr, 0, 0, nullptr, R.tie_margin,
-                                            R.count_only ? PickLazy{R.d_scored, R.d_unscored, R.d_flags + 1} : PickLazy());
-                    if (rc != RSDSFM_OK) return rc;
+                    const bool pick_in_final = R.pick_in_final && !R.count_only;
+                    const RansacFinalPick fp{R.d_tcount, R.d_terr, R.d_hyp, T, R.h_best, nullptr, nullptr, 0, R.tie_margin};
+                    if (!pick_in_final) {
+                        rc = ransac_pick_launch(c, R.d_tcount, R.d_terr, T, R.d_hyp, R.d_best, R.h_best, nullptr, nullptr, 0, nullptr, 0, 0, nullptr, R.tie_margin,
+                                                R.count_only ? PickLazy{R.d_scored, R.d_unscored, R.d_flags + 1} : PickLazy());
+                        if (rc != RSDSFM_OK) return rc;
+                    }
                     rc = ransac_final_launch(c, R.d_q, R.d_u, R.d_a, R.d_ak, n, R.d_best, R.d_states, depth_mode, tol, R.d_rho, R.d_mask, R.d_bcounts,
-                                             R.d_boffs, out->inlier_idx, out->inliers, out->alpha, out->alpha_k, R.h_best, R.refine_flag_words);
+                                             R.d_boffs, out->inlier_idx, out->inliers, out->alpha, out->alpha_k, R.h_best, R.refine_flag_words,
+                                             pick_in_final ? &fp : nullptr);
                     if (rc != RSDSFM_OK) return rc;
                 }
                 if (R.spec_tail && !R.tail_enqueued) {
@@ -371,9 +381,11 @@
 int ransac_begin(Ctx* c, const double* d_q, const double* d_u, const double* d_a, const double* d_ak, int64_t n, int use_alpha_k, int T,
                  double tol, const int32_t* h_samples, uint64_t seed, int depth_mode, int k_sign_mode, rsdsfm_ransac_out* out,
                  const RansacSpecTail* spec_tail, bool* spec_tail_held, RansacRun* run, const Minimal9Direct* direct,
-                 const std::function<int()>* after_minimal9, const DenseFlatten* dense, bool tail_ahead, bool count_only, int* refine_flag_words) {
+                 const std::function<int()>* after_minimal9, const DenseFlatten* dense, bool tail_ahead, bool count_only, int* refine_flag_words,
+                 int frame_chain) {
     RansacRun& R = *run;
     R = RansacRun();
+    R.pick_in_final = (frame_chain & 1) != 0;
     R.tail_ahead = tail_ahead;
     R.core_math = c->ransac_math_mode == 0 && c->ransac_standard_math == 0;
     R.analytic = depth_mode == RSDSFM_DEPTH_CERES_LM && T > 0 && c->lm_arithmetic == 0 && c->lma_hold == 0;
diff --git a/rs-aware-differential-sfm_amd/csrc/ransac_kernels.hip b/rs-aware-differential-sfm_amd/csrc/ransac_kernels.hip
--- a/rs-aware-differential-sfm_amd/csrc/ransac_kernels.hip
+++ b/rs-aware-differential-sfm_amd/csrc/ransac_kernels.hip
@@ -607,12 +607,13 @@
 }
 
 __device__ __forceinline__ void pick_best_trial(const double* __restrict__ trial_count, const double* __restrict__ trial_err, int T,
-                                                int lane, int& bi, double& best_count, double& best_err) {
+                                                int lane, int& bi, double& best_count, double& best_err, double* c0 = nullptr, double* e0 = nullptr) {
     best_count = -1.0, best_err = 0.0;
     bi = -1;
     for (int t0 = 0; t0 < T; t0 += 64) {
         const int t = t0 + lane;
         const double cl = t < T ? trial_count[t] : 0.0, el = t < T ? trial_err[t] : 0.0;
+        if (c0 && t0 == 0) *c0 = cl, *e0 = el;
         const int nt = T - t0 < 64 ? T - t0 : 64;
         for (int j = 0; j < nt; ++j) {
             const double c = lane_value(cl, j), e = lane_value(el, j);
@@ -699,38 +700,129 @@
     }
 }
 
+struct FinalPick {
+    const double* trial_count = nullptr;
+    const double* trial_err = nullptr;
+    const double* hyp = nullptr;
+    const int* flags = nullptr;
+    int* flags_host = nullptr;
+    RansacBest* best_host = nullptr;
+    int T = 0, scored_ahead = 0;
+    double tie_margin = 0.0;
+};
+template <bool PICK>
 __global__ __launch_bounds__(kRB) void ransac_final_kernel(const double2* __restrict__ q, const double2* __restrict__ u,
                                                           const double* __restrict__ alpha,
                                                           const double* __restrict__ alpha_k, int64_t n, int64_t chunk,
-                                                          const RansacBest* __restrict__ best,
+                                                          RansacBest* __restrict__ best,
                                                           const LmState* __restrict__ states, int depth_mode, double tol,
                                                           double* __restrict__ rho_out, uint8_t* __restrict__ mask_out,
-                                                          int64_t* __restrict__ block_counts) {
+                                                          int64_t* __restrict__ block_counts, FinalPick pk) {
     __shared__ LmPlanLds plan;
     __shared__ int s_cnt[kRB / 64];
+    __shared__ double s_hyp[8];
+    __shared__ int s_pick[2];
     const int tid = threadIdx.x, lane = tid & 63, wv = tid >> 6;
-    if (best->undecided) return;
-    const int bt = best->best_trial;
-    Pose pose;
-    pose.w[0] = best->hyp[0], pose.w[1] = best->hyp[1], pose.w[2] = best->hyp[2];
-    pose.v[0] = best->hyp[3], pose.v[1] = best->hyp[4], pose.v[2] = best->hyp[5];
-    pose.k = best->hyp[6];
-    if (depth_mode == RSDSFM_DEPTH_CERES_LM && bt >= 0) {
-        if (tid == 0) {
-            plan.n_hist = states[bt].n_hist;
-            plan.K = 0;
-            plan.write_which = 0;
-        }
-        if (tid < kMaxIter) plan.inv_hist[tid] = 1.0 / states[bt].hist[tid];
-    }
-    __syncthreads();
-    const double two_over = 2.0 / (2.0 + pose.k);
     const int64_t i0 = (int64_t)blockIdx.x * chunk;
     const int64_t i1 = (i0 + chunk < n) ? i0 + chunk : n;
+    double2 qq0 = make_double2(0.0, 0.0), uu0 = make_double2(0.0, 0.0);
+    double al0 = 0.0, ak0 = 0.0;
+    if (PICK && i0 + tid < i1) qq0 = q[i0 + tid], uu0 = u[i0 + tid], al0 = alpha[i0 + tid], ak0 = alpha_k[i0 + tid];
+    int bt;
+    Pose pose;
+    if (PICK) {
+        static_assert(kMaxIter <= 64, "the winner's history is loaded by one wave");
+        if (wv == 0) {
+            const int T = pk.T;
+            const int fl = (pk.flags && lane < 8) ? pk.flags[lane] : 0;
+            double best_count, best_err, c0, e0;
+            int bi;
+            pick_best_trial(pk.trial_count, pk.trial_err, T, lane, bi, best_count, best_err, &c0, &e0);
+            const int f0 = __builtin_amdgcn_readlane(fl, 0), f1 = __builtin_amdgcn_readlane(fl, 1), f3 = __builtin_amdgcn_readlane(fl, 3);
+            const bool incomplete = f0 != 0 || (f1 > 0 && !pk.scored_ahead);
+            int undecided = (incomplete || f3 != 0) ? 1 : 0;
+            int tie = 0, ns = 0;
+            const bool guard = pk.tie_margin != 0.0 && bi >= 0 && best_count > 0.0 && !incomplete;
+            const bool shared = bi >= 0 && best_count > 0.0 && !undecided;
+            if (guard || shared) {
+                const double tm = fabs(pk.tie_margin);
+                for (int t0 = 0; t0 < T; t0 += 64) {
+                    const int t = t0 + lane;
+                    const double cl = t0 == 0 ? c0 : (t < T ? pk.trial_count[t] : 0.0), el = t0 == 0 ? e0 : (t < T ? pk.trial_err[t] : 0.0);
+                    const bool same = t < T && cl == best_count;
+                    const bool hit = same && t != bi && fabs(el - best_err) <= tm * best_count;
+                    if (guard && __builtin_amdgcn_ballot_w64(hit) != 0) tie = 1;
+                    if (shared) ns += __builtin_popcountll(__builtin_amdgcn_ballot_w64(same));
+                }
+            }
+            if (pk.tie_margin > 0.0) undecided |= tie;
+            const bool plan_on = depth_mode == RSDSFM_DEPTH_CERES_LM && bi >= 0;
+            const double h = (lane < 8 && bi >= 0) ? pk.hyp[(int64_t)bi * 8 + lane] : 0.0;
+            const double hist = (plan_on && lane < kMaxIter) ? states[bi].hist[lane] : 1.0;
+            const int n_hist = plan_on ? states[bi].n_hist : 0;
+            if (lane < 8) s_hyp[lane] = h;
+            if (lane == 0) s_pick[0] = bi, s_pick[1] = undecided;
+            if (plan_on) {
+                if (lane == 0) {
+                    plan.n_hist = n_hist;
+                    plan.K = 0;
+                    plan.write_which = 0;
+                }
+                if (lane < kMaxIter) plan.inv_hist[lane] = 1.0 / hist;
+            }
+            if (blockIdx.x == 0) {
+                RansacBest* best_host = pk.best_host;
+                if (pk.flags_host && lane < 8) pk.flags_host[lane] = fl | ((lane == 3 && tie && pk.tie_margin > 0.0) ? 4 : 0);
+                if (lane < 8) best->hyp[lane] = h;
+                if (lane < 8 && best_host) best_host->hyp[lane] = h;
+                if (lane == 0) {
+                    best->best_trial = bi;
+                    best->undecided = undecided;
+                    best->lma_tie = tie;
+                    best->lazy_pending = 0;
+                    best->shared_best = ns;
+                    best->num_inliers = bi >= 0 ? (int64_t)best_count : 0;
+                    best->inlier_error = best_err;
+                    if (best_host) {
+                        best_host->best_trial = bi;
+                        best_host->undecided = undecided;
+                        best_host->lma_tie = tie;
+                        best_host->lazy_pending = 0;
+                        best_host->shared_best = ns;
+                        best_host->num_inliers = bi >= 0 ? (int64_t)best_count : 0;
+                        best_host->inlier_error = best_err;
+                    }
+                }
+            }
+        }
+        __syncthreads();
+        if (s_pick[1]) return;
+        bt = s_pick[0];
+        pose.w[0] = s_hyp[0], pose.w[1] = s_hyp[1], pose.w[2] = s_hyp[2];
+        pose.v[0] = s_hyp[3], pose.v[1] = s_hyp[4], pose.v[2] = s_hyp[5];
+        pose.k = s_hyp[6];
+    } else {
+        if (best->undecided) return;
+        bt = best->best_trial;
+        pose.w[0] = best->hyp[0], pose.w[1] = best->hyp[1], pose.w[2] = best->hyp[2];
+        pose.v[0] = best->hyp[3], pose.v[1] = best->hyp[4], pose.v[2] = best->hyp[5];
+        pose.k = best->hyp[6];
+        if (depth_mode == RSDSFM_DEPTH_CERES_LM && bt >= 0) {
+            if (tid == 0) {
+                plan.n_hist = states[bt].n_hist;
+                plan.K = 0;
+                plan.write_which = 0;
+            }
+            if (tid < kMaxIter) plan.inv_hist[tid] = 1.0 / states[bt].hist[tid];
+        }
+        __syncthreads();
+    }
+    const double two_over = 2.0 / (2.0 + pose.k);
     int count = 0;
     for (int64_t i = i0 + tid; i < i1; i += kRB) {
-        double2 qq = q[i], uu = u[i];
-        const double al = alpha[i], ak = alpha_k[i];
+        const bool ahead = PICK && i == i0 + tid;
+        double2 qq = ahead ? qq0 : q[i], uu = ahead ? uu0 : u[i];
+        const double al = ahead ? al0 : alpha[i], ak = ahead ? ak0 : alpha_k[i];
         bool in = false;
         double rho = 0.0;
         if (bt >= 0) {
@@ -1019,18 +1111,25 @@
 int ransac_final_launch(Ctx* c, const double* q, const double* u, const double* a, const double* ak, int64_t n,
                         RansacBest* best, const LmState* states, int depth_mode, double tol, double* rho, uint8_t* mask,
                         int64_t* block_counts, int64_t* block_offsets, int64_t* inlier_idx, double* inliers,
-                        double* out_alpha, double* out_alpha_k, RansacBest* best_host, int* zero_words) {
+                        double* out_alpha, double* out_alpha_k, RansacBest* best_host, int* zero_words, const RansacFinalPick* pick) {
     int64_t blocks = (n + kRB - 1) / kRB;
     if (blocks < 1) blocks = 1;
-    const int64_t cap = 2048;
+    const int64_t cap = pick ? std::min<int64_t>(2048, std::max(1, c->num_cus * 4)) : 2048;
     int64_t chunk = kRB;
     if (blocks > cap) {
         chunk = ((blocks + cap - 1) / cap) * kRB;
         blocks = (n + chunk - 1) / chunk;
     }
-    hipLaunchKernelGGL(ransac_final_kernel, dim3((int)blocks), dim3(kRB), 0, c->stream, reinterpret_cast<const double2*>(q),
-                       reinterpret_cast<const double2*>(u), a, ak, n, chunk, best, states, depth_mode, tol, rho, mask,
-                       block_counts);
+    if (pick) {
+        FinalPick pk;
+        pk.trial_count = pick->trial_count, pk.trial_err = pick->trial_err, pk.hyp = pick->hyp, pk.flags = pick->d_flags, pk.flags_host = pick->h_flags;
+        pk.best_host = pick->best_host, pk.T = pick->T, pk.scored_ahead = pick->scored_ahead, pk.tie_margin = pick->tie_margin;
+        hipLaunchKernelGGL(ransac_final_kernel<true>, dim3((int)blocks), dim3(kRB), 0, c->stream, reinterpret_cast<const double2*>(q),
+                           reinterpret_cast<const double2*>(u), a, ak, n, chunk, best, states, depth_mode, tol, rho, mask, block_counts, pk);
+    } else {
+        hipLaunchKernelGGL(ransac_final_kernel<false>, dim3((int)blocks), dim3(kRB), 0, c->stream, reinterpret_cast<const double2*>(q),
+                           reinterpret_cast<const double2*>(u), a, ak, n, chunk, best, states, depth_mode, tol, rho, mask, block_counts, FinalPick());
+    }
     RSDSFM_HIP_CHECK(c, hipGetLastError());
     if (inlier_idx || inliers || out_alpha || out_alpha_k) {
         hipLaunchKernelGGL(ransac_scatter_kernel, dim3((int)blocks), dim3(kRB), 0, c->stream, reinterpret_cast<const double2*>(q),
diff --git a/rs-aware-differential-sfm_amd/csrc/refine_host.hip b/rs-aware-differential-sfm_amd/csrc/refine_host.hip
--- a/rs-aware-differential-sfm_amd/csrc/refine_host.hip
+++ b/rs-aware-differential-sfm_amd/csrc/refine_host.hip
@@ -60,6 +60,7 @@
     run->prefetch = hs_prefetch != nullptr;
     run->prefetched = false;
     B.state_host = hs_prefetch;
+    run->close_in_output = run->rf && B.claim.on && !c->refine_stage_separate && (c->frame_chain & 2) != 0;
     if (d_best && claim && claim->on && run->rf && !c->refine_stage_separate) {
         B.best_dev = d_best;
     } else if (d_best) {
@@ -103,12 +104,13 @@
         });
     }
     if (run->rf) {
-        for (int i = 0; i <= run->chunk; ++i) {
+        const int closing = run->close_in_output ? 0 : 1;
+        for (int i = 0; i < run->chunk + closing; ++i) {
             const int g = run->launched + i;
             int rc = refine_rf_pass_launch(c, run->B, run->np, g, run->launched, nullptr, 0, -1, nullptr, i == run->chunk);
             if (rc != RSDSFM_OK) return rc;
         }
-        run->launched += 1;
+        run->launched += closing;
     } else {
         for (int i = 0; i < run->chunk; ++i) {
             int rc = refine_iter_launch(c, run->B, run->np, i, run->chunk);
@@ -124,7 +126,7 @@
         rc = claim_map_acquire(c, 2, (size_t)std::max<int64_t>(std::max<int64_t>(npix, run->B.m), 1), &C.owner, &C.tag, &C.mask);
         if (rc != RSDSFM_OK) return rc;
     }
-    rc = refine_finish_launch(c, run->B, run->d_inl_out);
+    rc = run->rf && run->close_in_output ? refine_rf_finish_launch(c, run->B, run->np, run->launched, run->d_inl_out) : refine_finish_launch(c, run->B, run->d_inl_out);
     if (rc != RSDSFM_OK) return rc;
     run->tail_done = false;
     if (run->tail && !(run->hint_prev > run->launched + 1)) {
diff --git a/rs-aware-differential-sfm_amd/csrc/refine_rf_kernels.hip b/rs-aware-differential-sfm_amd/csrc/refine_rf_kernels.hip
--- a/rs-aware-differential-sfm_amd/csrc/refine_rf_kernels.hip
+++ b/rs-aware-differential-sfm_amd/csrc/refine_rf_kernels.hip
@@ -900,6 +900,78 @@
     if (threadIdx.x == 0) st->pending_apply = 0;
     __syncthreads();
     state_from_lds(st_out, st);
+}
+
+struct RfFinishArgs {
+    int64_t m;
+    const RefineState* st_in;
+    RefineState* st_out;
+    RefineState* state_host;
+    const double* rows_prev;
+    int nrows_prev, row_stride;
+    RfLists lists_prev;
+    const RfExt* ext_in;
+    RfExt* ext_out;
+    double* trace;
+    int trace_rows;
+    const double* inl;
+    const double* rho_a;
+    const double* rho_b;
+    double* inl_out;
+    double* zpartials;
+    const int* bad_index;
+    double fx, fy, cx, cy;
+    int rows, ncols;
+    unsigned* owner;
+    unsigned tag;
+    int32_t* ys;
+};
+template <int NP>
+__global__ __launch_bounds__(kFB) void refine_rf_finish_claim_kernel(const RfFinishArgs F) {
+    __shared__ RfStageLds<NP> s_stage;
+    __shared__ RefineState s_state;
+    __shared__ double s_red[kFB / 64];
+    state_to_lds(&s_state, F.st_in);
+    RefineState* st = &s_state;
+    if (st->termination < 0 && st->pending_apply) {
+        const int64_t mt = F.m >= 0 ? F.m : st->m;
+        rf_apply_body<NP>(st, s_stage, F.rows_prev, F.nrows_prev >= 0 ? F.nrows_prev : st->grid, F.row_stride, F.lists_prev, F.ext_in,
+                          blockIdx.x == 0 ? F.ext_out : nullptr, mt, blockIdx.x == 0 ? F.trace : nullptr, F.trace_rows);
+        __syncthreads();
+    }
+    if (threadIdx.x == 0) st->pending_apply = 0;
+    __syncthreads();
+    if (blockIdx.x == 0) {
+        state_from_lds(F.st_out, st);
+        if (F.state_host) {
+            state_from_lds(F.state_host, st);
+            if (threadIdx.x == 0) *reinterpret_cast<int*>(reinterpret_cast<char*>(F.state_host) + sizeof(RefineState)) = *F.bad_index;
+        }
+    }
+    const double* __restrict__ rho = st->cur ? F.rho_b : F.rho_a;
+    const int64_t m = F.m < 0 ? st->m : F.m;
+    const int64_t stride = (int64_t)gridDim.x * kFB;
+    double acc = 0.0;
+    for (int64_t i = (int64_t)blockIdx.x * kFB + threadIdx.x; i < m; i += stride) {
+        const double xn = F.inl[3 * i], yn = F.inl[3 * i + 1];
+        F.inl_out[3 * i] = xn;
+        F.inl_out[3 * i + 1] = yn;
+        const double z = 1.0 / rho[i];
+        F.inl_out[3 * i + 2] = z;
+        acc += z;
+        const int x = (int)(F.fx * xn + F.cx + 0.5);
+        const int y = (int)(F.fy * yn + F.cy + 0.5);
+        F.ys[i] = y;
+        if (x >= 0 && x < F.ncols && y >= 0 && y < F.rows) atomicMax(&F.owner[(int64_t)x * F.rows + y], F.tag | (unsigned)i);
+    }
+    const double r = wave_sum(acc);
+    if ((threadIdx.x & 63) == 0) s_red[threadIdx.x >> 6] = r;
+    __syncthreads();
+    if (threadIdx.x == 0) {
+        double t = s_red[0];
+        for (int w2 = 1; w2 < kFB / 64; ++w2) t += s_red[w2];
+        F.zpartials[blockIdx.x] = t;
+    }
 }
 
 template <int NP>
@@ -1075,6 +1147,33 @@
     return RSDSFM_OK;
 }
 
+int refine_rf_finish_launch(Ctx* c, const RefineBuffers& B, int np, int g, double* inl_out) {
+    const RfLayout Lo = rf_layout(c, B);
+    const int grid = B.m_on_device ? rf_grid_cap(c) : rf_grid(c, B.m);
+    const int nw = np == 7 ? RfRow<7>::NW : RfRow<6>::NW;
+    RfFinishArgs F = {};
+    F.m = B.m_on_device ? -1 : B.m;
+    F.st_in = Lo.cs[(g - 1) & 1];
+    F.st_out = B.state;
+    F.state_host = B.state_host;
+    F.rows_prev = Lo.rows[(g - 1) & 1], F.nrows_prev = B.m_on_device ? -1 : grid, F.row_stride = nw;
+    F.lists_prev = rf_lists_of(Lo, B, g - 1, nullptr, 0, nw);
+    F.ext_in = Lo.ext[(g - 1) & 1];
+    F.ext_out = Lo.ext[g & 1];
+    F.trace = c->d_refine_trace;
+    F.trace_rows = c->refine_trace_rows;
+    F.inl = B.inl, F.rho_a = B.rho_a, F.rho_b = B.rho_b, F.inl_out = inl_out, F.zpartials = B.zpartials, F.bad_index = B.bad_index;
+    F.fx = B.claim.fx, F.fy = B.claim.fy, F.cx = B.claim.cx, F.cy = B.claim.cy, F.rows = B.claim.rows, F.ncols = B.claim.cols;
+    F.owner = B.claim.owner, F.tag = B.claim.tag, F.ys = B.claim.ys;
+    const int out_grid = refine_finish_grid(c, B);
+    if (np == 7)
+        hipLaunchKernelGGL(refine_rf_finish_claim_kernel<7>, dim3(out_grid), dim3(kFB), 0, c->stream, F);
+    else
+        hipLaunchKernelGGL(refine_rf_finish_claim_kernel<6>, dim3(out_grid), dim3(kFB), 0, c->stream, F);
+    RSDSFM_HIP_CHECK(c, hipGetLastError());
+    return RSDSFM_OK;
+}
+
 int refine_rf_apply_launch(Ctx* c, const RefineBuffers& B, int np, int g, bool to_published, const double* rows_all, int nranks, int64_t m_total,
                            const int64_t* m_total_dev) {
     const RfLayout Lo = rf_layout(c, B);
diff --git a/rs-aware-differential-sfm_amd/csrc/rsdsfm_internal.hpp b/rs-aware-differential-sfm_amd/csrc/rsdsfm_internal.hpp
--- a/rs-aware-differential-sfm_amd/csrc/rsdsfm_internal.hpp
+++ b/rs-aware-differential-sfm_amd/csrc/rsdsfm_internal.hpp
@@ -2,6 +2,7 @@
 
 #include <hip/hip_runtime.h>
 #include <stdint.h>
+#include <stdlib.h>
 
 #include <functional>
 #include <string>
@@ -81,6 +82,14 @@
 
 constexpr int kScoreIdleLimit = 4;
 constexpr int kRansacBatch = 128;
+
+inline int frame_chain_default() {
+    static const int v = [] {
+        const char* e = getenv("RSDSFM_FRAME_CHAIN");
+        return e && *e ? atoi(e) & 3 : 3;
+    }();
+    return v;
+}
 
 struct Ctx {
     int device = 0;
@@ -159,6 +168,7 @@
     hipEvent_t ev_fork = nullptr, ev_join = nullptr, ev_seq = nullptr;
     int frame_side_flatten = 3;
     int frame_tail = 0;
+    int frame_chain = frame_chain_default();
     unsigned long long* d_flat_counters = nullptr;
     int seq_lanes = 0;
     int refine_stage_mode = 0;
@@ -348,10 +358,20 @@
                        RansacBest* best_host = nullptr, const int* d_flags = nullptr, int* h_flags = nullptr, int scored_ahead = 0,
                        const double* cnt_rt = nullptr, int cnt_stride = 0, int nranks = 0, int64_t* m_all = nullptr, double tie_margin = 0.0,
                        PickLazy lazy = PickLazy());
+struct RansacFinalPick {
+    const double *trial_count = nullptr, *trial_err = nullptr, *hyp = nullptr;
+    int T = 0;
+    RansacBest* best_host = nullptr;
+    const int* d_flags = nullptr;
+    int* h_flags = nullptr;
+    int scored_ahead = 0;
+    double tie_margin = 0.0;
+};
 int ransac_final_launch(Ctx* c, const double* q, const double* u, const double* a, const double* ak, int64_t n,
                         RansacBest* best, const LmState* states, int depth_mode, double tol, double* rho, uint8_t* mask,
                         int64_t* block_counts, int64_t* block_offsets, int64_t* inlier_idx, double* inliers,
-                        double* out_alpha, double* out_alpha_k, RansacBest* best_host = nullptr, int* zero_words = nullptr);
+                        double* out_alpha, double* out_alpha_k, RansacBest* best_host = nullptr, int* zero_words = nullptr,
+                        const RansacFinalPick* pick = nullptr);
 int ransac_rows_doubles();
 int ransac_lm_rows_launch(Ctx* c, const double* q, const double* u, const double* a, const double* ak, int64_t n,
                           const double* hyp, int T, const LmState* states, double* partials, int round, double tol, double* rows,
@@ -447,6 +467,7 @@
     bool analytic = false;
     bool lma_restarted = false;
     int* refine_flag_words = nullptr;
+    bool pick_in_final = false;
     bool count_only = false;
     int lazy_rounds = 0;
     int shared_best = 0;
@@ -483,7 +504,7 @@
                  double tol, const int32_t* h_samples, uint64_t seed, int depth_mode, int k_sign_mode, rsdsfm_ransac_out* out,
                  const RansacSpecTail* spec_tail, bool* spec_tail_held, RansacRun* run, const Minimal9Direct* direct,
                  const std::function<int()>* after_minimal9, const DenseFlatten* dense = nullptr, bool tail_ahead = true, bool count_only = false,
-                 int* refine_flag_words = nullptr);
+                 int* refine_flag_words = nullptr, int frame_chain = 0);
 int ransac_finish(Ctx* c, RansacRun* run);
 void ransac_commit_hints(Ctx* c, const RansacRun& run);
 int flatten_enqueue(Ctx* c, const double* d_img, int32_t rows, int32_t cols, double fx, double fy, double cx, double cy, double gamma,
@@ -496,6 +517,7 @@
     RefineBuffers B;
     int np = 6, launched = 0, chunk = 5, hint_prev = -1;
     bool rf = false;
+    bool close_in_output = false;
     double* d_inl_out = nullptr;
     const RefineTail* tail = nullptr;
     RefineState* hs = nullptr;
@@ -530,6 +552,7 @@
                           const int64_t* m_total_dev, bool publish = false);
 int refine_rf_apply_launch(Ctx* c, const RefineBuffers& B, int np, int g, bool to_published, const double* rows_all, int nranks, int64_t m_total,
                            const int64_t* m_total_dev);
+int refine_rf_finish_launch(Ctx* c, const RefineBuffers& B, int np, int g, double* inl_out);
 int refine_rf_row_launch(Ctx* c, const RefineBuffers& B, int np, int g, double* row);
 int refine_rf_row_doubles(int np);
 void refine_rf_debug_dump(Ctx* c, const RefineBuffers& B);
```

Result: no change. 1762, median of 2 (+0.1%).
